# rug-marl-group2/scopa

Measured on AMD Instinct MI355X. Metric: MiniScopa infoset-traversals/sec, higher is better.
Workload: dtype f64

## Files before the change

include/scopa.h:

```cpp
#ifndef SCOPA_H
#define SCOPA_H
#include <stddef.h>
#include <stdint.h>

#ifdef __cplusplus
extern "C" {
#endif

#define SCOPA_ABI_VERSION 1

enum {
    SCOPA_OK = 0,
    SCOPA_EINVAL = -1,
    SCOPA_ENODEV = -2,
    SCOPA_EHIP = -3,
    SCOPA_ESTATE = -4,
    SCOPA_ENOMEM = -5,
    SCOPA_ELIMIT = -6,
    SCOPA_ETIMEOUT = -7
};

#define SCOPA_N_CARDS 16
#define SCOPA_N_PLIES 8
#define SCOPA_N_DECISION 1653
#define SCOPA_N_TERMINAL 576
#define SCOPA_N_NODES 2229
#define SCOPA_MAX_ACTIONS 4

#define SCOPA_STEP_CLONED 0x80u
#define SCOPA_STEP_COUNT_MASK 0x7Fu
typedef struct scopa_state {
    uint16_t hand[2];
    uint32_t table;
    uint8_t  nh[2];
    uint8_t  nt;
    uint8_t  step;
    uint8_t  ncap[2];
    uint8_t  scopas[2];
} scopa_state;

typedef struct scopa_ctx scopa_ctx;

int32_t     scopa_abi_version(void);
const char *scopa_strerror(int32_t status);
const char *scopa_last_error(const scopa_ctx *ctx);

int32_t scopa_ctx_create(int32_t device_id, void *hip_stream, scopa_ctx **out);
int32_t scopa_ctx_destroy(scopa_ctx *ctx);
int32_t scopa_ctx_synchronize(scopa_ctx *ctx);

int32_t scopa_deal_py_seed(int64_t seed, uint8_t perm16[16]);
int32_t scopa_state_init(const uint8_t perm16[16], scopa_state *out);
int32_t scopa_state_step(scopa_state *s, int32_t action);
int32_t scopa_state_clone(const scopa_state *s, scopa_state *out);
int32_t scopa_state_is_terminal(const scopa_state *s);
int32_t scopa_state_current_player(const scopa_state *s);
int32_t scopa_state_legal(const scopa_state *s, int32_t player , int32_t out[4], int32_t *n);
int32_t scopa_state_rewards_x2(const scopa_state *s, int32_t r2[2]);
int32_t scopa_state_infoset_key(const scopa_state *s, int32_t player, uint64_t *key);
int32_t scopa_key_to_string(uint64_t key, char *buf, int32_t cap);
int32_t scopa_state_infoset_string(const scopa_state *s, int32_t player, char *buf, int32_t cap);

int32_t scopa_step_batch(scopa_ctx *ctx, scopa_state *d_states, const uint8_t *d_actions, int64_t n);
int32_t scopa_step_batch_host(scopa_ctx *ctx, scopa_state *h_states, const uint8_t *h_actions, int64_t n);

int32_t scopa_set_deal(scopa_ctx *ctx, const uint8_t perm16[16]);
int32_t scopa_tree_counts(scopa_ctx *ctx, int32_t *n_nodes, int32_t *n_decision, int32_t *n_infosets);
int32_t scopa_tree_export(scopa_ctx *ctx, scopa_state *h_states, int32_t *h_infoset, int8_t *h_r2,
                          uint64_t *h_infoset_key, int8_t *h_infoset_nlegal, int8_t *h_infoset_legal);

int32_t scopa_tables_reset(scopa_ctx *ctx);
int32_t scopa_tables_get(scopa_ctx *ctx, double *h_regret, double *h_strategy, double *h_local);
int32_t scopa_tables_set(scopa_ctx *ctx, const double *h_regret, const double *h_strategy, const double *h_local);

int32_t scopa_visited_get(scopa_ctx *ctx, uint32_t *h_seq);

int32_t scopa_cfr_exact_iterate(scopa_ctx *ctx, int32_t n_iters, double *h_root_values);
int32_t scopa_cfr_exact_traverse(scopa_ctx *ctx, int32_t traverser, double *h_value);
int32_t scopa_cfr_exact_mode(scopa_ctx *ctx, int32_t sequential);
int32_t scopa_cfr_exact_last_route(scopa_ctx *ctx, int32_t *route);
int32_t scopa_cfr_exact_traverse_from(scopa_ctx *ctx, int32_t traverser, int32_t depth, const int32_t *path,
                                      double reach_p0, double reach_p1, double *h_value);

int32_t scopa_cfr_sync_iterate(scopa_ctx *ctx, int32_t n_iters);

int32_t scopa_mccfr_replay(scopa_ctx *ctx, int32_t n_iters, const double *h_uniforms, int64_t n_uniforms,
                           int64_t *consumed);

int32_t scopa_mccfr_seed(scopa_ctx *ctx, uint64_t seed);
int32_t scopa_mccfr_iterate(scopa_ctx *ctx, uint32_t batch, uint32_t n_iters);
int32_t scopa_mccfr_traverse(scopa_ctx *ctx, uint32_t iteration, uint32_t b0, uint32_t nb);
int32_t scopa_mccfr_delta_buffer(scopa_ctx *ctx, void **d_delta, size_t *bytes);
int32_t scopa_mccfr_bind_delta(scopa_ctx *ctx, void *d_buf, size_t bytes);
int32_t scopa_mccfr_delta_get(scopa_ctx *ctx, double *h_delta);
int32_t scopa_mccfr_delta_set(scopa_ctx *ctx, const double *h_delta);
int32_t scopa_mccfr_apply(scopa_ctx *ctx);
int32_t scopa_mccfr_iteration_counter(scopa_ctx *ctx, uint32_t *iteration);
int32_t scopa_mccfr_graph_mode(scopa_ctx *ctx, int32_t on);
int32_t scopa_debug_lds_limit(scopa_ctx *ctx, int32_t bytes);

int32_t scopa_sdcfr_frontier_width(int32_t traverser, int32_t ply);
int32_t scopa_sdcfr_features(scopa_ctx *ctx, int32_t ply, int64_t n, const int32_t *d_idx, float *d_feats, float *d_mask);
int32_t scopa_sdcfr_expand(scopa_ctx *ctx, int32_t ply, int32_t traverser, int64_t n, const int32_t *d_idx, const float *d_adv,
                           int32_t *d_child_idx, float *d_pol, const double *d_uniforms, uint32_t iteration, uint32_t b0);
int32_t scopa_sdcfr_terminal_values(scopa_ctx *ctx, int32_t traverser, int64_t n, const int32_t *d_idx, float *d_val);
int32_t scopa_sdcfr_backward(scopa_ctx *ctx, int32_t ply, int32_t traverser, int64_t n, const int32_t *d_idx, const float *d_pol,
                             const float *d_child_val, float *d_val, const float *d_feats, const float *d_mask, float *d_mem_feat,
                             float *d_mem_regret, float *d_mem_mask, int64_t capacity, int64_t write_base);
int32_t scopa_sdcfr_visits(scopa_ctx *ctx, uint64_t *decision_visits);
int32_t scopa_sdcfr_policy_get(scopa_ctx *ctx, float *h_policy, uint64_t *h_thr);
#define SCOPA_SDCFR_IMAGE_FLOATS 13520
int32_t scopa_sdcfr_image_floats(void);
int32_t scopa_sdcfr_pack_weights(scopa_ctx *ctx, int32_t player, const float *d_w1, const float *d_b1, const float *d_w2,
                                 const float *d_b2, const float *d_w3, const float *d_b3, float *d_image);
int32_t scopa_sdcfr_traverse_fused(scopa_ctx *ctx, int32_t traverser, int32_t batch, const float *d_image, float *d_mem_feat,
                                   float *d_mem_regret, float *d_mem_mask, int64_t capacity, int64_t write_base,
                                   float *d_root_values, const double *d_uniforms, uint32_t iteration, uint32_t b0);
int32_t scopa_sdcfr_mode(scopa_ctx *ctx, int32_t forward_per_visit);
int32_t scopa_sdcfr_tuning(scopa_ctx *ctx, int32_t traversals_per_task, int32_t wavefronts_per_task);
int32_t scopa_sdcfr_train_params(void);
int32_t scopa_sdcfr_train_steps(scopa_ctx *ctx, const int64_t *d_rows, int32_t n_rows, int32_t n_steps, const float *d_feat, const float *d_regret, const float *d_mask,
                                int64_t capacity, float *d_w1, float *d_b1, float *d_w2, float *d_b2, float *d_w3, float *d_b3, float *d_state,
                                int32_t first_step, float lr, float *d_loss);
int32_t scopa_sdcfr_train_step(scopa_ctx *ctx, const int64_t *d_rows, int32_t n_rows, const float *d_feat, const float *d_regret, const float *d_mask,
                               int64_t capacity, float *d_w1, float *d_b1, float *d_w2, float *d_b2, float *d_w3, float *d_b3, float *d_state,
                               int32_t step, float lr, float *d_loss);
int32_t scopa_sdcfr_average_policy(scopa_ctx *ctx, int32_t player, int32_t n_snap, const float *d_w1, const float *d_b1, const float *d_w2,
                                   const float *d_b2, const float *d_w3, const float *d_b3, int32_t max_size, const int32_t *d_slots,
                                   const float *d_coef, double *d_policy);
int32_t scopa_features_from_states(scopa_ctx *ctx, const scopa_state *d_states, int64_t n, float *d_feats, float *d_mask);
int32_t scopa_eval_init_states(scopa_ctx *ctx, scopa_state *d_states, int64_t n);
int32_t scopa_eval_step(scopa_ctx *ctx, scopa_state *d_states, int64_t n, const float *d_probs, const int32_t *d_trained_seat,
                        uint32_t stream_id, uint32_t ply_tag);

int32_t scopa_eval_tabular_prepare(scopa_ctx *ctx, const double *d_policy);
int32_t scopa_eval_tabular_step(scopa_ctx *ctx, scopa_state *d_states, int32_t *d_node_idx, int64_t n, int32_t ply,
                                const double *d_policy, const int32_t *d_trained_seat, uint32_t stream_id);
int32_t scopa_eval_tabular_match(scopa_ctx *ctx, int64_t n, int64_t n_seat0, uint32_t stream_id, scopa_state *d_states_out, int32_t *d_node_idx_out,
                                 int64_t h_stats[10]);

int32_t scopa_exploitability(scopa_ctx *ctx, const double *h_policy, double *h_out4, double *h_policy_out);

typedef struct scopa_multi scopa_multi;
int32_t scopa_multi_create(scopa_ctx *ctx, int32_t n_deals, scopa_multi **out);
int32_t scopa_multi_destroy(scopa_multi *m);
int32_t scopa_multi_deal_py_seeds(scopa_multi *m, const int64_t *h_seeds);
int32_t scopa_multi_set_perms(scopa_multi *m, const uint8_t *h_perms );
int32_t scopa_multi_perms_get(scopa_multi *m, uint8_t *h_perms);
int32_t scopa_multi_build(scopa_multi *m, int32_t *h_n_infosets);
int32_t scopa_multi_cfr_exact_iterate(scopa_multi *m, int32_t n_iters);
int32_t scopa_multi_cfr_exact_iterate_lanes(scopa_multi *m, int32_t n_iters);
int32_t scopa_multi_cfr_sync_iterate(scopa_multi *m, int32_t n_iters);
int32_t scopa_multi_mccfr_iterate(scopa_multi *m, uint32_t batch, uint32_t n_iters, uint64_t seed);
int32_t scopa_multi_exploitability(scopa_multi *m, double *h_out4);
int32_t scopa_multi_tables_get(scopa_multi *m, int32_t deal, double *h_regret, double *h_strategy, double *h_local, uint64_t *h_keys);
int32_t scopa_multi_tables_set(scopa_multi *m, int32_t deal, const double *h_regret, const double *h_strategy, const double *h_local);
int32_t scopa_multi_counters(scopa_multi *m, uint64_t *decision_visits, uint64_t *terminal_visits);

typedef struct scopa_full_state {
    uint64_t table[2];
    uint64_t cap[2];
    uint32_t hand[2];
    uint32_t game;
    uint8_t  nh[2], nt, deck_pos, round, last_capture , scopas[2];
    uint16_t step;
    uint8_t  terminal;
    int8_t   r2_p0;
    uint8_t  flags;
    uint8_t  pad[7];
} scopa_full_state;
int32_t scopa_full_deal_py_seed(int64_t seed, uint8_t perm40[40]);
int32_t scopa_full_state_init(const uint8_t deck40[40], uint32_t game, scopa_full_state *out);
int32_t scopa_full_state_step(scopa_full_state *s, const uint8_t deck40[40], int32_t action);
int32_t scopa_full_state_legal(const scopa_full_state *s, int32_t player, int32_t out[3], int32_t *n);
int32_t scopa_full_state_infoset_string(const scopa_full_state *s, int32_t player, char *buf, int32_t cap);
int32_t scopa_full_step_batch(scopa_ctx *ctx, scopa_full_state *d_states, const uint8_t *d_actions, const uint8_t *d_decks, int64_t n);
int32_t scopa_full_step_batch_host(scopa_ctx *ctx, scopa_full_state *h_states, const uint8_t *h_actions, const uint8_t *h_decks,
                                   int64_t n_decks, int64_t n);
int32_t scopa_full_random_playouts(scopa_ctx *ctx, const int64_t *h_seeds, int64_t n_games, int8_t *h_r2_p0, int16_t *h_plies);

typedef struct scopa_team_state {
    uint64_t history;
    uint32_t table;
    uint16_t hand[4];
    uint16_t cap[4];
    uint8_t  nh[4];
    uint8_t  scopas[4];
    uint8_t  nt, step, last_capture_team , flags ;
} scopa_team_state;
int32_t scopa_team_state_init(const uint8_t perm16[16], scopa_team_state *out);
int32_t scopa_team_state_step(scopa_team_state *s, int32_t action);
int32_t scopa_team_state_legal(const scopa_team_state *s, int32_t out[4], int32_t *n);
int32_t scopa_team_state_rewards_x2(const scopa_team_state *s, int32_t r2_seat[4]);
int32_t scopa_team_state_infoset_string(const scopa_team_state *s, int32_t team, char *buf, int32_t cap);
int32_t scopa_team_step_batch(scopa_ctx *ctx, scopa_team_state *d_states, const uint8_t *d_actions, int64_t n);
int32_t scopa_team_step_batch_host(scopa_ctx *ctx, scopa_team_state *h_states, const uint8_t *h_actions, int64_t n);
int32_t scopa_team_random_playouts(scopa_ctx *ctx, const int64_t *h_seeds, int64_t n_games, int8_t *h_r2_team0, uint8_t *h_scopas);

int32_t scopa_p2p_create(scopa_ctx *ctx, int32_t rank, int32_t world, uint8_t handle_out[64]);
int32_t scopa_p2p_connect(scopa_ctx *ctx, const uint8_t *handles );
int32_t scopa_p2p_allreduce_delta(scopa_ctx *ctx);
int32_t scopa_p2p_set_form(scopa_ctx *ctx, int32_t light);
int32_t scopa_p2p_set_budget(scopa_ctx *ctx, double seconds);
int32_t scopa_mccfr_iterate_sharded(scopa_ctx *ctx, uint32_t b0, uint32_t nb, uint32_t n_iters);
int32_t scopa_p2p_status(scopa_ctx *ctx, int32_t *timeouts, uint64_t *exchanges);
int32_t scopa_p2p_destroy(scopa_ctx *ctx);

int32_t scopa_counters(scopa_ctx *ctx, uint64_t *decision_visits, uint64_t *terminal_visits);
int32_t scopa_prof_enable(scopa_ctx *ctx, int32_t stride);
int32_t scopa_prof_read(scopa_ctx *ctx, int64_t *launches, double *kernel_ms);
int32_t scopa_prof_device(scopa_ctx *ctx, int64_t *launches, double *kernel_ms);
int32_t scopa_prof_phases(scopa_ctx *ctx, double out_us[3]);
int32_t scopa_prof_spread(scopa_ctx *ctx, double out_us[3]);

#ifdef __cplusplus
}
#endif
#endif
```

scopa_amd/_lib.py:

```python
import ctypes as C
import os

import numpy as np

_HERE = os.path.dirname(os.path.abspath(__file__))
LIB_PATH = os.environ.get("SCOPA_HIP_LIBRARY") or os.path.join(_HERE, "libscopa_hip.so")

SCOPA_OK, SCOPA_EINVAL, SCOPA_ENODEV, SCOPA_EHIP, SCOPA_ESTATE, SCOPA_ENOMEM, SCOPA_ELIMIT, SCOPA_ETIMEOUT = 0, -1, -2, -3, -4, -5, -6, -7
N_NODES, N_DECISION, N_TERMINAL = 2229, 1653, 576

SYMBOLS = [
    "scopa_abi_version", "scopa_strerror", "scopa_last_error", "scopa_ctx_create", "scopa_ctx_destroy",
    "scopa_ctx_synchronize", "scopa_deal_py_seed", "scopa_state_init", "scopa_state_step", "scopa_state_clone", "scopa_state_is_terminal",
    "scopa_state_current_player", "scopa_state_legal", "scopa_state_rewards_x2", "scopa_state_infoset_key",
    "scopa_key_to_string", "scopa_state_infoset_string", "scopa_step_batch", "scopa_step_batch_host", "scopa_set_deal",
    "scopa_tree_counts", "scopa_tree_export", "scopa_tables_reset", "scopa_tables_get", "scopa_tables_set",
    "scopa_visited_get", "scopa_cfr_exact_iterate", "scopa_cfr_exact_traverse", "scopa_cfr_exact_mode", "scopa_cfr_exact_last_route", "scopa_cfr_exact_traverse_from", "scopa_mccfr_replay", "scopa_mccfr_seed",
    "scopa_mccfr_iterate", "scopa_mccfr_traverse", "scopa_mccfr_delta_buffer", "scopa_mccfr_bind_delta", "scopa_mccfr_delta_get", "scopa_mccfr_delta_set", "scopa_mccfr_apply",
    "scopa_mccfr_iteration_counter", "scopa_mccfr_graph_mode", "scopa_debug_lds_limit", "scopa_sdcfr_frontier_width", "scopa_sdcfr_features", "scopa_sdcfr_expand",
    "scopa_sdcfr_terminal_values", "scopa_sdcfr_backward", "scopa_sdcfr_visits", "scopa_sdcfr_policy_get", "scopa_sdcfr_traverse_fused", "scopa_sdcfr_image_floats", "scopa_sdcfr_pack_weights", "scopa_sdcfr_tuning", "scopa_sdcfr_mode", "scopa_sdcfr_train_params", "scopa_sdcfr_train_step", "scopa_sdcfr_train_steps", "scopa_sdcfr_average_policy", "scopa_features_from_states",
    "scopa_eval_init_states", "scopa_eval_step", "scopa_eval_tabular_step", "scopa_eval_tabular_prepare", "scopa_eval_tabular_match", "scopa_cfr_sync_iterate", "scopa_multi_create", "scopa_multi_destroy",
    "scopa_multi_deal_py_seeds", "scopa_multi_set_perms", "scopa_multi_perms_get", "scopa_multi_build", "scopa_multi_cfr_exact_iterate",
    "scopa_multi_cfr_exact_iterate_lanes", "scopa_multi_cfr_sync_iterate", "scopa_multi_mccfr_iterate", "scopa_multi_exploitability", "scopa_multi_tables_get", "scopa_multi_tables_set", "scopa_multi_counters", "scopa_full_deal_py_seed",
    "scopa_full_state_init", "scopa_full_state_step", "scopa_full_state_legal", "scopa_full_state_infoset_string",
    "scopa_full_step_batch", "scopa_full_step_batch_host", "scopa_full_random_playouts",
    "scopa_team_state_init", "scopa_team_state_step", "scopa_team_state_legal", "scopa_team_state_rewards_x2", "scopa_team_state_infoset_string",
    "scopa_team_step_batch", "scopa_team_step_batch_host", "scopa_team_random_playouts",
    "scopa_mccfr_iterate_sharded", "scopa_p2p_create", "scopa_p2p_connect", "scopa_p2p_allreduce_delta", "scopa_p2p_set_form", "scopa_p2p_set_budget", "scopa_p2p_status", "scopa_p2p_destroy", "scopa_exploitability", "scopa_counters", "scopa_prof_enable", "scopa_prof_read", "scopa_prof_device", "scopa_prof_phases", "scopa_prof_spread",
]


class ScopaError(RuntimeError):
    def __init__(self, status, where, detail=""):
        self.status = status
        msg = f"{where}: status {status}"
        try:
            msg += f" ({lib().scopa_strerror(status).decode()})"
        except Exception:
            pass
        if detail:
            msg += f": {detail}"
        super().__init__(msg)


class State16(C.Structure):
    _fields_ = [("hand", C.c_uint16 * 2), ("table", C.c_uint32), ("nh", C.c_uint8 * 2), ("nt", C.c_uint8),
                ("step", C.c_uint8), ("ncap", C.c_uint8 * 2), ("scopas", C.c_uint8 * 2)]


STEP_CLONED, STEP_COUNT_MASK = 0x80, 0x7F
STATE_DTYPE = np.dtype([("hand", "<u2", (2,)), ("table", "<u4"), ("nh", "u1", (2,)), ("nt", "u1"), ("step", "u1"),
                        ("ncap", "u1", (2,)), ("scopas", "u1", (2,))])
assert STATE_DTYPE.itemsize == 16 and C.sizeof(State16) == 16

_lib = None


def lib():
    global _lib
    if _lib is not None:
        return _lib
    try:
        import torch
    except ImportError:
        pass
    if not os.path.exists(LIB_PATH):
        raise OSError(f"{LIB_PATH} is missing: build it with `python __graft_entry__.py` or `python scopa_amd/build.py` "
                      "(the MiniScopa solver path has no fallback)")
    L = C.CDLL(LIB_PATH)
    vp, i32, i64, u32, u64 = C.c_void_p, C.c_int32, C.c_int64, C.c_uint32, C.c_uint64
    sig = {
        "scopa_abi_version": (i32, []),
        "scopa_strerror": (C.c_char_p, [i32]),
        "scopa_last_error": (C.c_char_p, [vp]),
        "scopa_ctx_create": (i32, [i32, vp, C.POINTER(vp)]),
        "scopa_ctx_destroy": (i32, [vp]),
        "scopa_ctx_synchronize": (i32, [vp]),
        "scopa_deal_py_seed": (i32, [i64, vp]),
        "scopa_state_init": (i32, [vp, C.POINTER(State16)]),
        "scopa_state_step": (i32, [C.POINTER(State16), i32]),
        "scopa_state_clone": (i32, [C.POINTER(State16), C.POINTER(State16)]),
        "scopa_state_is_terminal": (i32, [C.POINTER(State16)]),
        "scopa_state_current_player": (i32, [C.POINTER(State16)]),
        "scopa_state_legal": (i32, [C.POINTER(State16), i32, C.POINTER(i32 * 4), C.POINTER(i32)]),
        "scopa_state_rewards_x2": (i32, [C.POINTER(State16), C.POINTER(i32 * 2)]),
        "scopa_state_infoset_key": (i32, [C.POINTER(State16), i32, C.POINTER(u64)]),
        "scopa_key_to_string": (i32, [u64, C.c_char_p, i32]),
        "scopa_state_infoset_string": (i32, [C.POINTER(State16), i32, C.c_char_p, i32]),
        "scopa_step_batch": (i32, [vp, vp, vp, i64]),
        "scopa_step_batch_host": (i32, [vp, vp, vp, i64]),
        "scopa_set_deal": (i32, [vp, vp]),
        "scopa_tree_counts": (i32, [vp, C.POINTER(i32), C.POINTER(i32), C.POINTER(i32)]),
        "scopa_tree_export": (i32, [vp, vp, vp, vp, vp, vp, vp]),
        "scopa_tables_reset": (i32, [vp]),
        "scopa_tables_get": (i32, [vp, vp, vp, vp]),
        "scopa_tables_set": (i32, [vp, vp, vp, vp]),
        "scopa_cfr_exact_iterate": (i32, [vp, i32, vp]),
        "scopa_cfr_exact_traverse": (i32, [vp, i32, C.POINTER(C.c_double)]),
        "scopa_cfr_exact_mode": (i32, [vp, i32]),
        "scopa_cfr_exact_last_route": (i32, [vp, C.POINTER(i32)]),
        "scopa_cfr_exact_traverse_from": (i32, [vp, i32, i32, vp, C.c_double, C.c_double, C.POINTER(C.c_double)]),
        "scopa_visited_get": (i32, [vp, vp]),
        "scopa_mccfr_replay": (i32, [vp, i32, vp, i64, C.POINTER(i64)]),
        "scopa_mccfr_seed": (i32, [vp, u64]),
        "scopa_mccfr_iterate": (i32, [vp, u32, u32]),
        "scopa_mccfr_traverse": (i32, [vp, u32, u32, u32]),
        "scopa_mccfr_delta_buffer": (i32, [vp, C.POINTER(vp), C.POINTER(C.c_size_t)]),
        "scopa_mccfr_bind_delta": (i32, [vp, vp, C.c_size_t]),
        "scopa_mccfr_delta_get": (i32, [vp, vp]),
        "scopa_mccfr_delta_set": (i32, [vp, vp]),
        "scopa_mccfr_apply": (i32, [vp]),
        "scopa_mccfr_iteration_counter": (i32, [vp, C.POINTER(u32)]),
        "scopa_mccfr_graph_mode": (i32, [vp, i32]),
        "scopa_debug_lds_limit": (i32, [vp, i32]),
        "scopa_exploitability": (i32, [vp, vp, vp, vp]),
        "scopa_sdcfr_frontier_width": (i32, [i32, i32]),
        "scopa_sdcfr_features": (i32, [vp, i32, i64, vp, vp, vp]),
        "scopa_sdcfr_expand": (i32, [vp, i32, i32, i64, vp, vp, vp, vp, vp, u32, u32]),
        "scopa_sdcfr_terminal_values": (i32, [vp, i32, i64, vp, vp]),
        "scopa_sdcfr_backward": (i32, [vp, i32, i32, i64, vp, vp, vp, vp, vp, vp, vp, vp, vp, i64, i64]),
        "scopa_sdcfr_visits": (i32, [vp, C.POINTER(u64)]),
        "scopa_sdcfr_policy_get": (i32, [vp, vp, vp]),
        "scopa_sdcfr_traverse_fused": (i32, [vp, i32, i32, vp, vp, vp, vp, i64, i64, vp, vp, u32, u32]),
        "scopa_sdcfr_image_floats": (i32, []),
        "scopa_sdcfr_pack_weights": (i32, [vp, i32, vp, vp, vp, vp, vp, vp, vp]),
        "scopa_sdcfr_tuning": (i32, [vp, i32, i32]),
        "scopa_sdcfr_train_params": (i32, []),
        "scopa_sdcfr_train_step": (i32, [vp, vp, i32, vp, vp, vp, i64, vp, vp, vp, vp, vp, vp, vp, i32, C.c_float, vp]),
        "scopa_sdcfr_train_steps": (i32, [vp, vp, i32, i32, vp, vp, vp, i64, vp, vp, vp, vp, vp, vp, vp, i32, C.c_float, vp]),
        "scopa_sdcfr_mode": (i32, [vp, i32]),
        "scopa_sdcfr_average_policy": (i32, [vp, i32, i32, vp, vp, vp, vp, vp, vp, i32, vp, vp, vp]),
        "scopa_features_from_states": (i32, [vp, vp, i64, vp, vp]),
        "scopa_eval_init_states": (i32, [vp, vp, i64]),
        "scopa_eval_step": (i32, [vp, vp, i64, vp, vp, u32, u32]),
        "scopa_eval_tabular_step": (i32, [vp, vp, vp, i64, i32, vp, vp, u32]),
        "scopa_eval_tabular_prepare": (i32, [vp, vp]),
        "scopa_eval_tabular_match": (i32, [vp, i64, i64, u32, vp, vp, vp]),
        "scopa_cfr_sync_iterate": (i32, [vp, i32]),
        "scopa_multi_create": (i32, [vp, i32, C.POINTER(vp)]),
        "scopa_multi_destroy": (i32, [vp]),
        "scopa_multi_deal_py_seeds": (i32, [vp, vp]),
        "scopa_multi_set_perms": (i32, [vp, vp]),
        "scopa_multi_perms_get": (i32, [vp, vp]),
        "scopa_multi_build": (i32, [vp, vp]),
        "scopa_multi_cfr_exact_iterate": (i32, [vp, i32]),
        "scopa_multi_cfr_sync_iterate": (i32, [vp, i32]),
        "scopa_multi_cfr_exact_iterate_lanes": (i32, [vp, i32]),
        "scopa_multi_exploitability": (i32, [vp, vp]),
        "scopa_multi_mccfr_iterate": (i32, [vp, u32, u32, u64]),
        "scopa_multi_tables_get": (i32, [vp, i32, vp, vp, vp, vp]),
        "scopa_multi_tables_set": (i32, [vp, i32, vp, vp, vp]),
        "scopa_multi_counters": (i32, [vp, C.POINTER(u64), C.POINTER(u64)]),
        "scopa_full_deal_py_seed": (i32, [i64, vp]),
        "scopa_full_state_init": (i32, [vp, u32, vp]),
        "scopa_full_state_step": (i32, [vp, vp, i32]),
        "scopa_full_state_legal": (i32, [vp, i32, C.POINTER(i32 * 3), C.POINTER(i32)]),
        "scopa_full_state_infoset_string": (i32, [vp, i32, C.c_char_p, i32]),
        "scopa_full_step_batch": (i32, [vp, vp, vp, vp, i64]),
        "scopa_full_step_batch_host": (i32, [vp, vp, vp, vp, i64, i64]),
        "scopa_full_random_playouts": (i32, [vp, vp, i64, vp, vp]),
        "scopa_mccfr_iterate_sharded": (i32, [vp, u32, u32, u32]),
        "scopa_p2p_create": (i32, [vp, i32, i32, vp]),
        "scopa_p2p_connect": (i32, [vp, vp]),
        "scopa_p2p_allreduce_delta": (i32, [vp]),
        "scopa_p2p_set_form": (i32, [vp, i32]),
        "scopa_p2p_set_budget": (i32, [vp, C.c_double]),
        "scopa_p2p_status": (i32, [vp, C.POINTER(i32), C.POINTER(u64)]),
        "scopa_p2p_destroy": (i32, [vp]),
        "scopa_team_state_init": (i32, [vp, vp]),
        "scopa_team_state_step": (i32, [vp, i32]),
        "scopa_team_state_legal": (i32, [vp, C.POINTER(i32 * 4), C.POINTER(i32)]),
        "scopa_team_state_rewards_x2": (i32, [vp, C.POINTER(i32 * 4)]),
        "scopa_team_state_infoset_string": (i32, [vp, i32, C.c_char_p, i32]),
        "scopa_team_step_batch": (i32, [vp, vp, vp, i64]),
        "scopa_team_step_batch_host": (i32, [vp, vp, vp, i64]),
        "scopa_team_random_playouts": (i32, [vp, vp, i64, vp, vp]),
        "scopa_counters": (i32, [vp, C.POINTER(u64), C.POINTER(u64)]),
        "scopa_prof_enable": (i32, [vp, i32]),
        "scopa_prof_read": (i32, [vp, C.POINTER(i64), C.POINTER(C.c_double)]),
        "scopa_prof_device": (i32, [vp, C.POINTER(i64), C.POINTER(C.c_double)]),
        "scopa_prof_phases": (i32, [vp, C.POINTER(C.c_double * 3)]),
        "scopa_prof_spread": (i32, [vp, C.POINTER(C.c_double * 3)]),
    }
    lenient = bool(os.environ.get("SCOPA_HIP_LIBRARY")) and os.environ.get("SCOPA_AB_OLD_LIBRARY") == "1"
    for name, (res, args) in sig.items():
        if lenient and not hasattr(L, name):
            continue
        fn = getattr(L, name)
        fn.restype, fn.argtypes = res, args
    if L.scopa_abi_version() != 1:
        raise OSError("libscopa_hip.so ABI version mismatch")
    _lib = L
    return L


def _ptr(a):
    return a.ctypes.data_as(C.c_void_p) if a is not None else None


def deal_py_seed(seed):
    perm = np.zeros(16, np.uint8)
    rc = lib().scopa_deal_py_seed(int(seed), _ptr(perm))
    if rc:
        raise ScopaError(rc, "scopa_deal_py_seed")
    return perm


def key_to_string(key):
    buf = C.create_string_buffer(96)
    rc = lib().scopa_key_to_string(int(key), buf, 96)
    if rc < 0:
        raise ScopaError(rc, "scopa_key_to_string")
    return buf.value.decode()


class Context:

    def __init__(self, device=0, stream=None):
        self._h = C.c_void_p()
        self._L = lib()
        rc = self._L.scopa_ctx_create(int(device), C.c_void_p(stream) if stream else None, C.byref(self._h))
        if rc:
            self._h = None
            raise ScopaError(rc, "scopa_ctx_create", "a GPU is required: the solver path has no CPU fallback")
        self.device = device
        self.n_infosets = 0
        self._children = []

    def close(self):
        if getattr(self, "_h", None):
            for ref in getattr(self, "_children", []):
                child = ref()
                if child is not None:
                    child.close()
            self._L.scopa_ctx_destroy(self._h)
            self._h = None

    def __del__(self):
        try:
            self.close()
        except Exception:
            pass

    def _ck(self, rc, where):
        if rc:
            raise ScopaError(rc, where, self._L.scopa_last_error(self._h).decode())

    def synchronize(self):
        self._ck(self._L.scopa_ctx_synchronize(self._h), "scopa_ctx_synchronize")

    def step_batch_host(self, states, actions):
        assert states.dtype == STATE_DTYPE and states.flags.c_contiguous
        actions = np.ascontiguousarray(actions, np.uint8)
        assert actions.size == states.size
        self._ck(self._L.scopa_step_batch_host(self._h, _ptr(states), _ptr(actions), states.size), "scopa_step_batch_host")
        return states

    def step_batch(self, d_states_ptr, d_actions_ptr, n):
        self._ck(self._L.scopa_step_batch(self._h, C.c_void_p(d_states_ptr), C.c_void_p(d_actions_ptr), int(n)), "scopa_step_batch")

    def set_deal(self, perm16):
        perm = np.ascontiguousarray(perm16, np.uint8)
        assert perm.size == 16
        self._ck(self._L.scopa_set_deal(self._h, _ptr(perm)), "scopa_set_deal")
        a, b, c = C.c_int32(), C.c_int32(), C.c_int32()
        self._ck(self._L.scopa_tree_counts(self._h, C.byref(a), C.byref(b), C.byref(c)), "scopa_tree_counts")
        self.n_infosets = c.value
        self.perm = perm
        return self.n_infosets

    def tree_export(self):
        I = self.n_infosets
        out = dict(states=np.zeros(N_NODES, STATE_DTYPE), infoset=np.zeros(N_NODES, np.int32), r2=np.zeros((N_NODES, 2), np.int8),
                   infoset_key=np.zeros(I, np.uint64), infoset_nlegal=np.zeros(I, np.int8), infoset_legal=np.zeros((I, 4), np.int8))
        self._ck(self._L.scopa_tree_export(self._h, _ptr(out["states"]), _ptr(out["infoset"]), _ptr(out["r2"]),
                                           _ptr(out["infoset_key"]), _ptr(out["infoset_nlegal"]), _ptr(out["infoset_legal"])),
                 "scopa_tree_export")
        return out

    def tables_reset(self):
        self._ck(self._L.scopa_tables_reset(self._h), "scopa_tables_reset")

    def tables_get(self, regret=True, strategy=True, local=True):
        I = self.n_infosets
        R = np.zeros((I, 4)) if regret else None
        S = np.zeros((I, 4)) if strategy else None
        Lc = np.zeros((I, 4)) if local else None
        self._ck(self._L.scopa_tables_get(self._h, _ptr(R), _ptr(S), _ptr(Lc)), "scopa_tables_get")
        return R, S, Lc

    def tables_set(self, regret=None, strategy=None, local=None):
        arrs = []
        for a in (regret, strategy, local):
            if a is not None:
                a = np.ascontiguousarray(a, np.float64)
                assert a.shape == (self.n_infosets, 4)
            arrs.append(a)
        self._ck(self._L.scopa_tables_set(self._h, _ptr(arrs[0]), _ptr(arrs[1]), _ptr(arrs[2])), "scopa_tables_set")

    def cfr_exact_iterate(self, n_iters):
        rv = np.zeros((max(int(n_iters), 0), 2))
        self._ck(self._L.scopa_cfr_exact_iterate(self._h, int(n_iters), _ptr(rv)), "scopa_cfr_exact_iterate")
        return rv

    def cfr_exact_mode(self, sequential):
        self._ck(self._L.scopa_cfr_exact_mode(self._h, 1 if sequential else 0), "scopa_cfr_exact_mode")

    def cfr_exact_last_route(self):
        r = C.c_int32()
        self._ck(self._L.scopa_cfr_exact_last_route(self._h, C.byref(r)), "scopa_cfr_exact_last_route")
        return r.value

    def cfr_exact_traverse(self, traverser):
        v = C.c_double()
        self._ck(self._L.scopa_cfr_exact_traverse(self._h, int(traverser), C.byref(v)), "scopa_cfr_exact_traverse")
        return v.value

    def cfr_exact_traverse_from(self, traverser, path, reach_p0=1.0, reach_p1=1.0):
        pa = np.ascontiguousarray(path, np.int32)
        v = C.c_double()
        self._ck(self._L.scopa_cfr_exact_traverse_from(self._h, int(traverser), pa.size, _ptr(pa), float(reach_p0), float(reach_p1),
                                                       C.byref(v)), "scopa_cfr_exact_traverse_from")
        return v.value

    def visited_get(self):
        seq = np.zeros(self.n_infosets, np.uint32)
        self._ck(self._L.scopa_visited_get(self._h, _ptr(seq)), "scopa_visited_get")
        return seq

    def mccfr_replay(self, n_iters, uniforms):
        u = np.ascontiguousarray(uniforms, np.float64)
        used = C.c_int64()
        self._ck(self._L.scopa_mccfr_replay(self._h, int(n_iters), _ptr(u), u.size, C.byref(used)), "scopa_mccfr_replay")
        return used.value

    def mccfr_seed(self, seed):
        self._ck(self._L.scopa_mccfr_seed(self._h, int(seed)), "scopa_mccfr_seed")

    def mccfr_iterate(self, batch, n_iters):
        self._ck(self._L.scopa_mccfr_iterate(self._h, int(batch), int(n_iters)), "scopa_mccfr_iterate")

    def mccfr_traverse(self, iteration, b0, nb):
        self._ck(self._L.scopa_mccfr_traverse(self._h, int(iteration), int(b0), int(nb)), "scopa_mccfr_traverse")

    def mccfr_delta_buffer(self):
        p, n = C.c_void_p(), C.c_size_t()
        self._ck(self._L.scopa_mccfr_delta_buffer(self._h, C.byref(p), C.byref(n)), "scopa_mccfr_delta_buffer")
        return p.value, n.value

    def mccfr_bind_delta(self, d_ptr, nbytes):
        self._ck(self._L.scopa_mccfr_bind_delta(self._h, C.c_void_p(d_ptr) if d_ptr else None, int(nbytes)), "scopa_mccfr_bind_delta")

    def mccfr_delta_get(self):
        d = np.zeros((self.n_infosets, 5))
        self._ck(self._L.scopa_mccfr_delta_get(self._h, _ptr(d)), "scopa_mccfr_delta_get")
        return d

    def mccfr_delta_set(self, d):
        d = np.ascontiguousarray(d, np.float64)
        assert d.shape == (self.n_infosets, 5)
        self._ck(self._L.scopa_mccfr_delta_set(self._h, _ptr(d)), "scopa_mccfr_delta_set")

    def mccfr_apply(self):
        self._ck(self._L.scopa_mccfr_apply(self._h), "scopa_mccfr_apply")

    def mccfr_graph_mode(self, on):
        self._ck(self._L.scopa_mccfr_graph_mode(self._h, 1 if on else 0), "scopa_mccfr_graph_mode")

    def debug_lds_limit(self, nbytes):
        self._ck(self._L.scopa_debug_lds_limit(self._h, int(nbytes)), "scopa_debug_lds_limit")

    def mccfr_iteration(self):
        v = C.c_uint32()
        self._ck(self._L.scopa_mccfr_iteration_counter(self._h, C.byref(v)), "scopa_mccfr_iteration_counter")
        return v.value

    def exploitability(self, policy=None, return_policy=False):
        pin = None if policy is None else np.ascontiguousarray(policy, np.float64)
        out = np.zeros(4)
        pout = np.zeros((self.n_infosets, 4)) if return_policy else None
        self._ck(self._L.scopa_exploitability(self._h, _ptr(pin), _ptr(out), _ptr(pout)), "scopa_exploitability")
        res = dict(exploitability=out[0], br0=out[1], br1=out[2], value_p0=out[3])
        if return_policy:
            res["policy"] = pout
        return res

    def sdcfr_features(self, ply, n, idx_ptr, feats_ptr, mask_ptr):
        self._ck(self._L.scopa_sdcfr_features(self._h, ply, n, C.c_void_p(idx_ptr), C.c_void_p(feats_ptr), C.c_void_p(mask_ptr)), "scopa_sdcfr_features")

    def sdcfr_expand(self, ply, traverser, n, idx_ptr, adv_ptr, child_ptr, pol_ptr, uniforms_ptr, iteration, b0):
        self._ck(self._L.scopa_sdcfr_expand(self._h, ply, traverser, n, C.c_void_p(idx_ptr), C.c_void_p(adv_ptr), C.c_void_p(child_ptr),
                                            C.c_void_p(pol_ptr), C.c_void_p(uniforms_ptr) if uniforms_ptr else None, iteration, b0), "scopa_sdcfr_expand")

    def sdcfr_terminal_values(self, traverser, n, idx_ptr, val_ptr):
        self._ck(self._L.scopa_sdcfr_terminal_values(self._h, traverser, n, C.c_void_p(idx_ptr), C.c_void_p(val_ptr)), "scopa_sdcfr_terminal_values")

    def sdcfr_backward(self, ply, traverser, n, idx_ptr, pol_ptr, child_val_ptr, val_ptr, feats_ptr, mask_ptr, mem_feat_ptr, mem_regret_ptr,
                       mem_mask_ptr, capacity, write_base):
        vp = lambda x: C.c_void_p(x) if x else None
        self._ck(self._L.scopa_sdcfr_backward(self._h, ply, traverser, n, vp(idx_ptr), vp(pol_ptr), vp(child_val_ptr), vp(val_ptr), vp(feats_ptr),
                                              vp(mask_ptr), vp(mem_feat_ptr), vp(mem_regret_ptr), vp(mem_mask_ptr), capacity, write_base),
                 "scopa_sdcfr_backward")

    def sdcfr_pack_weights(self, player, w1_ptr, b1_ptr, w2_ptr, b2_ptr, w3_ptr, b3_ptr, image_ptr):
        self._ck(self._L.scopa_sdcfr_pack_weights(self._h, player, *(C.c_void_p(x) for x in (w1_ptr, b1_ptr, w2_ptr, b2_ptr, w3_ptr, b3_ptr, image_ptr))),
                 "scopa_sdcfr_pack_weights")

    def sdcfr_mode(self, forward_per_visit):
        self._ck(self._L.scopa_sdcfr_mode(self._h, 1 if forward_per_visit else 0), "scopa_sdcfr_mode")

    def sdcfr_tuning(self, traversals_per_task=0, wavefronts_per_task=0):
        self._ck(self._L.scopa_sdcfr_tuning(self._h, traversals_per_task, wavefronts_per_task), "scopa_sdcfr_tuning")

    def sdcfr_train_steps(self, rows_ptr, n_rows, n_steps, feat_ptr, regret_ptr, mask_ptr, capacity, param_ptrs, state_ptr, first_step, lr, loss_ptr):
        self._ck(self._L.scopa_sdcfr_train_steps(self._h, C.c_void_p(rows_ptr), int(n_rows), int(n_steps), C.c_void_p(feat_ptr), C.c_void_p(regret_ptr), C.c_void_p(mask_ptr),
                                                 int(capacity), *(C.c_void_p(p) for p in param_ptrs), C.c_void_p(state_ptr), int(first_step), float(lr),
                                                 C.c_void_p(loss_ptr)), "scopa_sdcfr_train_steps")

    def sdcfr_train_step(self, rows_ptr, n_rows, feat_ptr, regret_ptr, mask_ptr, capacity, param_ptrs, state_ptr, step, lr, loss_ptr):
        self._ck(self._L.scopa_sdcfr_train_step(self._h, C.c_void_p(rows_ptr), int(n_rows), C.c_void_p(feat_ptr), C.c_void_p(regret_ptr), C.c_void_p(mask_ptr),
                                                int(capacity), *(C.c_void_p(p) for p in param_ptrs), C.c_void_p(state_ptr), int(step), float(lr),
                                                C.c_void_p(loss_ptr)), "scopa_sdcfr_train_step")

    def sdcfr_traverse_fused(self, traverser, batch, weights_ptr, mem_feat_ptr, mem_regret_ptr, mem_mask_ptr, capacity, write_base,
                             root_values_ptr, uniforms_ptr, iteration, b0):
        self._ck(self._L.scopa_sdcfr_traverse_fused(self._h, traverser, batch, C.c_void_p(weights_ptr), C.c_void_p(mem_feat_ptr),
                                                    C.c_void_p(mem_regret_ptr), C.c_void_p(mem_mask_ptr), capacity, write_base,
                                                    C.c_void_p(root_values_ptr), C.c_void_p(uniforms_ptr) if uniforms_ptr else None,
                                                    iteration, b0), "scopa_sdcfr_traverse_fused")

    def sdcfr_average_policy(self, player, n_snap, param_ptrs, max_size, slots_ptr, coef_ptr, policy_ptr):
        vp = lambda x: C.c_void_p(x) if x else None
        self._ck(self._L.scopa_sdcfr_average_policy(self._h, int(player), int(n_snap), *(vp(p) for p in param_ptrs), int(max_size), vp(slots_ptr),
                                                    vp(coef_ptr), vp(policy_ptr)), "scopa_sdcfr_average_policy")

    def sdcfr_visits(self):
        v = C.c_uint64()
        self._ck(self._L.scopa_sdcfr_visits(self._h, C.byref(v)), "scopa_sdcfr_visits")
        return v.value

    def sdcfr_policy_get(self):
        pol, thr = np.zeros((N_DECISION, 4), np.float32), np.zeros((N_DECISION, 3), np.uint64)
        self._ck(self._L.scopa_sdcfr_policy_get(self._h, _ptr(pol), _ptr(thr)), "scopa_sdcfr_policy_get")
        return pol, thr

    def features_from_states(self, states_ptr, n, feats_ptr, mask_ptr):
        self._ck(self._L.scopa_features_from_states(self._h, C.c_void_p(states_ptr), n, C.c_void_p(feats_ptr), C.c_void_p(mask_ptr)), "scopa_features_from_states")

    def eval_init_states(self, states_ptr, n):
        self._ck(self._L.scopa_eval_init_states(self._h, C.c_void_p(states_ptr), n), "scopa_eval_init_states")

    def eval_step(self, states_ptr, n, probs_ptr, seat_ptr, stream_id, ply_tag):
        self._ck(self._L.scopa_eval_step(self._h, C.c_void_p(states_ptr), n, C.c_void_p(probs_ptr) if probs_ptr else None, C.c_void_p(seat_ptr),
                                         stream_id, ply_tag), "scopa_eval_step")

    def eval_tabular_prepare(self, policy_ptr):
        self._ck(self._L.scopa_eval_tabular_prepare(self._h, C.c_void_p(policy_ptr)), "scopa_eval_tabular_prepare")

    def eval_tabular_step(self, states_ptr, idx_ptr, n, ply, policy_ptr, seat_ptr, stream_id):
        self._ck(self._L.scopa_eval_tabular_step(self._h, C.c_void_p(states_ptr), C.c_void_p(idx_ptr), n, ply, C.c_void_p(policy_ptr) if policy_ptr else None,
                                                 C.c_void_p(seat_ptr), stream_id), "scopa_eval_tabular_step")

    def eval_tabular_match(self, n, n_seat0, stream_id, states_ptr=0, idx_ptr=0):
        st = np.zeros((2, 5), np.int64)
        self._ck(self._L.scopa_eval_tabular_match(self._h, int(n), int(n_seat0), stream_id, C.c_void_p(states_ptr) if states_ptr else None,
                                                  C.c_void_p(idx_ptr) if idx_ptr else None, _ptr(st)), "scopa_eval_tabular_match")
        return st

    def cfr_sync_iterate(self, n_iters):
        self._ck(self._L.scopa_cfr_sync_iterate(self._h, int(n_iters)), "scopa_cfr_sync_iterate")

    def full_step_batch_host(self, states, actions, decks):
        assert states.dtype == FULL_STATE_DTYPE
        actions = np.ascontiguousarray(actions, np.uint8)
        decks = np.ascontiguousarray(decks, np.uint8).reshape(-1, 40)
        self._ck(self._L.scopa_full_step_batch_host(self._h, _ptr(states), _ptr(actions), _ptr(decks), decks.shape[0], states.size),
                 "scopa_full_step_batch_host")
        return states

    def full_step_batch(self, states_ptr, actions_ptr, decks_ptr, n):
        self._ck(self._L.scopa_full_step_batch(self._h, C.c_void_p(states_ptr), C.c_void_p(actions_ptr), C.c_void_p(decks_ptr), int(n)), "scopa_full_step_batch")

    def full_random_playouts(self, seeds):
        seeds = np.ascontiguousarray(seeds, np.int64)
        r2, plies = np.zeros(seeds.size, np.int8), np.zeros(seeds.size, np.int16)
        self._ck(self._L.scopa_full_random_playouts(self._h, _ptr(seeds), seeds.size, _ptr(r2), _ptr(plies)), "scopa_full_random_playouts")
        return r2, plies

    def p2p_create(self, rank, world):
        h = np.zeros(64, np.uint8)
        self._ck(self._L.scopa_p2p_create(self._h, int(rank), int(world), _ptr(h)), "scopa_p2p_create")
        return h

    def p2p_connect(self, handles):
        handles = np.ascontiguousarray(handles, np.uint8).reshape(-1, 64)
        self._ck(self._L.scopa_p2p_connect(self._h, _ptr(handles)), "scopa_p2p_connect")

    def p2p_allreduce_delta(self):
        self._ck(self._L.scopa_p2p_allreduce_delta(self._h), "scopa_p2p_allreduce_delta")

    def mccfr_iterate_sharded(self, b0, nb, n_iters=1):
        self._ck(self._L.scopa_mccfr_iterate_sharded(self._h, int(b0), int(nb), int(n_iters)), "scopa_mccfr_iterate_sharded")

    def p2p_status(self):
        t, n = C.c_int32(), C.c_uint64()
        self._ck(self._L.scopa_p2p_status(self._h, C.byref(t), C.byref(n)), "scopa_p2p_status")
        return t.value, n.value

    def p2p_set_form(self, light):
        self._ck(self._L.scopa_p2p_set_form(self._h, 1 if light else 0), "scopa_p2p_set_form")

    def p2p_set_budget(self, seconds):
        self._ck(self._L.scopa_p2p_set_budget(self._h, float(seconds)), "scopa_p2p_set_budget")

    def p2p_destroy(self):
        self._ck(self._L.scopa_p2p_destroy(self._h), "scopa_p2p_destroy")

    def team_step_batch_host(self, states, actions):
        assert states.dtype == TEAM_STATE_DTYPE
        actions = np.ascontiguousarray(actions, np.uint8)
        self._ck(self._L.scopa_team_step_batch_host(self._h, _ptr(states), _ptr(actions), states.size), "scopa_team_step_batch_host")
        return states

    def team_step_batch(self, states_ptr, actions_ptr, n):
        self._ck(self._L.scopa_team_step_batch(self._h, C.c_void_p(states_ptr), C.c_void_p(actions_ptr), int(n)), "scopa_team_step_batch")

    def team_random_playouts(self, seeds):
        seeds = np.ascontiguousarray(seeds, np.int64)
        r2, sc = np.zeros(seeds.size, np.int8), np.zeros((seeds.size, 4), np.uint8)
        self._ck(self._L.scopa_team_random_playouts(self._h, _ptr(seeds), seeds.size, _ptr(r2), _ptr(sc)), "scopa_team_random_playouts")
        return r2, sc

    def counters(self):
        a, b = C.c_uint64(), C.c_uint64()
        self._ck(self._L.scopa_counters(self._h, C.byref(a), C.byref(b)), "scopa_counters")
        return a.value, b.value

    def prof_enable(self, stride=1):
        self._ck(self._L.scopa_prof_enable(self._h, int(stride)), "scopa_prof_enable")

    def prof_read(self):
        n, ms = C.c_int64(), C.c_double()
        self._ck(self._L.scopa_prof_read(self._h, C.byref(n), C.byref(ms)), "scopa_prof_read")
        return n.value, ms.value

    def prof_phases(self):
        out = (C.c_double * 3)()
        self._ck(self._L.scopa_prof_phases(self._h, C.byref(out)), "scopa_prof_phases")
        return tuple(out)

    def prof_spread(self):
        out = (C.c_double * 3)()
        self._ck(self._L.scopa_prof_spread(self._h, C.byref(out)), "scopa_prof_spread")
        return [out[0], out[1], out[2]]

    def prof_device(self):
        n, ms = C.c_int64(), C.c_double()
        self._ck(self._L.scopa_prof_device(self._h, C.byref(n), C.byref(ms)), "scopa_prof_device")
        return n.value, ms.value


FULL_STATE_DTYPE = np.dtype([("table", "<u8", (2,)), ("cap", "<u8", (2,)), ("hand", "<u4", (2,)), ("game", "<u4"), ("nh", "u1", (2,)),
                             ("nt", "u1"), ("deck_pos", "u1"), ("round", "u1"), ("last_capture", "u1"), ("scopas", "u1", (2,)),
                             ("step", "<u2"), ("terminal", "u1"), ("r2_p0", "i1"), ("flags", "u1"), ("pad", "u1", (7,))])
assert FULL_STATE_DTYPE.itemsize == 64


def full_deal_py_seed(seed):
    perm = np.zeros(40, np.uint8)
    rc = lib().scopa_full_deal_py_seed(int(seed), _ptr(perm))
    if rc:
        raise ScopaError(rc, "scopa_full_deal_py_seed")
    return perm


class FullState:

    def __init__(self, seed=42, deck=None, game=0):
        self.deck = np.ascontiguousarray(full_deal_py_seed(seed) if deck is None else deck, np.uint8)
        self.s = np.zeros(1, FULL_STATE_DTYPE)
        rc = lib().scopa_full_state_init(_ptr(self.deck), int(game), _ptr(self.s))
        if rc:
            raise ScopaError(rc, "scopa_full_state_init")

    def step(self, action):
        rc = lib().scopa_full_state_step(_ptr(self.s), _ptr(self.deck), int(action))
        if rc:
            raise ScopaError(rc, "scopa_full_state_step")

    def legal(self, player=-1):
        out, n = (C.c_int32 * 3)(), C.c_int32()
        lib().scopa_full_state_legal(_ptr(self.s), int(player), C.byref(out), C.byref(n))
        return [out[i] for i in range(n.value)]

    def is_terminal(self):
        return bool(self.s[0]["terminal"])

    def current_player(self):
        return -4 if self.is_terminal() else int(self.s[0]["step"]) & 1

    def rewards(self):
        r = int(self.s[0]["r2_p0"])
        return [r / 2.0, -r / 2.0] if self.is_terminal() else [0, 0]

    def infoset_string(self, player):
        buf = C.create_string_buffer(256)
        lib().scopa_full_state_infoset_string(_ptr(self.s), int(player), buf, 256)
        return buf.value.decode()

    def snapshot(self):
        return unpack_full_state(self.s[0])


def unpack_full_state(s):
    tab = [int((int(s["table"][i // 10]) >> (6 * (i % 10))) & 63) for i in range(int(s["nt"]))]
    hands = [[int((int(s["hand"][p]) >> (6 * i)) & 63) for i in range(int(s["nh"][p]))] for p in range(2)]
    caps = [[c for c in range(40) if (int(s["cap"][p]) >> c) & 1] for p in range(2)]
    last = int(s["last_capture"])
    return dict(hands=hands, table=tab, caps=caps, scopas=[int(s["scopas"][0]), int(s["scopas"][1])], round=int(s["round"]),
                step=int(s["step"]), deck_remaining=40 - int(s["deck_pos"]), last=-1 if last == 255 else last)


TEAM_STATE_DTYPE = np.dtype([("history", "<u8"), ("table", "<u4"), ("hand", "<u2", (4,)), ("cap", "<u2", (4,)), ("nh", "u1", (4,)),
                             ("scopas", "u1", (4,)), ("nt", "u1"), ("step", "u1"), ("last_capture_team", "u1"), ("flags", "u1")])
assert TEAM_STATE_DTYPE.itemsize == 40


class TeamState:

    def __init__(self, seed=42, perm=None):
        self.perm = np.ascontiguousarray(deal_py_seed(seed) if perm is None else perm, np.uint8)
        self.s = np.zeros(1, TEAM_STATE_DTYPE)
        rc = lib().scopa_team_state_init(_ptr(self.perm), _ptr(self.s))
        if rc:
            raise ScopaError(rc, "scopa_team_state_init")

    def copy(self):
        c = TeamState.__new__(TeamState)
        c.perm, c.s = self.perm, self.s.copy()
        return c

    def step(self, action):
        rc = lib().scopa_team_state_step(_ptr(self.s), int(action))
        if rc:
            raise ScopaError(rc, "scopa_team_state_step")

    def legal(self):
        out, n = (C.c_int32 * 4)(), C.c_int32()
        lib().scopa_team_state_legal(_ptr(self.s), C.byref(out), C.byref(n))
        return [out[i] for i in range(n.value)]

    def is_terminal(self):
        return bool(int(self.s[0]["flags"]) & 1)

    def seat(self):
        return int(self.s[0]["step"]) & 3

    def current_player(self):
        return -4 if self.is_terminal() else self.seat() >> 1

    def player_rewards(self):
        r = (C.c_int32 * 4)()
        lib().scopa_team_state_rewards_x2(_ptr(self.s), C.byref(r))
        return [r[i] / 2.0 for i in range(4)]

    def rewards(self):
        if not self.is_terminal():
            return [0, 0]
        r = self.player_rewards()
        return [(r[0] + r[1]) / 2, (r[2] + r[3]) / 2]

    def infoset_string(self, team):
        buf = C.create_string_buffer(256)
        lib().scopa_team_state_infoset_string(_ptr(self.s), int(team), buf, 256)
        return buf.value.decode()

    def history(self):
        h = int(self.s[0]["history"])
        return [(h >> (4 * i)) & 15 for i in range(int(self.s[0]["step"]))]

    def history_str(self):
        h = "-".join(map(str, self.history()))
        if self.is_terminal():
            return f"TERMINAL:{h}:" + ",".join(f"{r:.2f}" for r in self.rewards())
        return f"H:{h}:T{self.current_player()}"

    def snapshot(self):
        d = unpack_team_state(self.s[0])
        d.update(cur=self.current_player(), legal=self.legal(), info0=self.infoset_string(0), info1=self.infoset_string(1),
                 hist=self.history_str(), rewards=[float(r) for r in self.rewards()])
        return d


def unpack_team_state(s):
    hands = [[(int(s["hand"][p]) >> (4 * i)) & 15 for i in range(int(s["nh"][p]))] for p in range(4)]
    last = int(s["last_capture_team"])
    return dict(hands=hands, table=[(int(s["table"]) >> (4 * i)) & 15 for i in range(int(s["nt"]))],
                caps=[[c for c in range(16) if (int(s["cap"][p]) >> c) & 1] for p in range(4)], scopas=[int(x) for x in s["scopas"]],
                last=-1 if last == 255 else last, step=int(s["step"]), seat=int(s["step"]) & 3, term=bool(int(s["flags"]) & 1))


class MultiDeal:

    def __init__(self, ctx, n_deals):
        self.ctx, self.n = ctx, int(n_deals)
        self._L = lib()
        self._h = C.c_void_p()
        ctx._ck(self._L.scopa_multi_create(ctx._h, self.n, C.byref(self._h)), "scopa_multi_create")
        self.n_infosets = None
        import weakref
        ctx._children.append(weakref.ref(self))

    def close(self):
        if getattr(self, "_h", None):
            self._L.scopa_multi_destroy(self._h)
            self._h = None

    def __del__(self):
        try:
            self.close()
        except Exception:
            pass

    def deal_py_seeds(self, seeds):
        s = np.ascontiguousarray(seeds, np.int64)
        assert s.size == self.n
        self.ctx._ck(self._L.scopa_multi_deal_py_seeds(self._h, _ptr(s)), "scopa_multi_deal_py_seeds")

    def set_perms(self, perms):
        p = np.ascontiguousarray(perms, np.uint8)
        assert p.shape == (self.n, 16)
        self.ctx._ck(self._L.scopa_multi_set_perms(self._h, _ptr(p)), "scopa_multi_set_perms")

    def perms(self):
        p = np.zeros((self.n, 16), np.uint8)
        self.ctx._ck(self._L.scopa_multi_perms_get(self._h, _ptr(p)), "scopa_multi_perms_get")
        return p

    def build(self):
        ninf = np.zeros(self.n, np.int32)
        self.ctx._ck(self._L.scopa_multi_build(self._h, _ptr(ninf)), "scopa_multi_build")
        self.n_infosets = ninf
        return ninf

    def cfr_exact_iterate(self, n_iters):
        self.ctx._ck(self._L.scopa_multi_cfr_exact_iterate(self._h, int(n_iters)), "scopa_multi_cfr_exact_iterate")

    def cfr_exact_iterate_lanes(self, n_iters):
        self.ctx._ck(self._L.scopa_multi_cfr_exact_iterate_lanes(self._h, int(n_iters)), "scopa_multi_cfr_exact_iterate_lanes")

    def cfr_sync_iterate(self, n_iters):
        self.ctx._ck(self._L.scopa_multi_cfr_sync_iterate(self._h, int(n_iters)), "scopa_multi_cfr_sync_iterate")

    def mccfr_iterate(self, batch, n_iters, seed=0x5C09A):
        self.ctx._ck(self._L.scopa_multi_mccfr_iterate(self._h, int(batch), int(n_iters), int(seed)), "scopa_multi_mccfr_iterate")

    def exploitability(self):
        out = np.zeros((self.n, 4))
        self.ctx._ck(self._L.scopa_multi_exploitability(self._h, _ptr(out)), "scopa_multi_exploitability")
        return out

    def tables_get(self, deal):
        I = int(self.n_infosets[deal])
        R, S, Lc, K = np.zeros((I, 4)), np.zeros((I, 4)), np.zeros((I, 4)), np.zeros(I, np.uint64)
        self.ctx._ck(self._L.scopa_multi_tables_get(self._h, int(deal), _ptr(R), _ptr(S), _ptr(Lc), _ptr(K)), "scopa_multi_tables_get")
        return R, S, Lc, K

    def tables_set(self, deal, regret=None, strategy=None, local=None):
        arrs = []
        for a in (regret, strategy, local):
            if a is not None:
                a = np.ascontiguousarray(a, np.float64)
                assert a.shape == (int(self.n_infosets[deal]), 4)
            arrs.append(a)
        self.ctx._ck(self._L.scopa_multi_tables_set(self._h, int(deal), _ptr(arrs[0]), _ptr(arrs[1]), _ptr(arrs[2])), "scopa_multi_tables_set")

    def counters(self):
        a, b = C.c_uint64(), C.c_uint64()
        self.ctx._ck(self._L.scopa_multi_counters(self._h, C.byref(a), C.byref(b)), "scopa_multi_counters")
        return a.value, b.value
```

scopa_amd/csrc/scopa_ctx.h:

```cpp
#pragma once
#include <hip/hip_runtime.h>
#include <stdint.h>
#include <stdio.h>

#include <vector>

#include "../../include/scopa.h"
#include "scopa_rules.h"

struct scopa_p2p;

struct scopa_ctx {
    int device = -1;
    hipStream_t stream = nullptr;
    bool own_stream = false;
    char err[512] = {0};

    bool has_deal = false;
    uint8_t perm[16] = {0};
    int n_infosets = 0;

    scopa_state *d_states = nullptr;
    uint16_t *d_infoset = nullptr;
    int8_t *d_payoff = nullptr;
    uint64_t *d_key = nullptr;
    int32_t *d_meta = nullptr;
    uint32_t *d_visit = nullptr;

    double *d_regret = nullptr, *d_strat = nullptr, *d_local = nullptr;
    double *d_delta = nullptr;
    double *d_delta_own = nullptr;
    double *d_scratch = nullptr;
    double *d_sigcdf = nullptr;
    bool sigcdf_valid = false;
    bool mccfr_all_seen = false;
    uint32_t mccfr_seen_wait = 0;
    double *d_groups = nullptr;
    unsigned long long *d_clock = nullptr;
    uint16_t clock_grid[2048] = {0};
    double prof_phase_us[3] = {0.0, 0.0, 0.0};
    double prof_spread_us[3] = {0.0, 0.0, 0.0};
    size_t scratch_bytes = 0;

    unsigned long long *d_counters = nullptr;

    uint64_t seed = 0x5C09A;
    uint64_t sdcfr_visits = 0;
    void *d_sdnode = nullptr;
    bool sdnode_valid = false;
    void *d_eval_thr = nullptr;
    bool eval_thr_valid = false;
    void *d_train_partial = nullptr;
    void *d_sdpol = nullptr;
    void *d_sdavg = nullptr;
    size_t sdavg_bytes = 0;
    int sdcfr_mode = 0;
    uint32_t iteration = 0;

    bool prof_on = false;
    int prof_stride = 1;
    long long prof_tick = 0;
    std::vector<hipEvent_t> ev_pool;
    size_t ev_used = 0;
    int64_t prof_launches = 0;
    double prof_ms = 0.0;

    uint32_t *d_lane_tab = nullptr;
    uint16_t *d_sched = nullptr;
    int sched_steps = 0;
    bool sched_valid = false;
    int exact_last_route = -1;
    bool exact_sequential = false;

    scopa_p2p *p2p = nullptr;

    struct GraphEntry { uint32_t batch, k, track; void *exec; };
    std::vector<GraphEntry> mccfr_graphs;
    bool mccfr_graph_mode = false;

    int lds_limit = 160 * 1024;
    int n_cus = 256;
    uint32_t lds_attr_done = 0;
};

namespace scopa {

#ifndef SCOPA_GROUPS
#define SCOPA_GROUPS 16
#endif
#ifndef SCOPA_GROUP_PERM
#define SCOPA_GROUP_PERM 0
#endif
constexpr int kDeltaGroups = SCOPA_GROUPS;
constexpr int kGroupRows = 1664;
constexpr size_t kDeltaTable = (size_t)kGroupRows * 5;
__host__ __device__ inline size_t group_cell(int k, int r) {
#if SCOPA_GROUP_PERM == 1
    return (size_t)k * kGroupRows + (size_t)((r & 63) * 26 + (r >> 6));
#elif SCOPA_GROUP_PERM == 2
    return (size_t)k * kGroupRows + (size_t)((r & 7) * 208 + (r >> 3));
#else
    return (size_t)k * kGroupRows + (size_t)r;
#endif
}
constexpr int kClockSamples = 2048, kClockStride = 2048;

inline int32_t fail(scopa_ctx *ctx, int32_t code, const char *what, hipError_t e = hipSuccess) {
    if (ctx) {
        if (e != hipSuccess) snprintf(ctx->err, sizeof ctx->err, "%s: %s", what, hipGetErrorString(e));
        else snprintf(ctx->err, sizeof ctx->err, "%s", what);
    }
    return code;
}

#define SC_HIP(ctx, call)                                                         \
    do {                                                                          \
        hipError_t e__ = (call);                                                  \
        if (e__ != hipSuccess) return scopa::fail((ctx), SCOPA_EHIP, #call, e__); \
    } while (0)

#define SC_REQUIRE(ctx, cond, code, msg)                        \
    do {                                                        \
        if (!(cond)) return scopa::fail((ctx), (code), (msg)); \
    } while (0)

int32_t ensure_scratch(scopa_ctx *ctx, size_t bytes);

void range_push(const char *name);
void range_pop();
struct Range { explicit Range(const char *n) { range_push(n); } ~Range() { range_pop(); } };

enum LdsAttrKernel : uint32_t { kLdsTraverse = 1u, kLdsReplay = 8u, kLdsCfrExact = 16u, kLdsCfrSched = 512u, kLdsExploit = 32u, kLdsCfrSync = 64u, kLdsSdcfr = 128u, kLdsMulti = 256u, kLdsSdcfrReplay = 1024u, kLdsSdPolicy = 2048u, kLdsSdWalk0 = 4096u, kLdsSdWalk1 = 8192u };
inline int32_t ensure_lds_attr(scopa_ctx *ctx, uint32_t kernel_bit, const void *fn, int bytes) {
    if (ctx->lds_attr_done & kernel_bit) return SCOPA_OK;
    SC_HIP(ctx, hipFuncSetAttribute(fn, hipFuncAttributeMaxDynamicSharedMemorySize, bytes));
    ctx->lds_attr_done |= kernel_bit;
    return SCOPA_OK;
}
#define SC_LDS_ATTR(ctx, bit, kernel, bytes)                                                                     \
    do {                                                                                                         \
        const int32_t rc__ = scopa::ensure_lds_attr((ctx), (bit), reinterpret_cast<const void *>(kernel), (bytes)); \
        if (rc__ != SCOPA_OK) return rc__;                                                                       \
    } while (0)
bool prof_events(scopa_ctx *ctx, hipEvent_t *start, hipEvent_t *stop);
void p2p_release(scopa_ctx *ctx);
void mccfr_graphs_clear(scopa_ctx *ctx);

}
```

scopa_amd/csrc/scopa_host.hip:

```cpp
#include <string.h>

#include <new>

#include "scopa_ctx.h"

using namespace scopa;

namespace scopa {

int32_t ensure_scratch(scopa_ctx *ctx, size_t bytes) {
    if (bytes <= ctx->scratch_bytes) return SCOPA_OK;
    if (ctx->d_scratch) SC_HIP(ctx, hipFree(ctx->d_scratch));
    ctx->d_scratch = nullptr;
    ctx->scratch_bytes = 0;
    SC_HIP(ctx, hipMalloc(&ctx->d_scratch, bytes));
    ctx->scratch_bytes = bytes;
    return SCOPA_OK;
}

static void prof_pool_fill(scopa_ctx *ctx) {
    while (ctx->ev_pool.size() < 4096) {
        hipEvent_t e;
        if (hipEventCreate(&e) != hipSuccess) break;
        ctx->ev_pool.push_back(e);
    }
}

bool prof_events(scopa_ctx *ctx, hipEvent_t *start, hipEvent_t *stop) {
    if (!ctx->prof_on) return false;
    if ((ctx->prof_tick++ % ctx->prof_stride) != 0) return false;
    if (ctx->ev_used + 2 > ctx->ev_pool.size()) {
        if (ctx->ev_used) {
            (void)hipEventSynchronize(ctx->ev_pool[ctx->ev_used - 1]);
            for (size_t i = 0; i + 1 < ctx->ev_used; i += 2) {
                float ms = 0.f;
                if (hipEventElapsedTime(&ms, ctx->ev_pool[i], ctx->ev_pool[i + 1]) == hipSuccess) ctx->prof_ms += ms;
            }
            ctx->ev_used = 0;
        }
        if (ctx->ev_pool.empty()) prof_pool_fill(ctx);
    }
    if (ctx->ev_used + 2 > ctx->ev_pool.size()) return false;
    *start = ctx->ev_pool[ctx->ev_used];
    *stop = ctx->ev_pool[ctx->ev_used + 1];
    ctx->ev_used += 2;
    ctx->prof_launches++;
    return true;
}

}

#include <dlfcn.h>
namespace scopa {
namespace {
int (*g_roctx_push)(const char *) = nullptr;
int (*g_roctx_pop)() = nullptr;
int g_roctx_state = 0;
void roctx_resolve() {
    g_roctx_state = -1;
    const char *on = getenv("SCOPA_ROCTX");
    if (!on || on[0] != '1') return;
    for (const char *lib : {"librocprofiler-sdk-roctx.so", "libroctx64.so"}) {
        void *h = dlopen(lib, RTLD_NOW | RTLD_GLOBAL);
        if (!h) continue;
        g_roctx_push = reinterpret_cast<int (*)(const char *)>(dlsym(h, "roctxRangePushA"));
        g_roctx_pop = reinterpret_cast<int (*)()>(dlsym(h, "roctxRangePop"));
        if (g_roctx_push && g_roctx_pop) { g_roctx_state = 1; return; }
    }
}
}
void range_push(const char *name) {
    if (g_roctx_state == 0) roctx_resolve();
    if (g_roctx_state == 1) (void)g_roctx_push(name);
}
void range_pop() {
    if (g_roctx_state == 1) (void)g_roctx_pop();
}
}

extern "C" {

int32_t scopa_abi_version(void) { return SCOPA_ABI_VERSION; }

const char *scopa_strerror(int32_t status) {
    switch (status) {
        case SCOPA_OK: return "ok";
        case SCOPA_EINVAL: return "invalid argument";
        case SCOPA_ENODEV: return "no usable HIP device (the solver path has no CPU fallback)";
        case SCOPA_EHIP: return "HIP runtime error";
        case SCOPA_ESTATE: return "call order violated";
        case SCOPA_ENOMEM: return "out of memory";
        case SCOPA_ELIMIT: return "problem exceeds a compiled-in capacity";
        case SCOPA_ETIMEOUT: return "a peer did not answer within the wait budget";
        default: return "unknown status";
    }
}

const char *scopa_last_error(const scopa_ctx *ctx) { return ctx ? ctx->err : "null context"; }

int32_t scopa_ctx_create(int32_t device_id, void *hip_stream, scopa_ctx **out) {
    if (!out || device_id < 0) return SCOPA_EINVAL;
    *out = nullptr;
    int count = 0;
    if (hipGetDeviceCount(&count) != hipSuccess || count <= 0) return SCOPA_ENODEV;
    if (device_id >= count) return SCOPA_ENODEV;
    scopa_ctx *ctx = new (std::nothrow) scopa_ctx();
    if (!ctx) return SCOPA_ENOMEM;
    ctx->device = device_id;
    hipError_t e = hipSetDevice(device_id);
    if (e != hipSuccess) { delete ctx; return SCOPA_ENODEV; }
    hipDeviceProp_t prop;
    if (hipGetDeviceProperties(&prop, device_id) == hipSuccess) {
        ctx->n_cus = prop.multiProcessorCount;
        ctx->lds_limit = (int)prop.sharedMemPerBlock;
    }
    if (hip_stream) ctx->stream = (hipStream_t)hip_stream;
    else {
        e = hipStreamCreateWithFlags(&ctx->stream, hipStreamNonBlocking);
        if (e != hipSuccess) { delete ctx; return SCOPA_EHIP; }
        ctx->own_stream = true;
    }
    const size_t rows = (size_t)kDecision;
    bool ok = hipMalloc(&ctx->d_states, sizeof(scopa_state) * kNodes) == hipSuccess &&
              hipMalloc(&ctx->d_infoset, sizeof(uint16_t) * kDecision) == hipSuccess &&
              hipMalloc(&ctx->d_payoff, kTerminal) == hipSuccess &&
              hipMalloc(&ctx->d_key, sizeof(uint64_t) * kDecision) == hipSuccess &&
              hipMalloc(&ctx->d_meta, sizeof(int32_t) * 8) == hipSuccess &&
              hipMalloc(&ctx->d_visit, sizeof(uint32_t) * kDecision) == hipSuccess &&
              hipMalloc(&ctx->d_sigcdf, (size_t)kDecision * 6 * sizeof(double)) == hipSuccess &&
              hipMalloc(&ctx->d_groups, scopa::kDeltaGroups * scopa::kDeltaTable * sizeof(double)) == hipSuccess &&
              hipMalloc(&ctx->d_regret, rows * 4 * sizeof(double)) == hipSuccess &&
              hipMalloc(&ctx->d_strat, rows * 4 * sizeof(double)) == hipSuccess &&
              hipMalloc(&ctx->d_local, rows * 4 * sizeof(double)) == hipSuccess &&
              hipMalloc(&ctx->d_delta_own, rows * 5 * sizeof(double)) == hipSuccess &&
              hipMalloc(&ctx->d_counters, (8 + 2 * 1024) * sizeof(unsigned long long)) == hipSuccess;
    ctx->d_delta = ctx->d_delta_own;
    if (ok) ok = hipMemsetAsync(ctx->d_counters, 0, (8 + 2 * 1024) * sizeof(unsigned long long), ctx->stream) == hipSuccess &&
                 hipMemsetAsync(ctx->d_delta, 0, rows * 5 * sizeof(double), ctx->stream) == hipSuccess &&
                 hipMemsetAsync(ctx->d_groups, 0, scopa::kDeltaGroups * scopa::kDeltaTable * sizeof(double), ctx->stream) == hipSuccess;
    if (!ok) { scopa_ctx_destroy(ctx); return SCOPA_ENOMEM; }
    *out = ctx;
    return SCOPA_OK;
}

int32_t scopa_ctx_destroy(scopa_ctx *ctx) {
    if (!ctx) return SCOPA_EINVAL;
    (void)hipSetDevice(ctx->device);
    (void)hipStreamSynchronize(ctx->stream);
    scopa::p2p_release(ctx);
    scopa::mccfr_graphs_clear(ctx);
    for (hipEvent_t e : ctx->ev_pool) (void)hipEventDestroy(e);
    void *bufs[] = {ctx->d_states, ctx->d_infoset, ctx->d_payoff, ctx->d_key, ctx->d_meta, ctx->d_regret, ctx->d_strat,
                    ctx->d_local, ctx->d_delta_own, ctx->d_scratch, ctx->d_counters, ctx->d_visit, ctx->d_sigcdf, ctx->d_groups, ctx->d_clock, ctx->d_sched, ctx->d_lane_tab, ctx->d_sdnode, ctx->d_sdpol, ctx->d_train_partial, ctx->d_eval_thr, ctx->d_sdavg};
    for (void *b : bufs) if (b) (void)hipFree(b);
    if (ctx->own_stream) (void)hipStreamDestroy(ctx->stream);
    delete ctx;
    return SCOPA_OK;
}

int32_t scopa_debug_lds_limit(scopa_ctx *ctx, int32_t bytes) {
    if (!ctx || bytes < 0) return SCOPA_EINVAL;
    hipDeviceProp_t prop;
    SC_HIP(ctx, hipGetDeviceProperties(&prop, ctx->device));
    SC_REQUIRE(ctx, bytes == 0 || (bytes >= 64 * 1024 && (size_t)bytes <= prop.sharedMemPerBlock), SCOPA_EINVAL, "scopa_debug_lds_limit: 0 or 64 KB .. the device's limit");
    ctx->lds_limit = bytes ? bytes : (int)prop.sharedMemPerBlock;
    ctx->lds_attr_done = 0;
    scopa::mccfr_graphs_clear(ctx);
    return SCOPA_OK;
}

int32_t scopa_ctx_synchronize(scopa_ctx *ctx) {
    if (!ctx) return SCOPA_EINVAL;
    SC_HIP(ctx, hipStreamSynchronize(ctx->stream));
    return SCOPA_OK;
}

namespace {
struct Mt19937 {
    uint32_t mt[624];
    int at = 624;
    void seed_u32(uint32_t s) {
        mt[0] = s;
        for (int i = 1; i < 624; i++) mt[i] = 1812433253u * (mt[i - 1] ^ (mt[i - 1] >> 30)) + (uint32_t)i;
        at = 624;
    }
    void seed_array(const uint32_t *key, int n) {
        seed_u32(19650218u);
        int i = 1, j = 0;
        for (int k = n > 624 ? n : 624; k > 0; k--) {
            mt[i] = (mt[i] ^ ((mt[i - 1] ^ (mt[i - 1] >> 30)) * 1664525u)) + key[j] + (uint32_t)j;
            if (++i >= 624) { mt[0] = mt[623]; i = 1; }
            if (++j >= n) j = 0;
        }
        for (int k = 623; k > 0; k--) {
            mt[i] = (mt[i] ^ ((mt[i - 1] ^ (mt[i - 1] >> 30)) * 1566083941u)) - (uint32_t)i;
            if (++i >= 624) { mt[0] = mt[623]; i = 1; }
        }
        mt[0] = 0x80000000u;
    }
    void refill() {
        for (int k = 0; k < 624; k++) {
            const uint32_t y = (mt[k] & 0x80000000u) | (mt[(k + 1) % 624] & 0x7fffffffu);
            mt[k] = mt[(k + 397) % 624] ^ (y >> 1) ^ ((y & 1u) ? 0x9908b0dfu : 0u);
        }
        at = 0;
    }
    uint32_t next() {
        if (at >= 624) refill();
        uint32_t y = mt[at++];
        y ^= y >> 11;
        y ^= (y << 7) & 0x9d2c5680u;
        y ^= (y << 15) & 0xefc60000u;
        y ^= y >> 18;
        return y;
    }
    uint32_t below(uint32_t n) {
        int bits = 32 - __builtin_clz(n);
        uint32_t r;
        do r = next() >> (32 - bits); while (r >= n);
        return r;
    }
};
}

int32_t scopa_deal_py_seed(int64_t seed, uint8_t perm16[16]) {
    if (!perm16) return SCOPA_EINVAL;
    const uint64_t a = seed < 0 ? (uint64_t)0 - (uint64_t)seed : (uint64_t)seed;
    const uint32_t key[2] = {(uint32_t)a, (uint32_t)(a >> 32)};
    Mt19937 g;
    g.seed_array(key, key[1] ? 2 : 1);
    for (int i = 0; i < 16; i++) perm16[i] = (uint8_t)i;
    for (uint32_t i = 15; i >= 1; i--) {
        const uint32_t j = g.below(i + 1);
        const uint8_t t = perm16[i]; perm16[i] = perm16[j]; perm16[j] = t;
    }
    return SCOPA_OK;
}

static bool perm_ok(const uint8_t *p) {
    uint32_t seen = 0;
    for (int i = 0; i < 16; i++) { if (p[i] > 15) return false; seen |= 1u << p[i]; }
    return seen == 0xFFFFu;
}

int32_t scopa_state_init(const uint8_t perm16[16], scopa_state *out) {
    if (!perm16 || !out || !perm_ok(perm16)) return SCOPA_EINVAL;
    state_init(*out, perm16);
    return SCOPA_OK;
}

int32_t scopa_state_step(scopa_state *s, int32_t action) {
    if (!s || action < 0 || action > 15) return SCOPA_EINVAL;
    step(*s, action);
    return SCOPA_OK;
}

int32_t scopa_state_clone(const scopa_state *s, scopa_state *out) {
    if (!s || !out) return SCOPA_EINVAL;
    scopa_state c = *s;
    if (!is_terminal(c)) c.step = (uint8_t)(c.step | SCOPA_STEP_CLONED);
    *out = c;
    return SCOPA_OK;
}

int32_t scopa_state_is_terminal(const scopa_state *s) { return s ? (is_terminal(*s) ? 1 : 0) : SCOPA_EINVAL; }

int32_t scopa_state_current_player(const scopa_state *s) { return s ? current_player(*s) : SCOPA_EINVAL; }

int32_t scopa_state_legal(const scopa_state *s, int32_t player, int32_t out[4], int32_t *n) {
    if (!s || !out || !n || player > 1) return SCOPA_EINVAL;
    int tmp[4];
    *n = legal(*s, player, tmp);
    for (int i = 0; i < *n; i++) out[i] = tmp[i];
    return SCOPA_OK;
}

int32_t scopa_state_rewards_x2(const scopa_state *s, int32_t r2[2]) {
    if (!s || !r2) return SCOPA_EINVAL;
    int a, b;
    rewards_x2(*s, a, b);
    r2[0] = a; r2[1] = b;
    return SCOPA_OK;
}

int32_t scopa_state_infoset_key(const scopa_state *s, int32_t player, uint64_t *key) {
    if (!s || !key || player > 1) return SCOPA_EINVAL;
    if (player < 0) player = s->step & 1;
    *key = infoset_key(*s, player);
    return SCOPA_OK;
}

int32_t scopa_key_to_string(uint64_t key, char *buf, int32_t cap) {
    if (!buf || cap < 64) return SCOPA_EINVAL;
    static const char suit[4] = {'c', 'f', 'p', 'b'};
    const int player = (int)(key & 1), nh = (int)((key >> 1) & 7), nt = (int)((key >> 20) & 15);
    const uint32_t hand = (uint32_t)((key >> 4) & 0xFFFF), table = (uint32_t)(key >> 24);
    char *w = buf;
    w += sprintf(w, "P%d:H[", player);
    for (int i = 0; i < nh; i++) w += sprintf(w, "%s%d%c", i ? "-" : "", card_rank(nib(hand, i)), suit[nib(hand, i) >> 2]);
    w += sprintf(w, "]_T[");
    for (int i = 0; i < nt; i++) w += sprintf(w, "%s%d%c", i ? "-" : "", card_rank(nib(table, i)), suit[nib(table, i) >> 2]);
    w += sprintf(w, "]");
    return (int32_t)(w - buf);
}

int32_t scopa_state_infoset_string(const scopa_state *s, int32_t player, char *buf, int32_t cap) {
    if (!s || !buf || cap < 64 || player > 1) return SCOPA_EINVAL;
    if (player < 0) player = current_player(*s);
    if (is_terminal(*s) || player < 0) return (int32_t)sprintf(buf, "TERMINAL");
    return scopa_key_to_string(infoset_key(*s, player), buf, cap);
}

int32_t scopa_tables_get(scopa_ctx *ctx, double *h_regret, double *h_strategy, double *h_local) {
    if (!ctx) return SCOPA_EINVAL;
    SC_REQUIRE(ctx, ctx->has_deal, SCOPA_ESTATE, "scopa_tables_get: no deal set");
    const size_t bytes = (size_t)ctx->n_infosets * 4 * sizeof(double);
    if (h_regret) SC_HIP(ctx, hipMemcpyAsync(h_regret, ctx->d_regret, bytes, hipMemcpyDeviceToHost, ctx->stream));
    if (h_strategy) SC_HIP(ctx, hipMemcpyAsync(h_strategy, ctx->d_strat, bytes, hipMemcpyDeviceToHost, ctx->stream));
    if (h_local) SC_HIP(ctx, hipMemcpyAsync(h_local, ctx->d_local, bytes, hipMemcpyDeviceToHost, ctx->stream));
    SC_HIP(ctx, hipStreamSynchronize(ctx->stream));
    return SCOPA_OK;
}

int32_t scopa_tables_set(scopa_ctx *ctx, const double *h_regret, const double *h_strategy, const double *h_local) {
    if (!ctx) return SCOPA_EINVAL;
    SC_REQUIRE(ctx, ctx->has_deal, SCOPA_ESTATE, "scopa_tables_set: no deal set");
    const size_t bytes = (size_t)ctx->n_infosets * 4 * sizeof(double);
    if (h_regret) SC_HIP(ctx, hipMemcpyAsync(ctx->d_regret, h_regret, bytes, hipMemcpyHostToDevice, ctx->stream));
    if (h_strategy) SC_HIP(ctx, hipMemcpyAsync(ctx->d_strat, h_strategy, bytes, hipMemcpyHostToDevice, ctx->stream));
    if (h_local) SC_HIP(ctx, hipMemcpyAsync(ctx->d_local, h_local, bytes, hipMemcpyHostToDevice, ctx->stream));
    SC_HIP(ctx, hipStreamSynchronize(ctx->stream));
    ctx->sigcdf_valid = false;
    return SCOPA_OK;
}

int32_t scopa_sdcfr_policy_get(scopa_ctx *ctx, float *h_policy, uint64_t *h_thr) {
    if (!ctx || (!h_policy && !h_thr)) return SCOPA_EINVAL;
    SC_REQUIRE(ctx, ctx->d_sdpol != nullptr, SCOPA_ESTATE, "scopa_sdcfr_policy_get: no policy-table launch yet");
    if (h_policy) SC_HIP(ctx, hipMemcpyAsync(h_policy, ctx->d_sdpol, (size_t)kDecision * 4 * sizeof(float), hipMemcpyDeviceToHost, ctx->stream));
    if (h_thr) SC_HIP(ctx, hipMemcpyAsync(h_thr, reinterpret_cast<const float4 *>(ctx->d_sdpol) + kDecision, (size_t)kDecision * 3 * sizeof(uint64_t),
                                          hipMemcpyDeviceToHost, ctx->stream));
    SC_HIP(ctx, hipStreamSynchronize(ctx->stream));
    return SCOPA_OK;
}

int32_t scopa_visited_get(scopa_ctx *ctx, uint32_t *h_seq) {
    if (!ctx || !h_seq) return SCOPA_EINVAL;
    SC_REQUIRE(ctx, ctx->has_deal, SCOPA_ESTATE, "scopa_visited_get: no deal set");
    SC_HIP(ctx, hipMemcpyAsync(h_seq, ctx->d_visit, (size_t)ctx->n_infosets * sizeof(uint32_t), hipMemcpyDeviceToHost, ctx->stream));
    SC_HIP(ctx, hipStreamSynchronize(ctx->stream));
    return SCOPA_OK;
}

int32_t scopa_counters(scopa_ctx *ctx, uint64_t *decision_visits, uint64_t *terminal_visits) {
    if (!ctx) return SCOPA_EINVAL;
    static_assert(sizeof(unsigned long long) == 8, "counter layout");
    std::vector<unsigned long long> h(8 + 2 * 1024);
    SC_HIP(ctx, hipMemcpyAsync(h.data(), ctx->d_counters, h.size() * sizeof(unsigned long long), hipMemcpyDeviceToHost, ctx->stream));
    SC_HIP(ctx, hipStreamSynchronize(ctx->stream));
    unsigned long long d = h[0], t = h[1];
    for (int w = 0; w < 1024; w++) { d += h[8 + 2 * w]; t += h[9 + 2 * w]; }
    if (decision_visits) *decision_visits = d;
    if (terminal_visits) *terminal_visits = t;
    return SCOPA_OK;
}

int32_t scopa_prof_device(scopa_ctx *ctx, int64_t *launches, double *kernel_ms) {
    if (!ctx) return SCOPA_EINVAL;
    SC_HIP(ctx, hipStreamSynchronize(ctx->stream));
    const int64_t n = ctx->d_clock ? (ctx->prof_launches < scopa::kClockSamples ? ctx->prof_launches : scopa::kClockSamples) : 0;
    unsigned long long ticks = 0;
    if (n > 0) {
        std::vector<unsigned long long> h((size_t)n * scopa::kClockStride);
        SC_HIP(ctx, hipMemcpy(h.data(), ctx->d_clock, h.size() * sizeof(unsigned long long), hipMemcpyDeviceToHost));
        double ph[3] = {0.0, 0.0, 0.0}, sp[4] = {0.0, 0.0, 0.0, 0.0};
        long long wgs = 0, launches_seen = 0;
        for (int64_t s = 0; s < n; s++) {
            unsigned long long t0 = ~0ull, t1 = 0ull, late = 0ull, longest = 0ull;
            for (int w = 0; w < ctx->clock_grid[s]; w++) {
                const unsigned long long *q = &h[(size_t)s * scopa::kClockStride + 4 * w];
                t0 = q[0] < t0 ? q[0] : t0; t1 = q[3] > t1 ? q[3] : t1;
                for (int k = 0; k < 3; k++) ph[k] += (double)(q[k + 1] - q[k]);
                wgs++;
            }
            for (int w = 0; w < ctx->clock_grid[s]; w++) {
                const unsigned long long *q = &h[(size_t)s * scopa::kClockStride + 4 * w];
                sp[0] += (double)(q[0] - t0);
                late = q[0] - t0 > late ? q[0] - t0 : late;
                longest = q[3] - q[0] > longest ? q[3] - q[0] : longest;
            }
            if (ctx->clock_grid[s]) { sp[1] += (double)late; sp[2] += (double)longest; launches_seen++; }
            if (t1 > t0) ticks += t1 - t0;
        }
        for (int k = 0; k < 3; k++) ctx->prof_phase_us[k] = wgs ? ph[k] * 1e-2 / (double)wgs : 0.0;
        ctx->prof_spread_us[0] = wgs ? sp[0] * 1e-2 / (double)wgs : 0.0;
        ctx->prof_spread_us[1] = launches_seen ? sp[1] * 1e-2 / (double)launches_seen : 0.0;
        ctx->prof_spread_us[2] = launches_seen ? sp[2] * 1e-2 / (double)launches_seen : 0.0;
    }
    if (launches) *launches = n;
    if (kernel_ms) *kernel_ms = (double)ticks * 1e-5;
    return SCOPA_OK;
}

int32_t scopa_prof_phases(scopa_ctx *ctx, double out_us[3]) {
    if (!ctx || !out_us) return SCOPA_EINVAL;
    for (int k = 0; k < 3; k++) out_us[k] = ctx->prof_phase_us[k];
    return SCOPA_OK;
}

int32_t scopa_debug_clock_dump(scopa_ctx *ctx, unsigned long long *out, int32_t n, int32_t max_grid) {
    if (!ctx || !out || n <= 0 || !ctx->d_clock) return SCOPA_EINVAL;
    SC_HIP(ctx, hipStreamSynchronize(ctx->stream));
    const int64_t have = ctx->prof_launches < scopa::kClockSamples ? ctx->prof_launches : scopa::kClockSamples;
    if (have < n) return SCOPA_ESTATE;
    int grid = 0;
    for (int32_t s = 0; s < n; s++) {
        const int64_t slot = (ctx->prof_launches - 1 - s) % scopa::kClockSamples;
        grid = ctx->clock_grid[slot];
        if (grid <= 0 || grid > max_grid) return SCOPA_ELIMIT;
        SC_HIP(ctx, hipMemcpy(out + (size_t)s * max_grid * 4, ctx->d_clock + (size_t)slot * scopa::kClockStride, (size_t)grid * 4 * sizeof(unsigned long long), hipMemcpyDeviceToHost));
    }
    return grid;
}

int32_t scopa_prof_spread(scopa_ctx *ctx, double out_us[3]) {
    if (!ctx || !out_us) return SCOPA_EINVAL;
    for (int k = 0; k < 3; k++) out_us[k] = ctx->prof_spread_us[k];
    return SCOPA_OK;
}

int32_t scopa_prof_enable(scopa_ctx *ctx, int32_t stride) {
    if (!ctx || stride < 0) return SCOPA_EINVAL;
    SC_HIP(ctx, hipStreamSynchronize(ctx->stream));
    ctx->prof_on = stride != 0;
    ctx->prof_stride = stride > 0 ? stride : 1;
    ctx->prof_tick = 0;
    ctx->ev_used = 0;
    ctx->prof_launches = 0;
    ctx->prof_ms = 0.0;
    if (ctx->prof_on) scopa::prof_pool_fill(ctx);
    if (ctx->prof_on && !ctx->d_clock)
        SC_HIP(ctx, hipMalloc(&ctx->d_clock, (size_t)scopa::kClockSamples * scopa::kClockStride * sizeof(unsigned long long)));
    return SCOPA_OK;
}

int32_t scopa_prof_read(scopa_ctx *ctx, int64_t *launches, double *kernel_ms) {
    if (!ctx) return SCOPA_EINVAL;
    SC_HIP(ctx, hipStreamSynchronize(ctx->stream));
    for (size_t i = 0; i + 1 < ctx->ev_used; i += 2) {
        float ms = 0.f;
        if (hipEventElapsedTime(&ms, ctx->ev_pool[i], ctx->ev_pool[i + 1]) == hipSuccess) ctx->prof_ms += ms;
    }
    ctx->ev_used = 0;
    if (launches) *launches = ctx->prof_launches;
    if (kernel_ms) *kernel_ms = ctx->prof_ms;
    return SCOPA_OK;
}

}
```

scopa_amd/csrc/scopa_mccfr.hip:

```cpp
#include <hip/hip_ext.h>

#include "scopa_ctx.h"
#include "scopa_p2p.h"
#include "scopa_philox.h"

using namespace scopa;

namespace {

__device__ __forceinline__ void mc_sigma(const double *R, int n, double *sigma) {
    double pos[4];
#pragma unroll
    for (int i = 0; i < 4; i++) pos[i] = (i < n && R[i] > 0.0) ? R[i] : 0.0;
    double s = pos[0];
#pragma unroll
    for (int i = 1; i < 4; i++) if (i < n) s += pos[i];
#pragma unroll
    for (int i = 0; i < 4; i++) sigma[i] = i < n ? (s == 0.0 ? 1.0 / (double)n : pos[i] / s) : 0.0;
}

__device__ __forceinline__ void choice_cdf(const double *sigma, int n, uint32_t *thr) {
    double cdf[4];
    double c = sigma[0];
    cdf[0] = c;
#pragma unroll
    for (int i = 1; i < 4; i++) { if (i < n) c += sigma[i]; cdf[i] = c; }
    const double last = c;
#pragma unroll
    for (int i = 0; i < 4; i++) thr[i] = i < n ? (uint32_t)ceil((cdf[i] / last) * 2147483648.0) : 0xFFFFFFFFu;
}
__device__ __forceinline__ void row_store(double *__restrict__ row, const double *sg, const uint32_t *thr) {
    double2 *out = reinterpret_cast<double2 *>(row);
    out[0] = make_double2(sg[0], sg[1]);
    out[1] = make_double2(sg[2], sg[3]);
    out[2] = make_double2(__longlong_as_double((long long)(((unsigned long long)thr[1] << 32) | thr[0])),
                          __longlong_as_double((long long)(((unsigned long long)thr[3] << 32) | thr[2])));
}
__device__ __forceinline__ void choice_cdf_f64(const double *sigma, int n, double *cdf) {
    double c = sigma[0];
    cdf[0] = c;
    for (int i = 1; i < n; i++) { c += sigma[i]; cdf[i] = c; }
    const double last = cdf[n - 1];
    for (int i = 0; i < 4; i++) cdf[i] = i < n ? cdf[i] / last : 2.0;
}

__host__ __device__ constexpr int ntl_at(int trav, int d) { return trav == 0 ? (d + 1) >> 1 : d >> 1; }
__host__ __device__ constexpr int task_nodes(int trav, int d) {
    return ntl_at(trav, d) == 0 ? 1 : ntl_at(trav, d) == 1 ? 5 : ntl_at(trav, d) == 2 ? 20 : 60;
}

constexpr int kRow = 6;
constexpr int kUpd = 26;
constexpr unsigned int kPairDecisionVisits = (1 + 5 + 5 + 20 + 20 + 60 + 60 + 120) + (1 + 1 + 5 + 5 + 20 + 20 + 60 + 60), kPairTerminalVisits = 120 + 120;
static_assert(kPairDecisionVisits == 463, "291 + 172");

}

__global__ void __launch_bounds__(256)
k_mccfr_prepare(const uint64_t *__restrict__ g_key, const double *__restrict__ g_regret, double *__restrict__ g_sigcdf, int n_infosets) {
    const int r = blockIdx.x * blockDim.x + threadIdx.x;
    if (r >= n_infosets) return;
    const int n = (int)((g_key[r] >> 1) & 7);
    double R[4], sg[4];
    uint32_t thr[4];
    for (int c = 0; c < 4; c++) R[c] = g_regret[r * 4 + c];
    mc_sigma(R, n, sg);
    choice_cdf(sg, n, thr);
    row_store(g_sigcdf + r * kRow, sg, thr);
}

constexpr int kIdentSlot = 166;
struct WaveScratch {
    uint32_t npk[168];
    int8_t p6[128];
    uint32_t kdraw[64][4];
};
static_assert(sizeof(WaveScratch) % 16 == 0, "WaveScratch must keep 16-byte alignment");

__device__ __forceinline__ void wave_lds_sync() {
    __builtin_amdgcn_fence(__ATOMIC_RELEASE, "wavefront");
    __builtin_amdgcn_s_waitcnt(0xc07f);
    __builtin_amdgcn_wave_barrier();
    __builtin_amdgcn_fence(__ATOMIC_ACQUIRE, "wavefront");
}

__device__ __forceinline__ uint32_t lds_addr(const void *p) { return (uint32_t)(uintptr_t)(__attribute__((address_space(3))) const void *)p; }
__device__ __forceinline__ uint32_t lds_read_u32(uint32_t a) { return *(__attribute__((address_space(3))) const uint32_t *)(uintptr_t)a; }
__device__ __forceinline__ int lds_read_i8(uint32_t a) { return *(__attribute__((address_space(3))) const int8_t *)(uintptr_t)a; }
__device__ __forceinline__ double lds_read_f64(uint32_t a) { return *(__attribute__((address_space(3))) const double *)(uintptr_t)a; }
typedef uint32_t u32x4 __attribute__((ext_vector_type(4)));
__device__ __forceinline__ uint4 lds_read_u4(uint32_t a) {
    const u32x4 v = *(__attribute__((address_space(3))) const u32x4 *)(uintptr_t)a;
    return make_uint4(v.x, v.y, v.z, v.w);
}
__device__ __forceinline__ void lds_write_u4(uint32_t a, uint32_t x, uint32_t y, uint32_t z, uint32_t w) {
    *(__attribute__((address_space(3))) u32x4 *)(uintptr_t)a = u32x4{x, y, z, w};
}

constexpr int kLaneSlotVecs = 15;
constexpr int kStaticLds = 64 + kLaneSlotVecs * 1024;
constexpr int kStaticLdsMulti = kStaticLds;

template <int NP>
__device__ __forceinline__ void draw_pairs(uint32_t wsb, int lane, const uint32_t (&b)[NP], uint32_t iteration, uint32_t seed_lo, uint32_t seed_hi) {
    const int trav = lane < 44 ? 0 : 1, p = trav ? lane - 44 : lane;
    philox_out x[NP];
#pragma unroll
    for (int i = 0; i < NP; i++) x[i] = philox4x32_10((uint32_t)p, b[i], iteration, (uint32_t)trav, seed_lo, seed_hi);
#pragma unroll
    for (int i = 0; i < NP; i++)
        lds_write_u4(wsb + (uint32_t)(i * sizeof(WaveScratch) + offsetof(WaveScratch, kdraw)) + 16u * (uint32_t)lane, x[i].x0 >> 1, x[i].x1 >> 1, x[i].x2 >> 1, x[i].x3 >> 1);
    wave_lds_sync();
}

struct NodeRegs {
    uint32_t pk;
};

__host__ __device__ constexpr int npk_offset(int d) { return d == 0 ? 0 : d == 1 ? 2 : d == 2 ? 8 : d == 3 ? 18 : d == 4 ? 43 : 86; }
__host__ __device__ constexpr int npk_slot(int trav, int d, int j) { return npk_offset(d) + (trav ? task_nodes(0, d) : 0) + j; }
static_assert(npk_offset(1) == task_nodes(0, 0) + task_nodes(1, 0) && npk_offset(2) == npk_offset(1) + task_nodes(0, 1) + task_nodes(1, 1) &&
              npk_offset(3) == npk_offset(2) + task_nodes(0, 2) + task_nodes(1, 2) && npk_offset(4) == npk_offset(3) + task_nodes(0, 3) + task_nodes(1, 3) &&
              npk_offset(4) + task_nodes(0, 4) + task_nodes(1, 4) <= npk_offset(5) && npk_offset(5) + task_nodes(0, 5) + task_nodes(1, 5) == kIdentSlot,
              "record slots of plies 0..5 tile WaveScratch::npk");

constexpr int kLvLeaf = 7, kLvUpd = 9;
struct LaneTabRow { uint4 v[kLaneSlotVecs]; };

template <int D, int ROUND>
__device__ __forceinline__ void lane_slot_build(LaneTabRow &row, int lane) {
    constexpr int S = D + ROUND;
    constexpr int c0 = task_nodes(0, D), c1 = task_nodes(1, D);
    const int t = lane + 64 * ROUND;
    const bool valid = t < c0 + c1;
    const int trav = t < c0 ? 0 : 1;
    const int j = valid ? (trav ? t - c0 : t) : 0;
    const bool is_trav = (D & 1) == trav;
    const int ntl = trav == 0 ? (D + 1) >> 1 : D >> 1;
    uint32_t plane4 = 0u, amask = valid ? ~0u : 0u, aforce = 0u;
    if constexpr (D > 0) {
        constexpr int pd = D > 0 ? D - 1 : 0, pn = 4 - (pd >> 1);
        const bool p_trav = (pd & 1) == trav;
        int pj = j, br = 0;
        if (p_trav) { pj = j / (pn + 1); br = j - pj * (pn + 1); }
        if (valid) plane4 = 4u * (uint32_t)((trav ? task_nodes(0, pd) : 0) + pj);
        if (valid && p_trav && br > 0) { amask = 0u; aforce = (uint32_t)(br - 1); }
    }
    const int blk = (ntl == 0 ? 0 : ntl == 1 ? 1 : ntl == 2 ? 4 : 14) + (j >> 1);
    const uint32_t kword = valid ? (uint32_t)(offsetof(WaveScratch, kdraw) + 16 * ((trav ? 44 : 0) + blk) + 4 * ((j & 1) * 2 + (is_trav ? 1 : 0)))
                                 : (uint32_t)offsetof(WaveScratch, kdraw);
    row.v[S] = make_uint4(plane4, amask, aforce, kword);
}

__device__ __forceinline__ void upd_build(LaneTabRow &row, int x) {
    const uint32_t ident = (uint32_t)(offsetof(WaveScratch, npk) + 4 * kIdentSlot);
    uint32_t rec[5] = {ident, ident, ident, ident, ident}, am[5] = {24u, 24u, 24u, 24u, 24u}, af[5] = {0u, 0u, 0u, 0u, 0u};
    uint32_t own = ident, nX = 1u, p6o[4] = {(uint32_t)offsetof(WaveScratch, p6), (uint32_t)offsetof(WaveScratch, p6), (uint32_t)offsetof(WaveScratch, p6), (uint32_t)offsetof(WaveScratch, p6)};
    if (x < 2 * kUpd) {
        const int trav = x < kUpd ? 0 : 1, xx = trav ? x - kUpd : x;
        const int m = xx == 0 ? 0 : xx < 6 ? 1 : 2;
        int j = xx - (m == 0 ? 0 : m == 1 ? 1 : 6);
        const int d = 2 * m + trav;
        nX = (uint32_t)(4 - m);
        const int stride = m == 0 ? 12 : m == 1 ? 3 : 1;
        const int base = m == 0 ? 0 : m == 1 ? j * 12 : j * 3;
        for (int c = 0; c < 4; c++) p6o[c] = (uint32_t)(offsetof(WaveScratch, p6) + trav * 60 + base + ((c < (int)nX ? c : (int)nX - 1) + 1) * stride);
        own = (uint32_t)(offsetof(WaveScratch, npk) + 4 * npk_slot(trav, d, j));
        for (int c = d; c > 0; c--) {
            const int pd = c - 1, pn = 4 - (pd >> 1);
            int forced = 0;
            if ((pd & 1) == trav) { const int pj = j / (pn + 1), br = j - pj * (pn + 1); forced = br; j = pj; }
            rec[pd] = (uint32_t)(offsetof(WaveScratch, npk) + 4 * npk_slot(trav, pd, j));
            if (forced) { am[pd] = 0u; af[pd] = 8u * (uint32_t)(forced - 1); }
        }
    }
    row.v[kLvUpd + 0] = make_uint4(rec[0], rec[1], rec[2], rec[3]);
    row.v[kLvUpd + 1] = make_uint4(rec[4], own, nX, 0u);
    row.v[kLvUpd + 2] = make_uint4(p6o[0], p6o[1], p6o[2], p6o[3]);
    row.v[kLvUpd + 3] = make_uint4(am[0], am[1], am[2], am[3]);
    row.v[kLvUpd + 4] = make_uint4(am[4], af[0], af[1], af[2]);
    row.v[kLvUpd + 5] = make_uint4(af[3], af[4], 0u, 0u);
}

struct WalkEnv {
    uint32_t wsb;
    uint32_t tab;
    const uint16_t *s_inf;
    const int8_t *s_pay;
    const double *s_sigcdf;
    double *s_dR;
    uint8_t *s_seen;
    unsigned int *s_cnt;
};

template <int D, int NP>
__device__ __forceinline__ void ply_step(const WalkEnv &e, int lane, NodeRegs (&st)[NP]) {
    constexpr int n = 4 - (D >> 1);
    constexpr int c0 = task_nodes(0, D), c1 = task_nodes(1, D);
    constexpr int NR = c0 + c1 > 64 ? 2 : 1;
    struct Pre {
        int idx, In;
        uint32_t k, thr0, thr1, thr2;
    };
    Pre g[NP][NR];
    uint4 sl[NR];
#pragma unroll
    for (int r = 0; r < NR; r++) sl[r] = lds_read_u4(e.tab + 1024u * (uint32_t)(D + r));
#pragma unroll
    for (int i = 0; i < NP; i++)
#pragma unroll
        for (int r = 0; r < NR; r++) {
            Pre &q = g[i][r];
            q.idx = 0;
            if constexpr (D > 0) {
                constexpr int pn = 4 - ((D > 0 ? D - 1 : 0) >> 1);
                const uint32_t ppk = (uint32_t)__builtin_amdgcn_ds_bpermute((int)sl[r].x, (int)st[i].pk);
                const uint32_t act = ((ppk >> 21) & sl[r].y) | sl[r].z;
                q.idx = (int)((ppk & 1023u) * pn + act);
            }
            q.In = e.s_inf[level_offset(D) + q.idx];
            q.k = lds_read_u32(e.wsb + sl[r].w + (uint32_t)(i * sizeof(WaveScratch)));
            const uint32_t *thr = reinterpret_cast<const uint32_t *>(e.s_sigcdf + q.In * kRow + 4);
            q.thr0 = thr[0];
            q.thr1 = n > 2 ? thr[1] : 0xFFFFFFFFu;
            q.thr2 = n > 3 ? thr[2] : 0xFFFFFFFFu;
        }
#pragma unroll
    for (int i = 0; i < NP; i++)
#pragma unroll
        for (int r = 0; r < NR; r++) {
            const Pre &q = g[i][r];
            const int t = 64 * r + lane;
            if (t < c0 + c1) {
                const int a = (q.thr0 <= q.k) + (q.thr1 <= q.k) + (q.thr2 <= q.k);
                if ((D & 1) == (t < c0 ? 0 : 1)) atomicAdd(&e.s_cnt[q.In], 1u);
                else if (e.s_seen) e.s_seen[q.In] = 1;
                const uint32_t pk = (uint32_t)q.idx | ((uint32_t)q.In << 10) | ((uint32_t)a << 21);
                *(__attribute__((address_space(3))) uint32_t *)(uintptr_t)(e.wsb + (uint32_t)(i * sizeof(WaveScratch) + offsetof(WaveScratch, npk) + 4 * npk_offset(D)) + 4u * (uint32_t)t) = pk;
                if constexpr (D < 5) st[i].pk = pk;
            }
        }
    if constexpr (D == 5) wave_lds_sync();
}

#ifdef SCOPA_WALK_STAMPS
__device__ unsigned long long g_walk_stamps[16];
__device__ unsigned long long g_wave_clocks[3 * 16];
__device__ unsigned long long g_wave_phases[4 * 16];
#define WALK_STAMP(i) do { const unsigned long long now_ = clock64(); if (blockIdx.x == 0 && threadIdx.x == 0) { g_walk_stamps[i] += now_ - t_prev_; } t_prev_ = now_; } while (0)
#else
#define WALK_STAMP(i) do { } while (0)
#endif

template <int NP>
__device__ __forceinline__ void walk_pairs(const WalkEnv &e, int lane, const uint32_t (&b)[NP], uint32_t iteration, uint32_t seed_lo,
                                           uint32_t seed_hi, unsigned int &my_pairs) {
#ifdef SCOPA_WALK_STAMPS
    const unsigned long long w_start_ = wall_clock64();
    unsigned long long t_prev_ = clock64();
#endif
    draw_pairs<NP>(e.wsb, lane, b, iteration, seed_lo, seed_hi);
    WALK_STAMP(0);
    NodeRegs st[NP];
#pragma unroll
    for (int i = 0; i < NP; i++) st[i].pk = 0u;
    ply_step<0, NP>(e, lane, st); WALK_STAMP(1);
    ply_step<1, NP>(e, lane, st); WALK_STAMP(2);
    ply_step<2, NP>(e, lane, st); WALK_STAMP(3);
    ply_step<3, NP>(e, lane, st); WALK_STAMP(4);
    ply_step<4, NP>(e, lane, st); WALK_STAMP(5);
    ply_step<5, NP>(e, lane, st); WALK_STAMP(6);
    my_pairs += NP;
    {
        uint4 lf[2];
#pragma unroll
        for (int q = 0; q < 2; q++) lf[q] = lds_read_u4(e.tab + 1024u * (uint32_t)(kLvLeaf + q));
        uint32_t ppk[NP][2];
#pragma unroll
        for (int i = 0; i < NP; i++)
#pragma unroll
            for (int q = 0; q < 2; q++) ppk[i][q] = lds_read_u32(e.wsb + lf[q].x + (uint32_t)(i * sizeof(WaveScratch)));
        int I6[NP][2], I7[NP][2], pay[NP][2];
#pragma unroll
        for (int i = 0; i < NP; i++)
#pragma unroll
            for (int q = 0; q < 2; q++) {
                const uint32_t act = ((ppk[i][q] >> 21) & lf[q].y) | lf[q].z;
                const int idx6 = (int)((ppk[i][q] & 1023u) * 2 + act);
                I6[i][q] = e.s_inf[level_offset(6) + idx6];
                I7[i][q] = e.s_inf[level_offset(7) + idx6];
                pay[i][q] = e.s_pay[idx6];
            }
#pragma unroll
        for (int i = 0; i < NP; i++)
#pragma unroll
            for (int q = 0; q < 2; q++) {
                const int t = lane + 64 * q;
                if (t < 2 * 60) {
                    const int trv = t < 60 ? 0 : 1;
                    if (e.s_seen) e.s_seen[trv == 0 ? I7[i][q] : I6[i][q]] = 1;
                    atomicAdd(&e.s_cnt[trv == 0 ? I6[i][q] : I7[i][q]], 1u);
                    *(__attribute__((address_space(3))) int8_t *)(uintptr_t)(e.wsb + (uint32_t)(i * sizeof(WaveScratch) + offsetof(WaveScratch, p6)) + (uint32_t)t) =
                        (int8_t)(trv == 0 ? pay[i][q] : -pay[i][q]);
                }
            }
    }
    wave_lds_sync();
    WALK_STAMP(7);
    if (lane < 2 * kUpd) {
        const bool trav1 = lane >= kUpd;
        uint4 u[6];
#pragma unroll
        for (int q = 0; q < 6; q++) u[q] = lds_read_u4(e.tab + 1024u * (uint32_t)(kLvUpd + q));
        const uint32_t ro[5] = {u[0].x, u[0].y, u[0].z, u[0].w, u[1].x}, own = u[1].y;
        const int nX = (int)u[1].z;
        const uint32_t p6o[4] = {u[2].x, u[2].y, u[2].z, u[2].w};
        const uint32_t am[5] = {u[3].x, u[3].y, u[3].z, u[3].w, u[4].x}, af[5] = {u[4].y, u[4].z, u[4].w, u[5].x, u[5].y};
        uint32_t rec[NP][5];
        int IX[NP], pv[NP][4];
#pragma unroll
        for (int i = 0; i < NP; i++) {
            const uint32_t wi = e.wsb + (uint32_t)(i * sizeof(WaveScratch));
#pragma unroll
            for (int q = 0; q < 5; q++) rec[i][q] = lds_read_u32(wi + ro[q]);
            IX[i] = (int)((lds_read_u32(wi + own) >> 10) & 2047u);
#pragma unroll
            for (int c = 0; c < 4; c++) pv[i][c] = lds_read_i8(wi + p6o[c]);
        }
        double fq[NP][5], sg[NP][4];
        const uint32_t sig = lds_addr(e.s_sigcdf);
#pragma unroll
        for (int i = 0; i < NP; i++) {
#pragma unroll
            for (int q = 0; q < 5; q++)
                fq[i][q] = lds_read_f64(sig + ((rec[i][q] >> 10) & 2047u) * (uint32_t)(kRow * 8) + (((rec[i][q] >> 18) & am[q]) | af[q]));
            const double2 s01 = *reinterpret_cast<const double2 *>(e.s_sigcdf + IX[i] * kRow), s23 = *reinterpret_cast<const double2 *>(e.s_sigcdf + IX[i] * kRow + 2);
            sg[i][0] = s01.x; sg[i][1] = s01.y; sg[i][2] = s23.x; sg[i][3] = s23.y;
        }
#pragma unroll
        for (int i = 0; i < NP; i++) {
            const double even = (fq[i][0] * fq[i][2]) * fq[i][4], odd = fq[i][1] * fq[i][3];
            const double sX = trav1 ? odd : even, rX = trav1 ? even : odd;
            const double w = sX > 0.0 ? rX / sX : 0.0;
            double cfv[4], v = 0.0;
#pragma unroll
            for (int c = 0; c < 4; c++) {
                cfv[c] = 0.5 * (double)pv[i][c];
                const double t = fma(sg[i][c], cfv[c], v);
                v = c < nX ? t : v;
            }
#pragma unroll
            for (int c = 0; c < 4; c++) {
                const double delta = w * (cfv[c] - v);
                if (c < nX && delta != 0.0) atomicAdd(&e.s_dR[IX[i] * 4 + c], delta);
            }
        }
    }
    wave_lds_sync();
    WALK_STAMP(8);
#ifdef SCOPA_WALK_STAMPS
    if (blockIdx.x == 0 && threadIdx.x == 0) { g_walk_stamps[15] += NP; g_walk_stamps[14] += wall_clock64() - w_start_; }
#endif
}

__global__ void __launch_bounds__(64) k_lane_table(uint4 *__restrict__ g_tab) {
    const int lane = threadIdx.x;
    LaneTabRow row;
    for (int i = 0; i < kLaneSlotVecs; i++) row.v[i] = make_uint4(0u, 0u, 0u, 0u);
    lane_slot_build<0, 0>(row, lane);
    lane_slot_build<1, 0>(row, lane);
    lane_slot_build<2, 0>(row, lane);
    lane_slot_build<3, 0>(row, lane);
    lane_slot_build<4, 0>(row, lane);
    lane_slot_build<5, 0>(row, lane);
    lane_slot_build<5, 1>(row, lane);
    for (int q = 0; q < 2; q++) {
        const int t = lane + 64 * q;
        const bool on = t < 2 * 60;
        const int tt = on ? t : 0, trv = tt < 60 ? 0 : 1, j = trv ? tt - 60 : tt;
        int pj = j, kk = 0;
        if (trv == 1) { pj = j / 3; kk = j - pj * 3; }
        row.v[kLvLeaf + q] = make_uint4((uint32_t)(offsetof(WaveScratch, npk) + 4 * (npk_offset(5) + (trv ? 60 : 0) + pj)),
                                        (trv == 1 && kk > 0) ? 0u : ~0u, (trv == 1 && kk > 0) ? (uint32_t)(kk - 1) : 0u, 0u);
    }
    upd_build(row, lane);
    for (int i = 0; i < kLaneSlotVecs; i++) g_tab[i * 64 + lane] = row.v[i];
}

__device__ __forceinline__ void wave_scratch_init(WaveScratch *ws, int n_scratch, int lane, int n_infosets) {
    if (lane == 0)
        for (int i = 0; i < n_scratch; i++) ws[i].npk[kIdentSlot] = (uint32_t)n_infosets << 10;
}

__device__ __forceinline__ int group_of(unsigned int b) { return (int)((b >> 3) % kDeltaGroups); }

__global__ void __launch_bounds__(1024)
k_mccfr_traverse(const uint16_t *__restrict__ g_infoset, const int8_t *__restrict__ g_payoff,
                 const double *__restrict__ g_sigcdf, double *__restrict__ g_groups,
                 int n_infosets, uint32_t seed_lo, uint32_t seed_hi, uint32_t iteration, uint32_t b0, uint32_t nb,
                 unsigned long long *__restrict__ g_wg_counts, uint32_t *__restrict__ g_visit, unsigned long long *__restrict__ g_clock,
                 const uint4 *__restrict__ g_lane_tab, const uint32_t *__restrict__ g_iter, uint32_t track_seen) {
    extern __shared__ __align__(16) unsigned char smem[];
    __shared__ unsigned int s_vis[2];
    if (g_iter) iteration = *g_iter;
    __shared__ uint32_t s_next[1];
    __shared__ uint32_t s_slice[1];
    __shared__ uint4 s_lane_tab[kLaneSlotVecs * 64];
    const unsigned long long t_start = wall_clock64();
#ifdef SCOPA_WALK_STAMPS
    const unsigned long long c_entry_ = clock64();
#endif
    const int I = n_infosets;
    double *s_sigcdf = reinterpret_cast<double *>(smem);
    double *s_dR = s_sigcdf + (size_t)(I + 1) * kRow;
    WaveScratch *s_wave = reinterpret_cast<WaveScratch *>(s_dR + (size_t)I * 4);
    unsigned int *s_cnt = reinterpret_cast<unsigned int *>(s_wave + 2 * (blockDim.x >> 6));
    uint16_t *s_inf = reinterpret_cast<uint16_t *>(reinterpret_cast<unsigned char *>(s_cnt) + (((size_t)I * 4 + 15) & ~(size_t)15));
    int8_t *s_pay = reinterpret_cast<int8_t *>(s_inf + 1656);
    uint8_t *s_seen = reinterpret_cast<uint8_t *>(s_pay + kTerminal);

    const int tid = threadIdx.x, lane = tid & 63, wave = tid >> 6, n_waves = blockDim.x >> 6, nthr = blockDim.x;
    if (tid < 2) s_vis[tid] = 0u;
    const uint4 lane_piece = tid < kLaneSlotVecs * 64 ? g_lane_tab[tid] : make_uint4(0u, 0u, 0u, 0u);
    if (tid == 0) {
        s_slice[0] = 0u;
        const uint32_t per_wg = (nb + gridDim.x - 1) / gridDim.x, W = blockDim.x >> 6;
        const uint32_t first = blockIdx.x * per_wg, count = first < nb ? (nb - first < per_wg ? nb - first : per_wg) : 0u;
        s_next[0] = count >= 2 * W ? 2 * W : W;
    }
    const uint32_t *gi = reinterpret_cast<const uint32_t *>(g_infoset), *gp = reinterpret_cast<const uint32_t *>(g_payoff);
    {
        constexpr int kSig = 5;
        const double2 *g2 = reinterpret_cast<const double2 *>(g_sigcdf);
        double2 *s2 = reinterpret_cast<double2 *>(s_sigcdf);
        double2 v[kSig];
#pragma unroll
        for (int j = 0; j < kSig; j++) {
            const int idx = tid + j * nthr;
            v[j] = idx < I * 3 ? g2[idx] : make_double2(0.0, 0.0);
        }
        const uint32_t wi = tid < kDecision / 2 ? gi[tid] : 0u;
        const uint32_t wp = tid < kTerminal / 4 ? gp[tid] : 0u;
        const uint16_t last_inf = g_infoset[kDecision - 1];
        for (int i = tid; i < I * 2; i += nthr) reinterpret_cast<double2 *>(s_dR)[i] = make_double2(0.0, 0.0);
        for (int r = tid; r < I; r += nthr) s_cnt[r] = 0u;
        if (track_seen) for (int r = tid; r < I; r += nthr) s_seen[r] = 0;
        if (tid < 4) s_sigcdf[(size_t)I * kRow + tid] = 1.0;
#pragma unroll
        for (int j = 0; j < kSig; j++) {
            const int idx = tid + j * nthr;
            if (idx < I * 3) s2[idx] = v[j];
        }
        for (int idx = tid + kSig * nthr; idx < I * 3; idx += nthr) s2[idx] = g2[idx];
        if (tid < kLaneSlotVecs * 64) s_lane_tab[tid] = lane_piece;
        if (tid < kDecision / 2) reinterpret_cast<uint32_t *>(s_inf)[tid] = wi;
        if (tid == 0) s_inf[kDecision - 1] = last_inf;
        if (tid < kTerminal / 4) reinterpret_cast<uint32_t *>(s_pay)[tid] = wp;
    }
    for (int i = tid + nthr; i < kLaneSlotVecs * 64; i += nthr) s_lane_tab[i] = g_lane_tab[i];
    for (int i = tid + nthr; i < kDecision / 2; i += nthr) reinterpret_cast<uint32_t *>(s_inf)[i] = gi[i];
    for (int i = tid + nthr; i < kTerminal / 4; i += nthr) reinterpret_cast<uint32_t *>(s_pay)[i] = gp[i];
    __syncthreads();
    const unsigned long long t_pro = wall_clock64();
#ifdef SCOPA_WALK_STAMPS
    const unsigned long long c_barrier_ = clock64();
    unsigned long long c_loop0_ = 0, c_loop1_ = 0;
#endif

    WaveScratch *ws = s_wave + 2 * wave;
    wave_scratch_init(ws, 2, lane, I);
    WalkEnv env;
    env.wsb = lds_addr(ws); env.tab = lds_addr(s_lane_tab) + 16u * (uint32_t)lane;
    env.s_inf = s_inf; env.s_pay = s_pay; env.s_sigcdf = s_sigcdf; env.s_dR = s_dR; env.s_seen = track_seen ? s_seen : nullptr; env.s_cnt = s_cnt;
    unsigned int my_pairs = 0;
    {
#ifdef SCOPA_WALK_STAMPS
        const unsigned long long loop_start_ = clock64();
        c_loop0_ = loop_start_;
#endif
        const uint32_t per_wg = (nb + gridDim.x - 1) / gridDim.x;
        const uint32_t first = blockIdx.x * per_wg, count = first < nb ? (nb - first < per_wg ? nb - first : per_wg) : 0u;
        const uint32_t W = (uint32_t)n_waves;
        const bool start_two = count >= 2 * W;
        uint32_t c = start_two ? 2 * (uint32_t)wave : (uint32_t)wave, g = start_two ? 2u : 1u;
        for (;;) {
            if (g == 2 && c + 1 < count) {
                const uint32_t two[2] = {b0 + first + c, b0 + first + c + 1};
                walk_pairs<2>(env, lane, two, iteration, seed_lo, seed_hi, my_pairs);
            } else if (c < count) {
                const uint32_t one[1] = {b0 + first + c};
                walk_pairs<1>(env, lane, one, iteration, seed_lo, seed_hi, my_pairs);
            }
            if (count <= W || c + g >= count) break;
            g = count - c > 4 * W ? 2u : 1u;
            uint32_t got = 0;
            if (lane == 0) got = atomicAdd(s_next, g);
            c = (uint32_t)__builtin_amdgcn_readfirstlane((int)got);
            if (c >= count) break;
        }
#ifdef SCOPA_WALK_STAMPS
        c_loop1_ = clock64();
        if (lane == 0 && (blockIdx.x == 0 || blockIdx.x == 100)) g_wave_clocks[(blockIdx.x == 0 ? 0 : 16) + wave] += c_loop1_ - loop_start_;
        if (lane == 0 && blockIdx.x == 0) { unsigned int hw; asm volatile("s_getreg_b32 %0, hwreg(HW_REG_HW_ID)" : "=s"(hw)); g_wave_clocks[32 + wave] = hw; }
#endif
    }
    {
        uint32_t sl = 0;
        if (lane == 0) sl = atomicAdd(s_slice, 1u);
        sl = (uint32_t)__builtin_amdgcn_readfirstlane((int)sl);
        const int W = n_waves;
        if ((int)sl < W - W / 4) {
            const int per = (I + W - 1) / W, r0 = (W - 1 - (int)sl) * per, r1 = r0 + per < I ? r0 + per : I;
            double *tab = g_groups + (size_t)group_of(blockIdx.x) * kDeltaTable;
            for (int r = r0 + lane; r < r1; r += 64) {
#pragma unroll
                for (int k = 0; k < 4; k++) {
                    const double v = __longlong_as_double((long long)atomicExch(reinterpret_cast<unsigned long long *>(&s_dR[r * 4 + k]), 0ull));
                    if (v != 0.0) atomicAdd(&tab[group_cell(k, r)], v);
                }
                const unsigned int c = atomicExch(&s_cnt[r], 0u);
                if (c != 0u) { atomicAdd(&tab[group_cell(4, r)], (double)c); if (track_seen) s_seen[r] = 1; }
            }
        }
    }
    __syncthreads();

    const unsigned long long t_walk = wall_clock64();
    {
        const bool first0 = track_seen && tid < I && (s_seen[tid] || s_cnt[tid]) && g_visit[tid] == 0u;
        const bool first1 = track_seen && tid + nthr < I && (s_seen[tid + nthr] || s_cnt[tid + nthr]) && g_visit[tid + nthr] == 0u;
        double *tab = g_groups + (size_t)group_of(blockIdx.x) * kDeltaTable;
        for (int r = tid; r < I; r += nthr) {
            const double2 a = reinterpret_cast<const double2 *>(s_dR)[r * 2], b = reinterpret_cast<const double2 *>(s_dR)[r * 2 + 1];
            const unsigned int c = s_cnt[r];
            if (a.x != 0.0) atomicAdd(&tab[group_cell(0, r)], a.x);
            if (a.y != 0.0) atomicAdd(&tab[group_cell(1, r)], a.y);
            if (b.x != 0.0) atomicAdd(&tab[group_cell(2, r)], b.x);
            if (b.y != 0.0) atomicAdd(&tab[group_cell(3, r)], b.y);
            if (c != 0u) atomicAdd(&tab[group_cell(4, r)], (double)c);
        }
        if (first0) g_visit[tid] = 0x40000000u + (uint32_t)tid;
        if (first1) g_visit[tid + nthr] = 0x40000000u + (uint32_t)(tid + nthr);
        if (track_seen)
            for (int r = tid + 2 * nthr; r < I; r += nthr)
                if ((s_seen[r] || s_cnt[r]) && g_visit[r] == 0u) g_visit[r] = 0x40000000u + (uint32_t)r;
    }
    if (lane == 0) { atomicAdd(&s_vis[0], my_pairs * kPairDecisionVisits); atomicAdd(&s_vis[1], my_pairs * kPairTerminalVisits); }
    __syncthreads();
    if (tid < 2) atomicAdd(&g_wg_counts[blockIdx.x * 2 + tid], (unsigned long long)s_vis[tid]);
#ifdef SCOPA_WALK_STAMPS
    if (blockIdx.x == 0 && (tid & 63) == 0) {
        g_wave_phases[(tid >> 6)] += c_barrier_ - c_entry_; g_wave_phases[16 + (tid >> 6)] += c_loop0_ - c_barrier_;
        g_wave_phases[32 + (tid >> 6)] += c_loop1_ - c_loop0_; g_wave_phases[48 + (tid >> 6)] += clock64() - c_loop1_;
    }
#endif
    if (g_clock && tid == 0) {
        g_clock[blockIdx.x * 4] = t_start; g_clock[blockIdx.x * 4 + 1] = t_pro; g_clock[blockIdx.x * 4 + 2] = t_walk; g_clock[blockIdx.x * 4 + 3] = wall_clock64();
    }
}

__global__ void __launch_bounds__(1024)
k_mccfr_multi(const uint16_t *__restrict__ g_infoset, const int8_t *__restrict__ g_payoff, const uint64_t *__restrict__ g_key,
              double *__restrict__ g_regret, double *__restrict__ g_strat, const int32_t *__restrict__ g_meta, uint32_t *__restrict__ g_visit,
              unsigned long long *__restrict__ g_counters, uint32_t seed_lo, uint32_t seed_hi, uint32_t iter0, uint32_t n_iters,
              uint32_t batch, const uint4 *__restrict__ g_lane_tab) {
    extern __shared__ __align__(16) unsigned char smem[];
    __shared__ unsigned int s_vis[2];
    __shared__ uint4 s_lane_tab[kLaneSlotVecs * 64];
    for (int i = threadIdx.x; i < kLaneSlotVecs * 64; i += blockDim.x) s_lane_tab[i] = g_lane_tab[i];
    {
        const size_t deal = blockIdx.x;
        g_infoset += deal * kDecision; g_payoff += deal * kTerminal; g_key += deal * kDecision; g_regret += deal * kDecision * 4;
        g_strat += deal * kDecision * 4; g_meta += deal * 8; g_visit += deal * kDecision; g_counters += deal * 8;
    }
    const int I = g_meta[0];
    double *s_sigcdf = reinterpret_cast<double *>(smem);
    double *s_R = s_sigcdf + (size_t)(I + 1) * kRow;
    WaveScratch *s_wave = reinterpret_cast<WaveScratch *>(s_R + (size_t)I * 4);
    unsigned int *s_cnt = reinterpret_cast<unsigned int *>(s_wave + (blockDim.x >> 6));
    uint16_t *s_inf = reinterpret_cast<uint16_t *>(reinterpret_cast<unsigned char *>(s_cnt) + (((size_t)I * 4 + 15) & ~(size_t)15));
    int8_t *s_pay = reinterpret_cast<int8_t *>(s_inf + 1656);
    uint8_t *s_seen = reinterpret_cast<uint8_t *>(s_pay + kTerminal);
    const int tid = threadIdx.x, lane = tid & 63, wave = tid >> 6, n_waves = blockDim.x >> 6;
    if (tid < 2) s_vis[tid] = 0u;
    for (int i = tid; i < I * 4; i += blockDim.x) s_R[i] = g_regret[i];
    for (int r = tid; r < I; r += blockDim.x) { s_cnt[r] = 0u; s_seen[r] = 0; }
    for (int i = tid; i < kDecision; i += blockDim.x) s_inf[i] = g_infoset[i];
    for (int i = tid; i < kTerminal; i += blockDim.x) s_pay[i] = g_payoff[i];
    if (tid < 4) s_sigcdf[(size_t)I * kRow + tid] = 1.0;
    __syncthreads();
    WaveScratch *ws = s_wave + wave;
    wave_scratch_init(ws, 1, lane, I);
    WalkEnv env;
    env.wsb = lds_addr(ws); env.tab = lds_addr(s_lane_tab) + 16u * (uint32_t)lane;
    env.s_inf = s_inf; env.s_pay = s_pay; env.s_sigcdf = s_sigcdf; env.s_dR = s_R; env.s_seen = s_seen; env.s_cnt = s_cnt;
    unsigned int my_pairs = 0;
    for (uint32_t it = 0; it < n_iters; it++) {
        for (int r = tid; r < I; r += blockDim.x) {
            const int n = (int)((g_key[r] >> 1) & 7);
            double sg[4];
            uint32_t thr[4];
            mc_sigma(s_R + r * 4, n, sg);
            choice_cdf(sg, n, thr);
            for (int c = 0; c < 4; c++) { s_sigcdf[r * kRow + c] = sg[c]; reinterpret_cast<uint32_t *>(s_sigcdf + r * kRow + 4)[c] = thr[c]; }
        }
        __syncthreads();
        for (uint32_t pg = (uint32_t)wave; pg < batch; pg += (uint32_t)n_waves) {
            const uint32_t one[1] = {pg};
            walk_pairs<1>(env, lane, one, iter0 + it, seed_lo, seed_hi, my_pairs);
        }
        __syncthreads();
        for (int r = tid; r < I; r += blockDim.x) {
            const unsigned int c = s_cnt[r];
            if (c) {
                s_seen[r] = 1;
                const int n = (int)((g_key[r] >> 1) & 7);
                for (int k = 0; k < n; k++) g_strat[r * 4 + k] += (double)c * s_sigcdf[r * kRow + k];
                s_cnt[r] = 0u;
            }
        }
        __syncthreads();
    }
    for (int i = tid; i < I * 4; i += blockDim.x) g_regret[i] = s_R[i];
    for (int r = tid; r < I; r += blockDim.x) if (s_seen[r] && g_visit[r] == 0u) g_visit[r] = 0x40000000u + (uint32_t)r;
    if (lane == 0) { atomicAdd(&s_vis[0], my_pairs * kPairDecisionVisits); atomicAdd(&s_vis[1], my_pairs * kPairTerminalVisits); }
    __syncthreads();
    if (tid < 2) g_counters[tid] += s_vis[tid];
}

__global__ void __launch_bounds__(256)
k_mccfr_fold(double *__restrict__ g_groups, double *__restrict__ g_delta, int n_infosets) {
    const int r = blockIdx.x * blockDim.x + threadIdx.x;
    if (r >= n_infosets) return;
    double d[5] = {0.0, 0.0, 0.0, 0.0, 0.0};
    for (int g = 0; g < kDeltaGroups; g++)
        for (int k = 0; k < 5; k++) {
            double *q = g_groups + (size_t)g * kDeltaTable + group_cell(k, r);
            d[k] += *q;
            *q = 0.0;
        }
    for (int k = 0; k < 5; k++) g_delta[r * 5 + k] += d[k];
}

struct ApplyRow { double R[4], S[4], sg[4]; int n; };

__device__ __forceinline__ ApplyRow apply_row_load(int r, const uint64_t *__restrict__ g_key, const double *__restrict__ g_regret,
                                                   const double *__restrict__ g_strat, const double *__restrict__ g_sigcdf) {
    ApplyRow a;
    const double2 r0 = *reinterpret_cast<const double2 *>(g_regret + r * 4), r1 = *reinterpret_cast<const double2 *>(g_regret + r * 4 + 2);
    const double2 s0 = *reinterpret_cast<const double2 *>(g_strat + r * 4), s1 = *reinterpret_cast<const double2 *>(g_strat + r * 4 + 2);
    const double2 g0 = *reinterpret_cast<const double2 *>(g_sigcdf + r * kRow), g1 = *reinterpret_cast<const double2 *>(g_sigcdf + r * kRow + 2);
    a.n = (int)((g_key[r] >> 1) & 7);
    a.R[0] = r0.x; a.R[1] = r0.y; a.R[2] = r1.x; a.R[3] = r1.y;
    a.S[0] = s0.x; a.S[1] = s0.y; a.S[2] = s1.x; a.S[3] = s1.y;
    a.sg[0] = g0.x; a.sg[1] = g0.y; a.sg[2] = g1.x; a.sg[3] = g1.y;
    return a;
}

__device__ __forceinline__ void apply_row_store(int r, ApplyRow &a, const double (&d)[5], double *__restrict__ g_regret,
                                                double *__restrict__ g_strat, double *__restrict__ g_sigcdf) {
#pragma unroll
    for (int c = 0; c < 4; c++)
        if (c < a.n) { a.R[c] += d[c]; a.S[c] += d[4] * a.sg[c]; }
    *reinterpret_cast<double2 *>(g_regret + r * 4) = make_double2(a.R[0], a.R[1]);
    *reinterpret_cast<double2 *>(g_regret + r * 4 + 2) = make_double2(a.R[2], a.R[3]);
    *reinterpret_cast<double2 *>(g_strat + r * 4) = make_double2(a.S[0], a.S[1]);
    *reinterpret_cast<double2 *>(g_strat + r * 4 + 2) = make_double2(a.S[2], a.S[3]);
    double sg[4];
    uint32_t thr[4];
    mc_sigma(a.R, a.n, sg);
    choice_cdf(sg, a.n, thr);
    row_store(g_sigcdf + r * kRow, sg, thr);
}

__device__ __forceinline__ double groups_cell_take(double *__restrict__ g_groups, int r, int k) {
    double v[kDeltaGroups];
#pragma unroll
    for (int g = 0; g < kDeltaGroups; g++) v[g] = g_groups[(size_t)g * kDeltaTable + group_cell(k, r)];
    double d = 0.0;
#pragma unroll
    for (int g = 0; g < kDeltaGroups; g++) {
        d += v[g];
        if (v[g] != 0.0) g_groups[(size_t)g * kDeltaTable + group_cell(k, r)] = 0.0;
    }
    return d;
}

constexpr int kApplyLanes = 8, kApplyThreads = 64;

__global__ void __launch_bounds__(kApplyThreads)
k_mccfr_apply_groups(const uint64_t *__restrict__ g_key, double *__restrict__ g_regret, double *__restrict__ g_strat,
                     double *__restrict__ g_groups, int n_infosets, double *__restrict__ g_sigcdf, uint32_t *__restrict__ g_iter) {
    if (g_iter && blockIdx.x == 0 && threadIdx.x == 0) *g_iter += 1u;
    const int lane = threadIdx.x & 63, k = lane & (kApplyLanes - 1);
    const int r = (int)(blockIdx.x * blockDim.x + threadIdx.x) / kApplyLanes;
    const bool valid = r < n_infosets;
    ApplyRow a{};
    if (valid && k == 0) a = apply_row_load(r, g_key, g_regret, g_strat, g_sigcdf);
    const double mine = (valid && k < 5) ? groups_cell_take(g_groups, r, k) : 0.0;
    double d[5];
#pragma unroll
    for (int j = 0; j < 5; j++) d[j] = __shfl(mine, (lane & ~(kApplyLanes - 1)) + j);
    if (valid && k == 0) apply_row_store(r, a, d, g_regret, g_strat, g_sigcdf);
}

__global__ void __launch_bounds__(64)
k_mccfr_apply(const uint64_t *__restrict__ g_key, double *__restrict__ g_regret, double *__restrict__ g_strat,
              double *__restrict__ g_delta, int n_infosets, double *__restrict__ g_sigcdf) {
    const int r = blockIdx.x * blockDim.x + threadIdx.x;
    if (r >= n_infosets) return;
    double d[5];
    for (int k = 0; k < 5; k++) d[k] = g_delta[r * 5 + k];
    ApplyRow a = apply_row_load(r, g_key, g_regret, g_strat, g_sigcdf);
    for (int k = 0; k < 5; k++) g_delta[r * 5 + k] = 0.0;
    apply_row_store(r, a, d, g_regret, g_strat, g_sigcdf);
}

__global__ void __launch_bounds__(64)
k_mccfr_exchange_apply(scopa::P2PArgs xa, double *__restrict__ g_groups, const uint64_t *__restrict__ g_key, double *__restrict__ g_regret,
                       double *__restrict__ g_strat, double *__restrict__ g_sigcdf, int n_infosets) {
    __shared__ double xch[4][scopa::kP2PMaxWorld][5];
    const int rl = threadIdx.x >> 4, q = threadIdx.x & 15;
    const int r = blockIdx.x * 4 + rl;
    const bool valid = r < n_infosets;
    const double mine = (valid && q < 5) ? groups_cell_take(g_groups, r, q) : 0.0;
    double d[5];
#pragma unroll
    for (int j = 0; j < 5; j++) d[j] = __shfl(mine, (int)(threadIdx.x & ~15u) + j);
    ApplyRow a{};
    if (valid && q == 0) a = apply_row_load(r, g_key, g_regret, g_strat, g_sigcdf);
    scopa::p2p_exchange_wave4(xa, r, valid, q, d, xch[rl]);
    if (valid && q == 0) apply_row_store(r, a, d, g_regret, g_strat, g_sigcdf);
}

namespace {
struct ReplayWalk {
    double *R, *S;
    const uint16_t *inf;
    const int8_t *pay;
    uint32_t *visit;
    const double *uniforms;
    long long upos, n_uniforms;
    uint32_t seq;
    unsigned long long dvis, tvis;
};

template <int D, int TRAV>
__device__ __forceinline__ double replay_rec(ReplayWalk &w, int idx, double reach_opp, double samp_trav) {
    if constexpr (D == kPlies) {
        w.tvis++;
        const int p0 = w.pay[idx];
        return 0.5 * (double)(TRAV == 0 ? p0 : -p0);
    } else {
        constexpr int n = 4 - (D >> 1);
        constexpr bool is_trav = (D & 1) == TRAV;
        w.dvis++;
        const int I = w.inf[level_offset(D) + idx];
        if (w.visit[I] == 0u) w.visit[I] = ++w.seq;
        double R[4], sigma[4], cdf[4];
        for (int c = 0; c < 4; c++) R[c] = w.R[I * 4 + c];
        mc_sigma(R, n, sigma);
        choice_cdf_f64(sigma, n, cdf);
        const double u = w.upos < w.n_uniforms ? w.uniforms[w.upos] : 0.0;
        w.upos++;
        int a = (cdf[0] <= u) + (cdf[1] <= u) + (cdf[2] <= u) + (cdf[3] <= u);
        a = a < n - 1 ? a : n - 1;
        double sa = sigma[0];
        for (int i = 1; i < n; i++) sa = a == i ? sigma[i] : sa;
        if constexpr (!is_trav) {
            return replay_rec<D + 1, TRAV>(w, idx * n + a, reach_opp * sa, samp_trav);
        } else {
            const double util = replay_rec<D + 1, TRAV>(w, idx * n + a, reach_opp, samp_trav * sa);
            double cfv[4] = {0.0, 0.0, 0.0, 0.0};
#pragma unroll 1
            for (int i = 0; i < n; i++)
                cfv[i] = replay_rec<D + 1, TRAV>(w, idx * n + i, reach_opp, samp_trav * sigma[i]);
            double v = 0.0;
            for (int i = 0; i < n; i++) v = fma(sigma[i], cfv[i], v);
            const double wt = samp_trav > 0.0 ? reach_opp / samp_trav : 0.0;
            for (int i = 0; i < n; i++) {
                w.R[I * 4 + i] += wt * (cfv[i] - v);
                w.S[I * 4 + i] += 1.0 * sigma[i];
            }
            return util;
        }
    }
}
}

__global__ void __launch_bounds__(256)
k_mccfr_replay(const uint16_t *__restrict__ g_infoset, const int8_t *__restrict__ g_payoff, const uint64_t *__restrict__ g_key,
               double *__restrict__ g_regret, double *__restrict__ g_strat, const double *__restrict__ uniforms,
               long long n_uniforms, int n_iters, unsigned long long *__restrict__ g_counters, long long *__restrict__ consumed,
               uint32_t *__restrict__ g_visit, int32_t *__restrict__ g_meta) {
    extern __shared__ __align__(16) unsigned char smem[];
    __shared__ uint16_t s_inf[1656];
    __shared__ int8_t s_pay[kTerminal];
    __shared__ uint32_t s_visit[kDecision];
    const int tid = threadIdx.x, I = g_meta[0], cells = I * 4;
    double *R = reinterpret_cast<double *>(smem), *S = R + cells;
    for (int i = tid; i < cells; i += blockDim.x) { R[i] = g_regret[i]; S[i] = g_strat[i]; }
    for (int i = tid; i < kDecision; i += blockDim.x) s_inf[i] = g_infoset[i];
    for (int i = tid; i < kTerminal; i += blockDim.x) s_pay[i] = g_payoff[i];
    for (int i = tid; i < I; i += blockDim.x) s_visit[i] = g_visit[i];
    __syncthreads();
    if (tid == 0) {
        ReplayWalk w;
        w.R = R; w.S = S; w.inf = s_inf; w.pay = s_pay; w.visit = s_visit; w.uniforms = uniforms; w.upos = 0; w.n_uniforms = n_uniforms;
        w.seq = (uint32_t)g_meta[1]; w.dvis = 0; w.tvis = 0;
#pragma unroll 1
        for (int it = 0; it < n_iters; it++) {
            replay_rec<0, 0>(w, 0, 1.0, 1.0);
            replay_rec<0, 1>(w, 0, 1.0, 1.0);
        }
        g_counters[0] += w.dvis;
        g_counters[1] += w.tvis;
        g_meta[1] = (int32_t)w.seq;
        *consumed = w.upos;
    }
    __syncthreads();
    for (int i = tid; i < cells; i += blockDim.x) { g_regret[i] = R[i]; g_strat[i] = S[i]; }
    for (int i = tid; i < I; i += blockDim.x) g_visit[i] = s_visit[i];
}


static size_t traverse_lds_bytes(int n_infosets, int waves) {
    size_t b = ((size_t)(n_infosets + 1) * kRow + (size_t)n_infosets * 4) * sizeof(double);
    b += (size_t)waves * 2 * sizeof(WaveScratch);
    b += (((size_t)n_infosets * 4 + 15) & ~(size_t)15);
    b += 1656 * 2 + 576;
    b += (size_t)n_infosets;
    return (b + 15) & ~(size_t)15;
}

static int32_t ensure_lane_table(scopa_ctx *ctx) {
    if (ctx->d_lane_tab) return SCOPA_OK;
    SC_HIP(ctx, hipMalloc(&ctx->d_lane_tab, (size_t)kLaneSlotVecs * 64 * sizeof(uint4)));
    hipLaunchKernelGGL(k_lane_table, dim3(1), dim3(64), 0, ctx->stream, (uint4 *)ctx->d_lane_tab);
    SC_HIP(ctx, hipGetLastError());
    return SCOPA_OK;
}

struct TraverseGeom { int threads; size_t lds; uint32_t grid; };

static int32_t refresh_all_seen(scopa_ctx *ctx, bool now) {
    if (ctx->mccfr_all_seen) return SCOPA_OK;
    if (!now && ++ctx->mccfr_seen_wait < 16u) return SCOPA_OK;
    ctx->mccfr_seen_wait = 0;
    uint32_t h[kDecision];
    SC_HIP(ctx, hipMemcpyAsync(h, ctx->d_visit, (size_t)ctx->n_infosets * sizeof(uint32_t), hipMemcpyDeviceToHost, ctx->stream));
    SC_HIP(ctx, hipStreamSynchronize(ctx->stream));
    bool all = true;
    for (int r = 0; r < ctx->n_infosets; r++) all = all && h[r] != 0u;
    ctx->mccfr_all_seen = all;
    return SCOPA_OK;
}

static int32_t prepare_traverse(scopa_ctx *ctx, uint32_t nb, TraverseGeom *g) {
    int waves = 16;
    while (waves > 1 && traverse_lds_bytes(ctx->n_infosets, waves) + kStaticLds > (size_t)ctx->lds_limit) waves = waves > 2 ? waves - 2 : 1;
    g->threads = waves * 64;
    g->lds = traverse_lds_bytes(ctx->n_infosets, waves);
    SC_REQUIRE(ctx, g->lds + kStaticLds <= (size_t)ctx->lds_limit, SCOPA_ELIMIT, "mccfr traverse: infoset tables do not fit in LDS");
    SC_LDS_ATTR(ctx, scopa::kLdsTraverse, k_mccfr_traverse, ctx->lds_limit - kStaticLds);
    const uint32_t n_passes = (nb + waves - 1) / waves;
    g->grid = n_passes < (uint32_t)ctx->n_cus ? n_passes : (uint32_t)ctx->n_cus;
    SC_REQUIRE(ctx, g->grid <= 1024u, SCOPA_ELIMIT, "mccfr traverse: more than 1024 compute units");
    static_assert(kClockStride >= 4 * 512, "clock sample stride");
    if (int32_t rc = ensure_lane_table(ctx)) return rc;
    if (int32_t rc = refresh_all_seen(ctx, false)) return rc;
    if (!ctx->sigcdf_valid) {
        hipLaunchKernelGGL(k_mccfr_prepare, dim3((ctx->n_infosets + 255) / 256), dim3(256), 0, ctx->stream, ctx->d_key,
                           ctx->d_regret, ctx->d_sigcdf, ctx->n_infosets);
        SC_HIP(ctx, hipGetLastError());
        ctx->sigcdf_valid = true;
    }
    return SCOPA_OK;
}

static int32_t launch_traverse(scopa_ctx *ctx, uint32_t iteration, uint32_t b0, uint32_t nb) {
    TraverseGeom g;
    if (int32_t rc = prepare_traverse(ctx, nb, &g)) return rc;
    const int threads = g.threads;
    const size_t lds = g.lds;
    const uint32_t grid = g.grid;
    hipEvent_t ev0 = nullptr, ev1 = nullptr;
    const bool sampled = prof_events(ctx, &ev0, &ev1);
    unsigned long long *clock = sampled && ctx->d_clock && grid <= 512u ? ctx->d_clock + (size_t)((ctx->prof_launches - 1) % kClockSamples) * kClockStride : nullptr;
    if (sampled) ctx->clock_grid[(ctx->prof_launches - 1) % kClockSamples] = clock ? (uint16_t)grid : (uint16_t)0;
    if (sampled)
        hipExtLaunchKernelGGL(k_mccfr_traverse, dim3(grid), dim3(threads), lds, ctx->stream, ev0, ev1, 0, ctx->d_infoset, ctx->d_payoff,
                              ctx->d_sigcdf, ctx->d_groups, ctx->n_infosets, (uint32_t)ctx->seed, (uint32_t)(ctx->seed >> 32),
                              iteration, b0, nb, ctx->d_counters + 8, ctx->d_visit, clock, (const uint4 *)ctx->d_lane_tab, (const uint32_t *)nullptr,
                              ctx->mccfr_all_seen ? 0u : 1u);
    else
        hipLaunchKernelGGL(k_mccfr_traverse, dim3(grid), dim3(threads), lds, ctx->stream, ctx->d_infoset, ctx->d_payoff,
                           ctx->d_sigcdf, ctx->d_groups, ctx->n_infosets, (uint32_t)ctx->seed, (uint32_t)(ctx->seed >> 32),
                           iteration, b0, nb, ctx->d_counters + 8, ctx->d_visit, clock, (const uint4 *)ctx->d_lane_tab, (const uint32_t *)nullptr,
                           ctx->mccfr_all_seen ? 0u : 1u);
    SC_HIP(ctx, hipGetLastError());
    return SCOPA_OK;
}

void scopa::mccfr_graphs_clear(scopa_ctx *ctx) {
    for (auto &e : ctx->mccfr_graphs) (void)hipGraphExecDestroy((hipGraphExec_t)e.exec);
    ctx->mccfr_graphs.clear();
}

static int32_t graph_for(scopa_ctx *ctx, uint32_t batch, uint32_t k, hipGraphExec_t *out) {
    const uint32_t track = ctx->mccfr_all_seen ? 0u : 1u;
    for (auto &e : ctx->mccfr_graphs)
        if (e.batch == batch && e.k == k && e.track == track) { *out = (hipGraphExec_t)e.exec; return SCOPA_OK; }
    TraverseGeom g;
    if (int32_t rc = prepare_traverse(ctx, batch, &g)) return rc;
    uint32_t *d_iter = reinterpret_cast<uint32_t *>(ctx->d_meta + 2);
    hipGraph_t graph = nullptr;
    SC_HIP(ctx, hipStreamBeginCapture(ctx->stream, hipStreamCaptureModeThreadLocal));
    for (uint32_t i = 0; i < k; i++) {
        hipLaunchKernelGGL(k_mccfr_traverse, dim3(g.grid), dim3(g.threads), g.lds, ctx->stream, ctx->d_infoset, ctx->d_payoff,
                           ctx->d_sigcdf, ctx->d_groups, ctx->n_infosets, (uint32_t)ctx->seed, (uint32_t)(ctx->seed >> 32),
                           0u, 0u, batch, ctx->d_counters + 8, ctx->d_visit, (unsigned long long *)nullptr, (const uint4 *)ctx->d_lane_tab, (const uint32_t *)d_iter, track);
        hipLaunchKernelGGL(k_mccfr_apply_groups, dim3((ctx->n_infosets * kApplyLanes + kApplyThreads - 1) / kApplyThreads), dim3(kApplyThreads), 0, ctx->stream, ctx->d_key,
                           ctx->d_regret, ctx->d_strat, ctx->d_groups, ctx->n_infosets, ctx->d_sigcdf, d_iter);
    }
    const hipError_t e_end = hipStreamEndCapture(ctx->stream, &graph);
    if (e_end != hipSuccess || !graph) return scopa::fail(ctx, SCOPA_EHIP, "mccfr graph: stream capture", e_end);
    hipGraphExec_t exec = nullptr;
    const hipError_t e_inst = hipGraphInstantiate(&exec, graph, nullptr, nullptr, 0);
    (void)hipGraphDestroy(graph);
    if (e_inst != hipSuccess) return scopa::fail(ctx, SCOPA_EHIP, "mccfr graph: instantiate", e_inst);
    if (ctx->mccfr_graphs.size() >= 16) { (void)hipGraphExecDestroy((hipGraphExec_t)ctx->mccfr_graphs.front().exec); ctx->mccfr_graphs.erase(ctx->mccfr_graphs.begin()); }
    ctx->mccfr_graphs.push_back({batch, k, track, (void *)exec});
    *out = exec;
    return SCOPA_OK;
}

namespace scopa {
int32_t launch_mccfr_multi(scopa_ctx *ctx, int n_deals, int max_infosets, const uint16_t *d_infoset, const int8_t *d_payoff,
                           const uint64_t *d_key, double *d_regret, double *d_strat, const int32_t *d_meta, uint32_t *d_visit,
                           unsigned long long *d_counters, uint64_t seed, uint32_t iter0, uint32_t n_iters, uint32_t batch) {
    int waves = 16;
    auto need = [&](int w) {
        size_t b = ((size_t)(max_infosets + 1) * kRow + (size_t)max_infosets * 4) * sizeof(double) + (size_t)w * sizeof(WaveScratch);
        b += (((size_t)max_infosets * 4 + 15) & ~(size_t)15) + 1656 * 2 + 576 + (size_t)max_infosets;
        return (b + 15) & ~(size_t)15;
    };
    while (waves > 1 && need(waves) + kStaticLdsMulti > (size_t)ctx->lds_limit) waves -= 2;
    SC_REQUIRE(ctx, need(waves) + kStaticLdsMulti <= (size_t)ctx->lds_limit, SCOPA_ELIMIT, "mccfr multi: infoset tables do not fit in LDS");
    SC_LDS_ATTR(ctx, scopa::kLdsMulti, k_mccfr_multi, ctx->lds_limit - kStaticLdsMulti);
    if (int32_t rc = ensure_lane_table(ctx)) return rc;
    hipLaunchKernelGGL(k_mccfr_multi, dim3(n_deals), dim3(waves * 64), need(waves), ctx->stream, d_infoset, d_payoff, d_key, d_regret, d_strat,
                       d_meta, d_visit, d_counters, (uint32_t)seed, (uint32_t)(seed >> 32), iter0, n_iters, batch, (const uint4 *)ctx->d_lane_tab);
    SC_HIP(ctx, hipGetLastError());
    return SCOPA_OK;
}
}

extern "C" {

int32_t scopa_mccfr_seed(scopa_ctx *ctx, uint64_t seed) {
    if (!ctx) return SCOPA_EINVAL;
    if (seed != ctx->seed) scopa::mccfr_graphs_clear(ctx);
    ctx->seed = seed;
    return SCOPA_OK;
}

int32_t scopa_mccfr_traverse(scopa_ctx *ctx, uint32_t iteration, uint32_t b0, uint32_t nb) {
    if (!ctx) return SCOPA_EINVAL;
    SC_REQUIRE(ctx, ctx->has_deal, SCOPA_ESTATE, "scopa_mccfr_traverse: no deal set");
    SC_REQUIRE(ctx, nb <= (1u << 30), SCOPA_EINVAL, "scopa_mccfr_traverse: batch too large");
    if (nb == 0) return SCOPA_OK;
    SC_HIP(ctx, hipSetDevice(ctx->device));
    scopa::Range r("scopa mccfr traverse (split path)");
    const int32_t rc = launch_traverse(ctx, iteration, b0, nb);
    if (rc != SCOPA_OK) return rc;
    hipLaunchKernelGGL(k_mccfr_fold, dim3((ctx->n_infosets + 255) / 256), dim3(256), 0, ctx->stream, ctx->d_groups, ctx->d_delta, ctx->n_infosets);
    SC_HIP(ctx, hipGetLastError());
    return SCOPA_OK;
}

int32_t scopa_mccfr_delta_buffer(scopa_ctx *ctx, void **d_delta, size_t *bytes) {
    if (!ctx || !d_delta || !bytes) return SCOPA_EINVAL;
    SC_REQUIRE(ctx, ctx->has_deal, SCOPA_ESTATE, "scopa_mccfr_delta_buffer: no deal set");
    *d_delta = ctx->d_delta;
    *bytes = (size_t)ctx->n_infosets * 5 * sizeof(double);
    return SCOPA_OK;
}

int32_t scopa_mccfr_bind_delta(scopa_ctx *ctx, void *d_buf, size_t bytes) {
    if (!ctx) return SCOPA_EINVAL;
    SC_REQUIRE(ctx, ctx->has_deal, SCOPA_ESTATE, "scopa_mccfr_bind_delta: no deal set");
    const size_t need = (size_t)ctx->n_infosets * 5 * sizeof(double);
    if (d_buf) {
        SC_REQUIRE(ctx, bytes >= need, SCOPA_EINVAL, "scopa_mccfr_bind_delta: buffer smaller than n_infosets*5 float64");
        SC_REQUIRE(ctx, ((uintptr_t)d_buf & 15) == 0, SCOPA_EINVAL, "scopa_mccfr_bind_delta: buffer must be 16-byte aligned");
        ctx->d_delta = static_cast<double *>(d_buf);
    } else {
        ctx->d_delta = ctx->d_delta_own;
    }
    SC_HIP(ctx, hipSetDevice(ctx->device));
    SC_HIP(ctx, hipMemsetAsync(ctx->d_delta, 0, need, ctx->stream));
    return SCOPA_OK;
}

int32_t scopa_mccfr_delta_get(scopa_ctx *ctx, double *h_delta) {
    if (!ctx || !h_delta) return SCOPA_EINVAL;
    SC_REQUIRE(ctx, ctx->has_deal, SCOPA_ESTATE, "scopa_mccfr_delta_get: no deal set");
    SC_HIP(ctx, hipMemcpyAsync(h_delta, ctx->d_delta, (size_t)ctx->n_infosets * 5 * sizeof(double), hipMemcpyDeviceToHost, ctx->stream));
    SC_HIP(ctx, hipStreamSynchronize(ctx->stream));
    return SCOPA_OK;
}

int32_t scopa_mccfr_delta_set(scopa_ctx *ctx, const double *h_delta) {
    if (!ctx || !h_delta) return SCOPA_EINVAL;
    SC_REQUIRE(ctx, ctx->has_deal, SCOPA_ESTATE, "scopa_mccfr_delta_set: no deal set");
    SC_HIP(ctx, hipMemcpyAsync(ctx->d_delta, h_delta, (size_t)ctx->n_infosets * 5 * sizeof(double), hipMemcpyHostToDevice, ctx->stream));
    SC_HIP(ctx, hipStreamSynchronize(ctx->stream));
    return SCOPA_OK;
}

int32_t scopa_mccfr_apply(scopa_ctx *ctx) {
    if (!ctx) return SCOPA_EINVAL;
    SC_REQUIRE(ctx, ctx->has_deal, SCOPA_ESTATE, "scopa_mccfr_apply: no deal set");
    SC_HIP(ctx, hipSetDevice(ctx->device));
    scopa::Range r("scopa mccfr apply (split path)");
    if (!ctx->sigcdf_valid) {
        hipLaunchKernelGGL(k_mccfr_prepare, dim3((ctx->n_infosets + 255) / 256), dim3(256), 0, ctx->stream, ctx->d_key,
                           ctx->d_regret, ctx->d_sigcdf, ctx->n_infosets);
        SC_HIP(ctx, hipGetLastError());
    }
    hipLaunchKernelGGL(k_mccfr_apply, dim3((ctx->n_infosets + 63) / 64), dim3(64), 0, ctx->stream, ctx->d_key,
                       ctx->d_regret, ctx->d_strat, ctx->d_delta, ctx->n_infosets, ctx->d_sigcdf);
    SC_HIP(ctx, hipGetLastError());
    ctx->sigcdf_valid = true;
    ctx->iteration++;
    return SCOPA_OK;
}

int32_t scopa_mccfr_iteration_counter(scopa_ctx *ctx, uint32_t *iteration) {
    if (!ctx || !iteration) return SCOPA_EINVAL;
    *iteration = ctx->iteration;
    return SCOPA_OK;
}

int32_t scopa_mccfr_iterate(scopa_ctx *ctx, uint32_t batch, uint32_t n_iters) {
    if (!ctx) return SCOPA_EINVAL;
    SC_REQUIRE(ctx, ctx->has_deal, SCOPA_ESTATE, "scopa_mccfr_iterate: no deal set");
    SC_REQUIRE(ctx, batch > 0 && batch <= (1u << 30), SCOPA_EINVAL, "scopa_mccfr_iterate: bad batch");
    SC_HIP(ctx, hipSetDevice(ctx->device));
    if (ctx->mccfr_graph_mode && !ctx->prof_on && n_iters > 1) {
        TraverseGeom g;
        if (int32_t rc = prepare_traverse(ctx, batch, &g)) return rc;
        SC_HIP(ctx, hipMemsetD32Async(reinterpret_cast<hipDeviceptr_t>(ctx->d_meta + 2), (int)ctx->iteration, 1, ctx->stream));
        for (uint32_t left = n_iters; left > 0;) {
            const uint32_t k = left >= 64u ? 64u : left;
            if (int32_t rc = refresh_all_seen(ctx, true)) return rc;
            hipGraphExec_t exec = nullptr;
            if (int32_t rc = graph_for(ctx, batch, k, &exec)) return rc;
            SC_HIP(ctx, hipGraphLaunch(exec, ctx->stream));
            ctx->iteration += k;
            left -= k;
        }
        ctx->sigcdf_valid = true;
        return SCOPA_OK;
    }
    for (uint32_t it = 0; it < n_iters; it++) {
        int32_t rc;
        { scopa::Range r("scopa mccfr traverse"); rc = launch_traverse(ctx, ctx->iteration, 0, batch); }
        if (rc != SCOPA_OK) return rc;
        scopa::Range r("scopa mccfr apply");
        hipLaunchKernelGGL(k_mccfr_apply_groups, dim3((ctx->n_infosets * kApplyLanes + kApplyThreads - 1) / kApplyThreads), dim3(kApplyThreads), 0, ctx->stream, ctx->d_key,
                           ctx->d_regret, ctx->d_strat, ctx->d_groups, ctx->n_infosets, ctx->d_sigcdf, (uint32_t *)nullptr);
        SC_HIP(ctx, hipGetLastError());
        ctx->sigcdf_valid = true;
        ctx->iteration++;
    }
    return SCOPA_OK;
}

int32_t scopa_mccfr_graph_mode(scopa_ctx *ctx, int32_t on) {
    if (!ctx) return SCOPA_EINVAL;
    ctx->mccfr_graph_mode = on != 0;
    if (!on) scopa::mccfr_graphs_clear(ctx);
    return SCOPA_OK;
}

int32_t scopa_mccfr_iterate_sharded(scopa_ctx *ctx, uint32_t b0, uint32_t nb, uint32_t n_iters) {
    if (!ctx) return SCOPA_EINVAL;
    SC_REQUIRE(ctx, ctx->has_deal, SCOPA_ESTATE, "scopa_mccfr_iterate_sharded: no deal set");
    SC_REQUIRE(ctx, nb > 0 && nb <= (1u << 30), SCOPA_EINVAL, "scopa_mccfr_iterate_sharded: bad slice");
    SC_HIP(ctx, hipSetDevice(ctx->device));
    for (uint32_t it = 0; it < n_iters; it++) {
        scopa::P2PArgs xa{};
        SC_REQUIRE(ctx, scopa::p2p_next_args(ctx, &xa), SCOPA_ESTATE, "mccfr sharded iteration: peer exchange not connected");
        int32_t rc;
        { scopa::Range r("scopa mccfr traverse"); rc = launch_traverse(ctx, ctx->iteration, b0, nb); }
        if (rc != SCOPA_OK) return rc;
        scopa::Range r("scopa mccfr exchange + apply");
        hipLaunchKernelGGL(k_mccfr_exchange_apply, dim3((ctx->n_infosets + 3) / 4), dim3(64), 0, ctx->stream, xa, ctx->d_groups, ctx->d_key,
                           ctx->d_regret, ctx->d_strat, ctx->d_sigcdf, ctx->n_infosets);
        SC_HIP(ctx, hipGetLastError());
        ctx->sigcdf_valid = true;
        ctx->iteration++;
    }
    SC_HIP(ctx, hipStreamSynchronize(ctx->stream));
    return scopa::p2p_check(ctx, "scopa_mccfr_iterate_sharded");
}

int32_t scopa_mccfr_replay(scopa_ctx *ctx, int32_t n_iters, const double *h_uniforms, int64_t n_uniforms, int64_t *consumed) {
    if (!ctx || n_iters < 0 || n_uniforms < 0 || (n_uniforms > 0 && !h_uniforms)) return SCOPA_EINVAL;
    SC_REQUIRE(ctx, ctx->has_deal, SCOPA_ESTATE, "scopa_mccfr_replay: no deal set");
    SC_HIP(ctx, hipSetDevice(ctx->device));
    const size_t ubytes = (size_t)n_uniforms * sizeof(double);
    { const int32_t rc = ensure_scratch(ctx, ubytes + 64); if (rc != SCOPA_OK) return rc; }
    long long *d_consumed = reinterpret_cast<long long *>(ctx->d_scratch);
    double *d_u = ctx->d_scratch + 8;
    if (n_uniforms) SC_HIP(ctx, hipMemcpyAsync(d_u, h_uniforms, ubytes, hipMemcpyHostToDevice, ctx->stream));
    SC_LDS_ATTR(ctx, scopa::kLdsReplay, k_mccfr_replay, ctx->lds_limit - 12 * 1024);
    hipLaunchKernelGGL(k_mccfr_replay, dim3(1), dim3(256), (size_t)ctx->n_infosets * 64, ctx->stream, ctx->d_infoset, ctx->d_payoff, ctx->d_key,
                       ctx->d_regret, ctx->d_strat, d_u, (long long)n_uniforms, (int)n_iters, ctx->d_counters, d_consumed,
                       ctx->d_visit, ctx->d_meta);
    SC_HIP(ctx, hipGetLastError());
    long long used = 0;
    SC_HIP(ctx, hipMemcpyAsync(&used, d_consumed, sizeof used, hipMemcpyDeviceToHost, ctx->stream));
    SC_HIP(ctx, hipStreamSynchronize(ctx->stream));
    ctx->sigcdf_valid = false;
    if (consumed) *consumed = used;
    return SCOPA_OK;
}

}

#ifdef SCOPA_WALK_STAMPS
extern "C" int scopa_debug_wave_phases(unsigned long long *out64) {
    return hipMemcpyFromSymbol(out64, HIP_SYMBOL(g_wave_phases), sizeof(unsigned long long) * 64) == hipSuccess ? 0 : -1;
}
extern "C" int scopa_debug_wave_clocks(unsigned long long *out48) {
    return hipMemcpyFromSymbol(out48, HIP_SYMBOL(g_wave_clocks), sizeof(unsigned long long) * 48) == hipSuccess ? 0 : -1;
}
extern "C" int scopa_debug_walk_stamps(unsigned long long *out16, int reset) {
    if (hipMemcpyFromSymbol(out16, HIP_SYMBOL(g_walk_stamps), sizeof(unsigned long long) * 16) != hipSuccess) return -1;
    if (reset) { unsigned long long z[16] = {0}; if (hipMemcpyToSymbol(HIP_SYMBOL(g_walk_stamps), z, sizeof(z)) != hipSuccess) return -1; }
    return 0;
}
#endif
```

scopa_amd/csrc/scopa_tree.hip:

```cpp
#include <string.h>

#include <vector>

#include "scopa_ctx.h"

using namespace scopa;

#ifndef SCOPA_STEP_UNROLL
#define SCOPA_STEP_UNROLL 2
#endif
__global__ void __launch_bounds__(256) k_step_batch(scopa_state *__restrict__ states,
                                                     const uint8_t *__restrict__ actions, int64_t n) {
    constexpr int U = SCOPA_STEP_UNROLL;
    const int64_t stride = (int64_t)gridDim.x * blockDim.x;
    uint4 *st = reinterpret_cast<uint4 *>(states);
    for (int64_t i = (int64_t)blockIdx.x * blockDim.x + threadIdx.x; i < n; i += U * stride) {
        uint4 v[U];
        int act[U];
#pragma unroll
        for (int u = 0; u < U; u++) {
            const int64_t j = i + u * stride;
            v[u] = j < n ? st[j] : make_uint4(0u, 0u, 0u, 0u);
            act[u] = j < n ? actions[j] & 15 : 0;
        }
#pragma unroll
        for (int u = 0; u < U; u++) {
            const int64_t j = i + u * stride;
            if (j < n) {
                step_words(v[u].x, v[u].y, v[u].z, v[u].w, act[u]);
                st[j] = v[u];
            }
        }
    }
}

__device__ __forceinline__ int dfs_index(int d, int j) {
    int dfs = 0;
    for (int k = d - 1; k >= 0; k--) {
        const int n = nlegal_at(k);
        const int a = j % n;
        j /= n;
        dfs += 1 + a * subtree_size(k + 1);
    }
    return dfs;
}

__global__ void __launch_bounds__(1024) k_tree_build(const uint8_t *__restrict__ perm16, scopa_state *__restrict__ states,
                                                      uint16_t *__restrict__ infoset_of, int8_t *__restrict__ payoff,
                                                      uint64_t *__restrict__ key_of_infoset, int32_t *__restrict__ meta) {
    __shared__ uint64_t s_key[576];
    __shared__ int s_dfs[576];
    __shared__ int s_first[kDecision];
    __shared__ int s_scan[kNodes + 1];
    const int tid = threadIdx.x, nt = blockDim.x;
    {
        const size_t deal = blockIdx.x;
        perm16 += deal * 16; states += deal * kNodes; infoset_of += deal * kDecision; payoff += deal * kTerminal;
        key_of_infoset += deal * kDecision; meta += deal * 8;
    }

    for (int i = tid; i <= kNodes; i += nt) s_scan[i] = 0;
    if (tid == 0) {
        uint8_t p[16];
        for (int i = 0; i < 16; i++) p[i] = perm16[i];
        scopa_state root;
        state_init(root, p);
        states[0] = root;
    }
    __syncthreads();
    for (int d = 0; d < kPlies; d++) {
        const int n = nlegal_at(d), w1 = level_width(d + 1);
        for (int j = tid; j < w1; j += nt) {
            scopa_state s = states[level_offset(d) + j / n];
            const int action = nib(s.hand[s.step & 1], j % n);
            step(s, action);
            states[level_offset(d + 1) + j] = s;
        }
        __syncthreads();
    }
    for (int j = tid; j < kTerminal; j += nt) {
        int r0, r1;
        rewards_x2(states[level_offset(8) + j], r0, r1);
        payoff[j] = (int8_t)r0;
    }
    for (int d = 0; d < kPlies; d++) {
        const int w = level_width(d), off = level_offset(d);
        for (int j = tid; j < w; j += nt) { s_key[j] = infoset_key(states[off + j], d & 1); s_dfs[j] = dfs_index(d, j); }
        __syncthreads();
        for (int j = tid; j < w; j += nt) {
            const uint64_t k = s_key[j];
            int first = s_dfs[j];
            for (int m = 0; m < w; m++) {
                if (s_key[m] == k) { first = s_dfs[m]; break; }
            }
            s_first[off + j] = first;
            if (first == s_dfs[j]) s_scan[first + 1] = 1;
        }
        __syncthreads();
    }
    {
        __shared__ int s_wsum[16];
        const int lane = tid & 63, wave = tid >> 6, base = tid * 4;
        int v[4], sum = 0;
        for (int q = 0; q < 4; q++) { v[q] = base + q <= kNodes ? s_scan[base + q] : 0; sum += v[q]; }
        int x = sum;
        for (int o = 1; o < 64; o <<= 1) { const int y = __shfl_up(x, o); if (lane >= o) x += y; }
        if (lane == 63) s_wsum[wave] = x;
        __syncthreads();
        if (tid == 0) {
            int acc = 0;
            for (int w = 0; w < 16; w++) { const int t = s_wsum[w]; s_wsum[w] = acc; acc += t; }
            meta[0] = acc;
        }
        __syncthreads();
        int run = x - sum + s_wsum[wave];
        for (int q = 0; q < 4; q++) { run += v[q]; if (base + q <= kNodes) s_scan[base + q] = run; }
    }
    __syncthreads();
    for (int d = 0; d < kPlies; d++) {
        const int w = level_width(d), off = level_offset(d);
        for (int j = tid; j < w; j += nt) {
            const int first = s_first[off + j];
            const int id = s_scan[first];
            infoset_of[off + j] = (uint16_t)id;
            if (first == dfs_index(d, j)) key_of_infoset[id] = infoset_key(states[off + j], d & 1);
        }
    }
}

__global__ void k_tables_reset(double *regret, double *strat, double *local, const uint64_t *key_of_infoset,
                               const int32_t *meta) {
    {
        const size_t deal = blockIdx.y;
        regret += deal * kDecision * 4; strat += deal * kDecision * 4; local += deal * kDecision * 4;
        key_of_infoset += deal * kDecision; meta += deal * 8;
    }
    const int I = meta[0];
    for (int i = blockIdx.x * blockDim.x + threadIdx.x; i < kDecision * 4; i += gridDim.x * blockDim.x) {
        const int row = i >> 2, col = i & 3;
        regret[i] = 0.0;
        strat[i] = 0.0;
        double l = 0.0;
        if (row < I) {
            const int n = (int)((key_of_infoset[row] >> 1) & 7);
            if (col < n) l = 1.0 / (double)n;
        }
        local[i] = l;
    }
}

extern "C" {

int32_t scopa_step_batch(scopa_ctx *ctx, scopa_state *d_states, const uint8_t *d_actions, int64_t n) {
    if (!ctx || n < 0 || (n > 0 && (!d_states || !d_actions))) return SCOPA_EINVAL;
    if (n == 0) return SCOPA_OK;
    SC_REQUIRE(ctx, ((uintptr_t)d_states & 15) == 0, SCOPA_EINVAL, "scopa_step_batch: states must be 16-byte aligned");
    SC_HIP(ctx, hipSetDevice(ctx->device));
    int64_t blocks = (n + 255) / 256;
#ifndef SCOPA_STEP_BLOCKS_PER_CU
#define SCOPA_STEP_BLOCKS_PER_CU 128
#endif
    const int64_t cap = (int64_t)ctx->n_cus * SCOPA_STEP_BLOCKS_PER_CU;
    if (blocks > cap) blocks = cap;
    hipLaunchKernelGGL(k_step_batch, dim3((unsigned)blocks), dim3(256), 0, ctx->stream, d_states, d_actions, n);
    SC_HIP(ctx, hipGetLastError());
    return SCOPA_OK;
}

int32_t scopa_step_batch_host(scopa_ctx *ctx, scopa_state *h_states, const uint8_t *h_actions, int64_t n) {
    if (!ctx || n < 0 || (n > 0 && (!h_states || !h_actions))) return SCOPA_EINVAL;
    if (n == 0) return SCOPA_OK;
    SC_HIP(ctx, hipSetDevice(ctx->device));
    scopa_state *d_s = nullptr;
    uint8_t *d_a = nullptr;
    SC_HIP(ctx, hipMalloc(&d_s, (size_t)n * sizeof(scopa_state)));
    hipError_t e = hipMalloc(&d_a, (size_t)n);
    if (e != hipSuccess) { (void)hipFree(d_s); return fail(ctx, SCOPA_EHIP, "hipMalloc(actions)", e); }
    int32_t rc = SCOPA_OK;
    if ((e = hipMemcpyAsync(d_s, h_states, (size_t)n * sizeof(scopa_state), hipMemcpyHostToDevice, ctx->stream)) != hipSuccess ||
        (e = hipMemcpyAsync(d_a, h_actions, (size_t)n, hipMemcpyHostToDevice, ctx->stream)) != hipSuccess)
        rc = fail(ctx, SCOPA_EHIP, "hipMemcpyAsync(H2D)", e);
    if (rc == SCOPA_OK) rc = scopa_step_batch(ctx, d_s, d_a, n);
    if (rc == SCOPA_OK && (e = hipMemcpyAsync(h_states, d_s, (size_t)n * sizeof(scopa_state), hipMemcpyDeviceToHost, ctx->stream)) != hipSuccess)
        rc = fail(ctx, SCOPA_EHIP, "hipMemcpyAsync(D2H)", e);
    e = hipStreamSynchronize(ctx->stream);
    if (rc == SCOPA_OK && e != hipSuccess) rc = fail(ctx, SCOPA_EHIP, "hipStreamSynchronize", e);
    (void)hipFree(d_s);
    (void)hipFree(d_a);
    return rc;
}

int32_t scopa_tables_reset(scopa_ctx *ctx) {
    if (!ctx) return SCOPA_EINVAL;
    SC_REQUIRE(ctx, ctx->has_deal, SCOPA_ESTATE, "scopa_tables_reset: no deal set");
    SC_HIP(ctx, hipSetDevice(ctx->device));
    hipLaunchKernelGGL(k_tables_reset, dim3(8), dim3(1024), 0, ctx->stream, ctx->d_regret, ctx->d_strat, ctx->d_local,
                       ctx->d_key, ctx->d_meta);
    SC_HIP(ctx, hipGetLastError());
    SC_HIP(ctx, hipMemsetAsync(ctx->d_visit, 0, sizeof(uint32_t) * kDecision, ctx->stream));
    SC_HIP(ctx, hipMemsetAsync(ctx->d_meta + 1, 0, sizeof(int32_t), ctx->stream));
    SC_HIP(ctx, hipMemsetAsync(ctx->d_delta, 0, (size_t)(ctx->d_delta == ctx->d_delta_own ? kDecision : ctx->n_infosets) * 5 * sizeof(double), ctx->stream));
    ctx->iteration = 0;
    ctx->sigcdf_valid = false;
    ctx->mccfr_all_seen = false;
    ctx->mccfr_seen_wait = 0;
    return SCOPA_OK;
}

int32_t scopa_set_deal(scopa_ctx *ctx, const uint8_t perm16[16]) {
    if (!ctx || !perm16) return SCOPA_EINVAL;
    uint32_t seen = 0;
    for (int i = 0; i < 16; i++) { if (perm16[i] > 15) return fail(ctx, SCOPA_EINVAL, "scopa_set_deal: card id > 15"); seen |= 1u << perm16[i]; }
    SC_REQUIRE(ctx, seen == 0xFFFFu, SCOPA_EINVAL, "scopa_set_deal: not a permutation of the 16 cards");
    SC_HIP(ctx, hipSetDevice(ctx->device));
    { const int32_t rc = ensure_scratch(ctx, 4096); if (rc != SCOPA_OK) return rc; }
    memcpy(ctx->perm, perm16, 16);
    SC_HIP(ctx, hipMemcpyAsync(ctx->d_scratch, ctx->perm, 16, hipMemcpyHostToDevice, ctx->stream));
    hipLaunchKernelGGL(k_tree_build, dim3(1), dim3(1024), 0, ctx->stream, (const uint8_t *)ctx->d_scratch, ctx->d_states,
                       ctx->d_infoset, ctx->d_payoff, ctx->d_key, ctx->d_meta);
    SC_HIP(ctx, hipGetLastError());
    int32_t n_inf = 0;
    SC_HIP(ctx, hipMemcpyAsync(&n_inf, ctx->d_meta, sizeof n_inf, hipMemcpyDeviceToHost, ctx->stream));
    SC_HIP(ctx, hipStreamSynchronize(ctx->stream));
    SC_REQUIRE(ctx, n_inf > 0 && n_inf <= kDecision, SCOPA_EHIP, "scopa_set_deal: tree build produced a bad infoset count");
    ctx->n_infosets = n_inf;
    ctx->has_deal = true;
    ctx->d_delta = ctx->d_delta_own;
    ctx->sched_valid = false;
    ctx->sdnode_valid = false;
    ctx->eval_thr_valid = false;
    scopa::mccfr_graphs_clear(ctx);
    return scopa_tables_reset(ctx);
}

int32_t scopa_tree_counts(scopa_ctx *ctx, int32_t *n_nodes, int32_t *n_decision, int32_t *n_infosets) {
    if (!ctx) return SCOPA_EINVAL;
    SC_REQUIRE(ctx, ctx->has_deal, SCOPA_ESTATE, "scopa_tree_counts: no deal set");
    if (n_nodes) *n_nodes = kNodes;
    if (n_decision) *n_decision = kDecision;
    if (n_infosets) *n_infosets = ctx->n_infosets;
    return SCOPA_OK;
}

int32_t scopa_tree_export(scopa_ctx *ctx, scopa_state *h_states, int32_t *h_infoset, int8_t *h_r2, uint64_t *h_infoset_key,
                          int8_t *h_infoset_nlegal, int8_t *h_infoset_legal) {
    if (!ctx) return SCOPA_EINVAL;
    SC_REQUIRE(ctx, ctx->has_deal, SCOPA_ESTATE, "scopa_tree_export: no deal set");
    SC_HIP(ctx, hipSetDevice(ctx->device));
    std::vector<scopa_state> st(kNodes);
    std::vector<uint16_t> inf(kDecision);
    std::vector<int8_t> pay(kTerminal);
    std::vector<uint64_t> keys((size_t)ctx->n_infosets);
    SC_HIP(ctx, hipMemcpyAsync(st.data(), ctx->d_states, sizeof(scopa_state) * kNodes, hipMemcpyDeviceToHost, ctx->stream));
    SC_HIP(ctx, hipMemcpyAsync(inf.data(), ctx->d_infoset, sizeof(uint16_t) * kDecision, hipMemcpyDeviceToHost, ctx->stream));
    SC_HIP(ctx, hipMemcpyAsync(pay.data(), ctx->d_payoff, kTerminal, hipMemcpyDeviceToHost, ctx->stream));
    SC_HIP(ctx, hipMemcpyAsync(keys.data(), ctx->d_key, sizeof(uint64_t) * keys.size(), hipMemcpyDeviceToHost, ctx->stream));
    SC_HIP(ctx, hipStreamSynchronize(ctx->stream));
    for (int d = 0; d <= kPlies; d++) {
        for (int j = 0; j < level_width(d); j++) {
            int dfs = 0, jj = j;
            for (int k = d - 1; k >= 0; k--) { const int n = nlegal_at(k); dfs += 1 + (jj % n) * subtree_size(k + 1); jj /= n; }
            const int bfs = level_offset(d) + j;
            if (h_states) h_states[dfs] = st[(size_t)bfs];
            if (h_infoset) h_infoset[dfs] = d < kPlies ? (int32_t)inf[(size_t)bfs] : -1;
            if (h_r2) {
                const int r0 = d < kPlies ? 0 : pay[(size_t)j];
                h_r2[dfs * 2] = (int8_t)r0;
                h_r2[dfs * 2 + 1] = (int8_t)-r0;
            }
        }
    }
    for (int i = 0; i < ctx->n_infosets; i++) {
        const uint64_t k = keys[(size_t)i];
        if (h_infoset_key) h_infoset_key[i] = k;
        const int n = (int)((k >> 1) & 7);
        if (h_infoset_nlegal) h_infoset_nlegal[i] = (int8_t)n;
        if (h_infoset_legal)
            for (int c = 0; c < 4; c++) h_infoset_legal[i * 4 + c] = (int8_t)(c < n ? (int)((k >> (4 + 4 * c)) & 15) : -1);
    }
    return SCOPA_OK;
}

}
```

Before: 140.2 billion.

## Precompute per-node threshold table in LDS and software-pipeline ply lookups

Thresholds move out of the per-infoset sigcdf rows, which shrink from 6 to 4 doubles, into a per-walk-node table of uint4 holding three thresholds plus the infoset id. The prepare and apply kernels scatter into this table through a node-to-infoset map built on the host at deal time. The walk then does one LDS uint4 read per node instead of a chained infoset lookup followed by a threshold read. Lane-table slices and scratch keys for the next ply are prefetched one step ahead to hide LDS latency. The cost is extra LDS (8 KB), extra scatter writes in every apply, and more live registers.

```diff
diff --git a/include/scopa.h b/include/scopa.h
--- a/include/scopa.h
+++ b/include/scopa.h
@@ -98,6 +98,7 @@
 int32_t scopa_mccfr_iteration_counter(scopa_ctx *ctx, uint32_t *iteration);
 int32_t scopa_mccfr_graph_mode(scopa_ctx *ctx, int32_t on);
 int32_t scopa_debug_lds_limit(scopa_ctx *ctx, int32_t bytes);
+int32_t scopa_debug_mccfr_node_table(scopa_ctx *ctx, uint32_t *h_entries);
 
 int32_t scopa_sdcfr_frontier_width(int32_t traverser, int32_t ply);
 int32_t scopa_sdcfr_features(scopa_ctx *ctx, int32_t ply, int64_t n, const int32_t *d_idx, float *d_feats, float *d_mask);
diff --git a/scopa_amd/_lib.py b/scopa_amd/_lib.py
--- a/scopa_amd/_lib.py
+++ b/scopa_amd/_lib.py
@@ -17,7 +17,7 @@
     "scopa_tree_counts", "scopa_tree_export", "scopa_tables_reset", "scopa_tables_get", "scopa_tables_set",
     "scopa_visited_get", "scopa_cfr_exact_iterate", "scopa_cfr_exact_traverse", "scopa_cfr_exact_mode", "scopa_cfr_exact_last_route", "scopa_cfr_exact_traverse_from", "scopa_mccfr_replay", "scopa_mccfr_seed",
     "scopa_mccfr_iterate", "scopa_mccfr_traverse", "scopa_mccfr_delta_buffer", "scopa_mccfr_bind_delta", "scopa_mccfr_delta_get", "scopa_mccfr_delta_set", "scopa_mccfr_apply",
-    "scopa_mccfr_iteration_counter", "scopa_mccfr_graph_mode", "scopa_debug_lds_limit", "scopa_sdcfr_frontier_width", "scopa_sdcfr_features", "scopa_sdcfr_expand",
+    "scopa_mccfr_iteration_counter", "scopa_mccfr_graph_mode", "scopa_debug_lds_limit", "scopa_debug_mccfr_node_table", "scopa_sdcfr_frontier_width", "scopa_sdcfr_features", "scopa_sdcfr_expand",
     "scopa_sdcfr_terminal_values", "scopa_sdcfr_backward", "scopa_sdcfr_visits", "scopa_sdcfr_policy_get", "scopa_sdcfr_traverse_fused", "scopa_sdcfr_image_floats", "scopa_sdcfr_pack_weights", "scopa_sdcfr_tuning", "scopa_sdcfr_mode", "scopa_sdcfr_train_params", "scopa_sdcfr_train_step", "scopa_sdcfr_train_steps", "scopa_sdcfr_average_policy", "scopa_features_from_states",
     "scopa_eval_init_states", "scopa_eval_step", "scopa_eval_tabular_step", "scopa_eval_tabular_prepare", "scopa_eval_tabular_match", "scopa_cfr_sync_iterate", "scopa_multi_create", "scopa_multi_destroy",
     "scopa_multi_deal_py_seeds", "scopa_multi_set_perms", "scopa_multi_perms_get", "scopa_multi_build", "scopa_multi_cfr_exact_iterate",
@@ -113,6 +113,7 @@
         "scopa_mccfr_iteration_counter": (i32, [vp, C.POINTER(u32)]),
         "scopa_mccfr_graph_mode": (i32, [vp, i32]),
         "scopa_debug_lds_limit": (i32, [vp, i32]),
+        "scopa_debug_mccfr_node_table": (i32, [vp, vp]),
         "scopa_exploitability": (i32, [vp, vp, vp, vp]),
         "scopa_sdcfr_frontier_width": (i32, [i32, i32]),
         "scopa_sdcfr_features": (i32, [vp, i32, i64, vp, vp, vp]),
@@ -370,6 +371,11 @@
     def debug_lds_limit(self, nbytes):
         self._ck(self._L.scopa_debug_lds_limit(self._h, int(nbytes)), "scopa_debug_lds_limit")
 
+    def debug_mccfr_node_table(self):
+        e = np.zeros((501, 4), np.uint32)
+        self._ck(self._L.scopa_debug_mccfr_node_table(self._h, _ptr(e)), "scopa_debug_mccfr_node_table")
+        return e
+
     def mccfr_iteration(self):
         v = C.c_uint32()
         self._ck(self._L.scopa_mccfr_iteration_counter(self._h, C.byref(v)), "scopa_mccfr_iteration_counter")
diff --git a/scopa_amd/csrc/scopa_ctx.h b/scopa_amd/csrc/scopa_ctx.h
--- a/scopa_amd/csrc/scopa_ctx.h
+++ b/scopa_amd/csrc/scopa_ctx.h
@@ -32,6 +32,8 @@
     double *d_delta_own = nullptr;
     double *d_scratch = nullptr;
     double *d_sigcdf = nullptr;
+    uint32_t *d_nodethr = nullptr;
+    uint16_t *d_nodemap = nullptr;
     bool sigcdf_valid = false;
     bool mccfr_all_seen = false;
     uint32_t mccfr_seen_wait = 0;
@@ -145,5 +147,6 @@
 bool prof_events(scopa_ctx *ctx, hipEvent_t *start, hipEvent_t *stop);
 void p2p_release(scopa_ctx *ctx);
 void mccfr_graphs_clear(scopa_ctx *ctx);
+int32_t mccfr_node_map_build(scopa_ctx *ctx);
 
 }
diff --git a/scopa_amd/csrc/scopa_host.hip b/scopa_amd/csrc/scopa_host.hip
--- a/scopa_amd/csrc/scopa_host.hip
+++ b/scopa_amd/csrc/scopa_host.hip
@@ -127,7 +127,7 @@
               hipMalloc(&ctx->d_key, sizeof(uint64_t) * kDecision) == hipSuccess &&
               hipMalloc(&ctx->d_meta, sizeof(int32_t) * 8) == hipSuccess &&
               hipMalloc(&ctx->d_visit, sizeof(uint32_t) * kDecision) == hipSuccess &&
-              hipMalloc(&ctx->d_sigcdf, (size_t)kDecision * 6 * sizeof(double)) == hipSuccess &&
+              hipMalloc(&ctx->d_sigcdf, (size_t)kDecision * 4 * sizeof(double)) == hipSuccess &&
               hipMalloc(&ctx->d_groups, scopa::kDeltaGroups * scopa::kDeltaTable * sizeof(double)) == hipSuccess &&
               hipMalloc(&ctx->d_regret, rows * 4 * sizeof(double)) == hipSuccess &&
               hipMalloc(&ctx->d_strat, rows * 4 * sizeof(double)) == hipSuccess &&
@@ -151,7 +151,7 @@
     scopa::mccfr_graphs_clear(ctx);
     for (hipEvent_t e : ctx->ev_pool) (void)hipEventDestroy(e);
     void *bufs[] = {ctx->d_states, ctx->d_infoset, ctx->d_payoff, ctx->d_key, ctx->d_meta, ctx->d_regret, ctx->d_strat,
-                    ctx->d_local, ctx->d_delta_own, ctx->d_scratch, ctx->d_counters, ctx->d_visit, ctx->d_sigcdf, ctx->d_groups, ctx->d_clock, ctx->d_sched, ctx->d_lane_tab, ctx->d_sdnode, ctx->d_sdpol, ctx->d_train_partial, ctx->d_eval_thr, ctx->d_sdavg};
+                    ctx->d_local, ctx->d_delta_own, ctx->d_scratch, ctx->d_counters, ctx->d_visit, ctx->d_sigcdf, ctx->d_nodemap, ctx->d_groups, ctx->d_clock, ctx->d_sched, ctx->d_lane_tab, ctx->d_sdnode, ctx->d_sdpol, ctx->d_train_partial, ctx->d_eval_thr, ctx->d_sdavg};
     for (void *b : bufs) if (b) (void)hipFree(b);
     if (ctx->own_stream) (void)hipStreamDestroy(ctx->stream);
     delete ctx;
diff --git a/scopa_amd/csrc/scopa_mccfr.hip b/scopa_amd/csrc/scopa_mccfr.hip
--- a/scopa_amd/csrc/scopa_mccfr.hip
+++ b/scopa_amd/csrc/scopa_mccfr.hip
@@ -29,12 +29,10 @@
 #pragma unroll
     for (int i = 0; i < 4; i++) thr[i] = i < n ? (uint32_t)ceil((cdf[i] / last) * 2147483648.0) : 0xFFFFFFFFu;
 }
-__device__ __forceinline__ void row_store(double *__restrict__ row, const double *sg, const uint32_t *thr) {
+__device__ __forceinline__ void row_store(double *__restrict__ row, const double *sg) {
     double2 *out = reinterpret_cast<double2 *>(row);
     out[0] = make_double2(sg[0], sg[1]);
     out[1] = make_double2(sg[2], sg[3]);
-    out[2] = make_double2(__longlong_as_double((long long)(((unsigned long long)thr[1] << 32) | thr[0])),
-                          __longlong_as_double((long long)(((unsigned long long)thr[3] << 32) | thr[2])));
 }
 __device__ __forceinline__ void choice_cdf_f64(const double *sigma, int n, double *cdf) {
     double c = sigma[0];
@@ -49,15 +47,32 @@
     return ntl_at(trav, d) == 0 ? 1 : ntl_at(trav, d) == 1 ? 5 : ntl_at(trav, d) == 2 ? 20 : 60;
 }
 
-constexpr int kRow = 6;
+constexpr int kRow = 4;
+constexpr int kWalkNodes = 501, kNodeTabLds = 512;
+constexpr int kNodeMapInline = 7, kNodeMapOverflow = kDecision * 8, kNodeMapHalves = kDecision * 8 + 512;
 constexpr int kUpd = 26;
 constexpr unsigned int kPairDecisionVisits = (1 + 5 + 5 + 20 + 20 + 60 + 60 + 120) + (1 + 1 + 5 + 5 + 20 + 20 + 60 + 60), kPairTerminalVisits = 120 + 120;
 static_assert(kPairDecisionVisits == 463, "291 + 172");
 
+__device__ __forceinline__ void node_thr_scatter(int r, const uint32_t *thr, uint4 desc, const uint16_t *__restrict__ g_nodemap, uint4 *__restrict__ g_nodethr) {
+    const uint32_t w[4] = {desc.x, desc.y, desc.z, desc.w};
+    const int cnt = (int)(w[0] & 0xFFFFu);
+    const uint4 e = make_uint4(thr[0], thr[1], thr[2], (uint32_t)r);
+    if (cnt <= kNodeMapInline) {
+#pragma unroll
+        for (int i = 1; i <= kNodeMapInline; i++)
+            if (i <= cnt) g_nodethr[(w[i >> 1] >> (16 * (i & 1))) & 0xFFFFu] = e;
+    } else {
+        const uint16_t *list = g_nodemap + kNodeMapOverflow + (w[0] >> 16);
+        for (int i = 0; i < cnt; i++) g_nodethr[list[i]] = e;
+    }
+}
+
 }
 
 __global__ void __launch_bounds__(256)
-k_mccfr_prepare(const uint64_t *__restrict__ g_key, const double *__restrict__ g_regret, double *__restrict__ g_sigcdf, int n_infosets) {
+k_mccfr_prepare(const uint64_t *__restrict__ g_key, const double *__restrict__ g_regret, double *__restrict__ g_sigcdf, int n_infosets,
+                const uint16_t *__restrict__ g_nodemap, uint4 *__restrict__ g_nodethr) {
     const int r = blockIdx.x * blockDim.x + threadIdx.x;
     if (r >= n_infosets) return;
     const int n = (int)((g_key[r] >> 1) & 7);
@@ -66,7 +81,8 @@
     for (int c = 0; c < 4; c++) R[c] = g_regret[r * 4 + c];
     mc_sigma(R, n, sg);
     choice_cdf(sg, n, thr);
-    row_store(g_sigcdf + r * kRow, sg, thr);
+    row_store(g_sigcdf + r * kRow, sg);
+    node_thr_scatter(r, thr, *reinterpret_cast<const uint4 *>(g_nodemap + r * 8), g_nodemap, g_nodethr);
 }
 
 constexpr int kIdentSlot = 166;
@@ -98,7 +114,7 @@
 }
 
 constexpr int kLaneSlotVecs = 15;
-constexpr int kStaticLds = 64 + kLaneSlotVecs * 1024;
+constexpr int kStaticLds = 64 + kLaneSlotVecs * 1024 + kNodeTabLds * 16;
 constexpr int kStaticLdsMulti = kStaticLds;
 
 template <int NP>
@@ -185,6 +201,7 @@
 struct WalkEnv {
     uint32_t wsb;
     uint32_t tab;
+    uint32_t nthr;
     const uint16_t *s_inf;
     const int8_t *s_pay;
     const double *s_sigcdf;
@@ -193,19 +210,32 @@
     unsigned int *s_cnt;
 };
 
-template <int D, int NP>
-__device__ __forceinline__ void ply_step(const WalkEnv &e, int lane, NodeRegs (&st)[NP]) {
+constexpr int ply_rounds(int d) { return task_nodes(0, d) + task_nodes(1, d) > 64 ? 2 : 1; }
+template <int NP, int NR>
+struct PlyAhead {
+    uint4 sl[NR];
+    uint32_t k[NP][NR];
+};
+struct LeafAhead { uint4 lf[2]; };
+
+template <int D, int NP, class Next>
+__device__ __forceinline__ void ply_step(const WalkEnv &e, int lane, NodeRegs (&st)[NP], const PlyAhead<NP, ply_rounds(D)> &cur, Next &nx) {
     constexpr int n = 4 - (D >> 1);
     constexpr int c0 = task_nodes(0, D), c1 = task_nodes(1, D);
-    constexpr int NR = c0 + c1 > 64 ? 2 : 1;
+    constexpr int NR = ply_rounds(D);
     struct Pre {
         int idx, In;
         uint32_t k, thr0, thr1, thr2;
     };
     Pre g[NP][NR];
-    uint4 sl[NR];
-#pragma unroll
-    for (int r = 0; r < NR; r++) sl[r] = lds_read_u4(e.tab + 1024u * (uint32_t)(D + r));
+    const uint4 (&sl)[NR] = cur.sl;
+    if constexpr (D < 5) {
+#pragma unroll
+        for (int r = 0; r < ply_rounds(D < 5 ? D + 1 : D); r++) nx.sl[r] = lds_read_u4(e.tab + 1024u * (uint32_t)(D + 1 + r));
+    } else {
+#pragma unroll
+        for (int q = 0; q < 2; q++) nx.lf[q] = lds_read_u4(e.tab + 1024u * (uint32_t)(kLvLeaf + q));
+    }
 #pragma unroll
     for (int i = 0; i < NP; i++)
 #pragma unroll
@@ -218,13 +248,19 @@
                 const uint32_t act = ((ppk >> 21) & sl[r].y) | sl[r].z;
                 q.idx = (int)((ppk & 1023u) * pn + act);
             }
-            q.In = e.s_inf[level_offset(D) + q.idx];
-            q.k = lds_read_u32(e.wsb + sl[r].w + (uint32_t)(i * sizeof(WaveScratch)));
-            const uint32_t *thr = reinterpret_cast<const uint32_t *>(e.s_sigcdf + q.In * kRow + 4);
-            q.thr0 = thr[0];
-            q.thr1 = n > 2 ? thr[1] : 0xFFFFFFFFu;
-            q.thr2 = n > 3 ? thr[2] : 0xFFFFFFFFu;
-        }
+            const uint4 nt = lds_read_u4(e.nthr + 16u * (uint32_t)(level_offset(D) + q.idx));
+            q.k = cur.k[i][r];
+            q.In = (int)nt.w;
+            q.thr0 = nt.x;
+            q.thr1 = n > 2 ? nt.y : 0xFFFFFFFFu;
+            q.thr2 = n > 3 ? nt.z : 0xFFFFFFFFu;
+        }
+    if constexpr (D < 5) {
+#pragma unroll
+        for (int i = 0; i < NP; i++)
+#pragma unroll
+            for (int r = 0; r < ply_rounds(D < 5 ? D + 1 : D); r++) nx.k[i][r] = lds_read_u32(e.wsb + nx.sl[r].w + (uint32_t)(i * sizeof(WaveScratch)));
+    }
 #pragma unroll
     for (int i = 0; i < NP; i++)
 #pragma unroll
@@ -259,27 +295,34 @@
     const unsigned long long w_start_ = wall_clock64();
     unsigned long long t_prev_ = clock64();
 #endif
+    PlyAhead<NP, 1> a0, a1, a2, a3, a4;
+    PlyAhead<NP, 2> a5;
+    LeafAhead al;
+    a0.sl[0] = lds_read_u4(e.tab);
     draw_pairs<NP>(e.wsb, lane, b, iteration, seed_lo, seed_hi);
+#pragma unroll
+    for (int i = 0; i < NP; i++) a0.k[i][0] = lds_read_u32(e.wsb + a0.sl[0].w + (uint32_t)(i * sizeof(WaveScratch)));
     WALK_STAMP(0);
     NodeRegs st[NP];
 #pragma unroll
     for (int i = 0; i < NP; i++) st[i].pk = 0u;
-    ply_step<0, NP>(e, lane, st); WALK_STAMP(1);
-    ply_step<1, NP>(e, lane, st); WALK_STAMP(2);
-    ply_step<2, NP>(e, lane, st); WALK_STAMP(3);
-    ply_step<3, NP>(e, lane, st); WALK_STAMP(4);
-    ply_step<4, NP>(e, lane, st); WALK_STAMP(5);
-    ply_step<5, NP>(e, lane, st); WALK_STAMP(6);
+    ply_step<0, NP>(e, lane, st, a0, a1); WALK_STAMP(1);
+    ply_step<1, NP>(e, lane, st, a1, a2); WALK_STAMP(2);
+    ply_step<2, NP>(e, lane, st, a2, a3); WALK_STAMP(3);
+    ply_step<3, NP>(e, lane, st, a3, a4); WALK_STAMP(4);
+    ply_step<4, NP>(e, lane, st, a4, a5); WALK_STAMP(5);
+    ply_step<5, NP>(e, lane, st, a5, al); WALK_STAMP(6);
     my_pairs += NP;
+    uint4 u[6];
     {
-        uint4 lf[2];
-#pragma unroll
-        for (int q = 0; q < 2; q++) lf[q] = lds_read_u4(e.tab + 1024u * (uint32_t)(kLvLeaf + q));
+        const uint4 (&lf)[2] = al.lf;
         uint32_t ppk[NP][2];
 #pragma unroll
         for (int i = 0; i < NP; i++)
 #pragma unroll
             for (int q = 0; q < 2; q++) ppk[i][q] = lds_read_u32(e.wsb + lf[q].x + (uint32_t)(i * sizeof(WaveScratch)));
+#pragma unroll
+        for (int q = 0; q < 6; q++) u[q] = lds_read_u4(e.tab + 1024u * (uint32_t)(kLvUpd + q));
         int I6[NP][2], I7[NP][2], pay[NP][2];
 #pragma unroll
         for (int i = 0; i < NP; i++)
@@ -309,9 +352,6 @@
     WALK_STAMP(7);
     if (lane < 2 * kUpd) {
         const bool trav1 = lane >= kUpd;
-        uint4 u[6];
-#pragma unroll
-        for (int q = 0; q < 6; q++) u[q] = lds_read_u4(e.tab + 1024u * (uint32_t)(kLvUpd + q));
         const uint32_t ro[5] = {u[0].x, u[0].y, u[0].z, u[0].w, u[1].x}, own = u[1].y;
         const int nX = (int)u[1].z;
         const uint32_t p6o[4] = {u[2].x, u[2].y, u[2].z, u[2].w};
@@ -405,7 +445,9 @@
     if (g_iter) iteration = *g_iter;
     __shared__ uint32_t s_next[1];
     __shared__ uint32_t s_slice[1];
-    __shared__ uint4 s_lane_tab[kLaneSlotVecs * 64];
+    __shared__ uint4 s_lane_tab[kLaneSlotVecs * 64 + kNodeTabLds];
+    uint4 *s_nodethr = s_lane_tab + kLaneSlotVecs * 64;
+    const uint4 *g_nodethr = g_lane_tab + kLaneSlotVecs * 64;
     const unsigned long long t_start = wall_clock64();
 #ifdef SCOPA_WALK_STAMPS
     const unsigned long long c_entry_ = clock64();
@@ -422,6 +464,7 @@
     const int tid = threadIdx.x, lane = tid & 63, wave = tid >> 6, n_waves = blockDim.x >> 6, nthr = blockDim.x;
     if (tid < 2) s_vis[tid] = 0u;
     const uint4 lane_piece = tid < kLaneSlotVecs * 64 ? g_lane_tab[tid] : make_uint4(0u, 0u, 0u, 0u);
+    const uint4 node_piece = tid < kWalkNodes ? g_nodethr[tid] : make_uint4(0u, 0u, 0u, 0u);
     if (tid == 0) {
         s_slice[0] = 0u;
         const uint32_t per_wg = (nb + gridDim.x - 1) / gridDim.x, W = blockDim.x >> 6;
@@ -430,14 +473,15 @@
     }
     const uint32_t *gi = reinterpret_cast<const uint32_t *>(g_infoset), *gp = reinterpret_cast<const uint32_t *>(g_payoff);
     {
-        constexpr int kSig = 5;
+        constexpr int kSig = 4;
+        constexpr int kRowPieces = kRow / 2;
         const double2 *g2 = reinterpret_cast<const double2 *>(g_sigcdf);
         double2 *s2 = reinterpret_cast<double2 *>(s_sigcdf);
         double2 v[kSig];
 #pragma unroll
         for (int j = 0; j < kSig; j++) {
             const int idx = tid + j * nthr;
-            v[j] = idx < I * 3 ? g2[idx] : make_double2(0.0, 0.0);
+            v[j] = idx < I * kRowPieces ? g2[idx] : make_double2(0.0, 0.0);
         }
         const uint32_t wi = tid < kDecision / 2 ? gi[tid] : 0u;
         const uint32_t wp = tid < kTerminal / 4 ? gp[tid] : 0u;
@@ -449,15 +493,17 @@
 #pragma unroll
         for (int j = 0; j < kSig; j++) {
             const int idx = tid + j * nthr;
-            if (idx < I * 3) s2[idx] = v[j];
-        }
-        for (int idx = tid + kSig * nthr; idx < I * 3; idx += nthr) s2[idx] = g2[idx];
+            if (idx < I * kRowPieces) s2[idx] = v[j];
+        }
+        for (int idx = tid + kSig * nthr; idx < I * kRowPieces; idx += nthr) s2[idx] = g2[idx];
         if (tid < kLaneSlotVecs * 64) s_lane_tab[tid] = lane_piece;
+        if (tid < kWalkNodes) s_nodethr[tid] = node_piece;
         if (tid < kDecision / 2) reinterpret_cast<uint32_t *>(s_inf)[tid] = wi;
         if (tid == 0) s_inf[kDecision - 1] = last_inf;
         if (tid < kTerminal / 4) reinterpret_cast<uint32_t *>(s_pay)[tid] = wp;
     }
     for (int i = tid + nthr; i < kLaneSlotVecs * 64; i += nthr) s_lane_tab[i] = g_lane_tab[i];
+    for (int i = tid + nthr; i < kWalkNodes; i += nthr) s_nodethr[i] = g_nodethr[i];
     for (int i = tid + nthr; i < kDecision / 2; i += nthr) reinterpret_cast<uint32_t *>(s_inf)[i] = gi[i];
     for (int i = tid + nthr; i < kTerminal / 4; i += nthr) reinterpret_cast<uint32_t *>(s_pay)[i] = gp[i];
     __syncthreads();
@@ -470,7 +516,7 @@
     WaveScratch *ws = s_wave + 2 * wave;
     wave_scratch_init(ws, 2, lane, I);
     WalkEnv env;
-    env.wsb = lds_addr(ws); env.tab = lds_addr(s_lane_tab) + 16u * (uint32_t)lane;
+    env.wsb = lds_addr(ws); env.tab = lds_addr(s_lane_tab) + 16u * (uint32_t)lane; env.nthr = lds_addr(s_nodethr);
     env.s_inf = s_inf; env.s_pay = s_pay; env.s_sigcdf = s_sigcdf; env.s_dR = s_dR; env.s_seen = track_seen ? s_seen : nullptr; env.s_cnt = s_cnt;
     unsigned int my_pairs = 0;
     {
@@ -504,6 +550,7 @@
         if (lane == 0 && blockIdx.x == 0) { unsigned int hw; asm volatile("s_getreg_b32 %0, hwreg(HW_REG_HW_ID)" : "=s"(hw)); g_wave_clocks[32 + wave] = hw; }
 #endif
     }
+    if (lane == 0) { atomicAdd(&s_vis[0], my_pairs * kPairDecisionVisits); atomicAdd(&s_vis[1], my_pairs * kPairTerminalVisits); }
     {
         uint32_t sl = 0;
         if (lane == 0) sl = atomicAdd(s_slice, 1u);
@@ -545,8 +592,6 @@
             for (int r = tid + 2 * nthr; r < I; r += nthr)
                 if ((s_seen[r] || s_cnt[r]) && g_visit[r] == 0u) g_visit[r] = 0x40000000u + (uint32_t)r;
     }
-    if (lane == 0) { atomicAdd(&s_vis[0], my_pairs * kPairDecisionVisits); atomicAdd(&s_vis[1], my_pairs * kPairTerminalVisits); }
-    __syncthreads();
     if (tid < 2) atomicAdd(&g_wg_counts[blockIdx.x * 2 + tid], (unsigned long long)s_vis[tid]);
 #ifdef SCOPA_WALK_STAMPS
     if (blockIdx.x == 0 && (tid & 63) == 0) {
@@ -567,6 +612,7 @@
     extern __shared__ __align__(16) unsigned char smem[];
     __shared__ unsigned int s_vis[2];
     __shared__ uint4 s_lane_tab[kLaneSlotVecs * 64];
+    __shared__ uint4 s_nodethr[kNodeTabLds];
     for (int i = threadIdx.x; i < kLaneSlotVecs * 64; i += blockDim.x) s_lane_tab[i] = g_lane_tab[i];
     {
         const size_t deal = blockIdx.x;
@@ -592,17 +638,23 @@
     WaveScratch *ws = s_wave + wave;
     wave_scratch_init(ws, 1, lane, I);
     WalkEnv env;
-    env.wsb = lds_addr(ws); env.tab = lds_addr(s_lane_tab) + 16u * (uint32_t)lane;
+    env.wsb = lds_addr(ws); env.tab = lds_addr(s_lane_tab) + 16u * (uint32_t)lane; env.nthr = lds_addr(s_nodethr);
     env.s_inf = s_inf; env.s_pay = s_pay; env.s_sigcdf = s_sigcdf; env.s_dR = s_R; env.s_seen = s_seen; env.s_cnt = s_cnt;
     unsigned int my_pairs = 0;
     for (uint32_t it = 0; it < n_iters; it++) {
         for (int r = tid; r < I; r += blockDim.x) {
             const int n = (int)((g_key[r] >> 1) & 7);
             double sg[4];
+            mc_sigma(s_R + r * 4, n, sg);
+            for (int c = 0; c < 4; c++) s_sigcdf[r * kRow + c] = sg[c];
+        }
+        for (int x = tid; x < kWalkNodes; x += blockDim.x) {
+            const int r = s_inf[x], n = (int)((g_key[r] >> 1) & 7);
+            double sg[4];
             uint32_t thr[4];
             mc_sigma(s_R + r * 4, n, sg);
             choice_cdf(sg, n, thr);
-            for (int c = 0; c < 4; c++) { s_sigcdf[r * kRow + c] = sg[c]; reinterpret_cast<uint32_t *>(s_sigcdf + r * kRow + 4)[c] = thr[c]; }
+            s_nodethr[x] = make_uint4(thr[0], thr[1], thr[2], (uint32_t)r);
         }
         __syncthreads();
         for (uint32_t pg = (uint32_t)wave; pg < batch; pg += (uint32_t)n_waves) {
@@ -642,11 +694,13 @@
     for (int k = 0; k < 5; k++) g_delta[r * 5 + k] += d[k];
 }
 
-struct ApplyRow { double R[4], S[4], sg[4]; int n; };
+struct ApplyRow { double R[4], S[4], sg[4]; int n; uint4 nodes; };
 
 __device__ __forceinline__ ApplyRow apply_row_load(int r, const uint64_t *__restrict__ g_key, const double *__restrict__ g_regret,
-                                                   const double *__restrict__ g_strat, const double *__restrict__ g_sigcdf) {
+                                                   const double *__restrict__ g_strat, const double *__restrict__ g_sigcdf,
+                                                   const uint16_t *__restrict__ g_nodemap) {
     ApplyRow a;
+    a.nodes = *reinterpret_cast<const uint4 *>(g_nodemap + r * 8);
     const double2 r0 = *reinterpret_cast<const double2 *>(g_regret + r * 4), r1 = *reinterpret_cast<const double2 *>(g_regret + r * 4 + 2);
     const double2 s0 = *reinterpret_cast<const double2 *>(g_strat + r * 4), s1 = *reinterpret_cast<const double2 *>(g_strat + r * 4 + 2);
     const double2 g0 = *reinterpret_cast<const double2 *>(g_sigcdf + r * kRow), g1 = *reinterpret_cast<const double2 *>(g_sigcdf + r * kRow + 2);
@@ -658,7 +712,8 @@
 }
 
 __device__ __forceinline__ void apply_row_store(int r, ApplyRow &a, const double (&d)[5], double *__restrict__ g_regret,
-                                                double *__restrict__ g_strat, double *__restrict__ g_sigcdf) {
+                                                double *__restrict__ g_strat, double *__restrict__ g_sigcdf,
+                                                const uint16_t *__restrict__ g_nodemap, uint4 *__restrict__ g_nodethr) {
 #pragma unroll
     for (int c = 0; c < 4; c++)
         if (c < a.n) { a.R[c] += d[c]; a.S[c] += d[4] * a.sg[c]; }
@@ -670,7 +725,8 @@
     uint32_t thr[4];
     mc_sigma(a.R, a.n, sg);
     choice_cdf(sg, a.n, thr);
-    row_store(g_sigcdf + r * kRow, sg, thr);
+    row_store(g_sigcdf + r * kRow, sg);
+    node_thr_scatter(r, thr, a.nodes, g_nodemap, g_nodethr);
 }
 
 __device__ __forceinline__ double groups_cell_take(double *__restrict__ g_groups, int r, int k) {
@@ -690,35 +746,38 @@
 
 __global__ void __launch_bounds__(kApplyThreads)
 k_mccfr_apply_groups(const uint64_t *__restrict__ g_key, double *__restrict__ g_regret, double *__restrict__ g_strat,
-                     double *__restrict__ g_groups, int n_infosets, double *__restrict__ g_sigcdf, uint32_t *__restrict__ g_iter) {
+                     double *__restrict__ g_groups, int n_infosets, double *__restrict__ g_sigcdf, uint32_t *__restrict__ g_iter,
+                     const uint16_t *__restrict__ g_nodemap, uint4 *__restrict__ g_nodethr) {
     if (g_iter && blockIdx.x == 0 && threadIdx.x == 0) *g_iter += 1u;
     const int lane = threadIdx.x & 63, k = lane & (kApplyLanes - 1);
     const int r = (int)(blockIdx.x * blockDim.x + threadIdx.x) / kApplyLanes;
     const bool valid = r < n_infosets;
     ApplyRow a{};
-    if (valid && k == 0) a = apply_row_load(r, g_key, g_regret, g_strat, g_sigcdf);
+    if (valid && k == 0) a = apply_row_load(r, g_key, g_regret, g_strat, g_sigcdf, g_nodemap);
     const double mine = (valid && k < 5) ? groups_cell_take(g_groups, r, k) : 0.0;
     double d[5];
 #pragma unroll
     for (int j = 0; j < 5; j++) d[j] = __shfl(mine, (lane & ~(kApplyLanes - 1)) + j);
-    if (valid && k == 0) apply_row_store(r, a, d, g_regret, g_strat, g_sigcdf);
+    if (valid && k == 0) apply_row_store(r, a, d, g_regret, g_strat, g_sigcdf, g_nodemap, g_nodethr);
 }
 
 __global__ void __launch_bounds__(64)
 k_mccfr_apply(const uint64_t *__restrict__ g_key, double *__restrict__ g_regret, double *__restrict__ g_strat,
-              double *__restrict__ g_delta, int n_infosets, double *__restrict__ g_sigcdf) {
+              double *__restrict__ g_delta, int n_infosets, double *__restrict__ g_sigcdf,
+              const uint16_t *__restrict__ g_nodemap, uint4 *__restrict__ g_nodethr) {
     const int r = blockIdx.x * blockDim.x + threadIdx.x;
     if (r >= n_infosets) return;
     double d[5];
     for (int k = 0; k < 5; k++) d[k] = g_delta[r * 5 + k];
-    ApplyRow a = apply_row_load(r, g_key, g_regret, g_strat, g_sigcdf);
+    ApplyRow a = apply_row_load(r, g_key, g_regret, g_strat, g_sigcdf, g_nodemap);
     for (int k = 0; k < 5; k++) g_delta[r * 5 + k] = 0.0;
-    apply_row_store(r, a, d, g_regret, g_strat, g_sigcdf);
+    apply_row_store(r, a, d, g_regret, g_strat, g_sigcdf, g_nodemap, g_nodethr);
 }
 
 __global__ void __launch_bounds__(64)
 k_mccfr_exchange_apply(scopa::P2PArgs xa, double *__restrict__ g_groups, const uint64_t *__restrict__ g_key, double *__restrict__ g_regret,
-                       double *__restrict__ g_strat, double *__restrict__ g_sigcdf, int n_infosets) {
+                       double *__restrict__ g_strat, double *__restrict__ g_sigcdf, int n_infosets,
+                       const uint16_t *__restrict__ g_nodemap, uint4 *__restrict__ g_nodethr) {
     __shared__ double xch[4][scopa::kP2PMaxWorld][5];
     const int rl = threadIdx.x >> 4, q = threadIdx.x & 15;
     const int r = blockIdx.x * 4 + rl;
@@ -728,9 +787,9 @@
 #pragma unroll
     for (int j = 0; j < 5; j++) d[j] = __shfl(mine, (int)(threadIdx.x & ~15u) + j);
     ApplyRow a{};
-    if (valid && q == 0) a = apply_row_load(r, g_key, g_regret, g_strat, g_sigcdf);
+    if (valid && q == 0) a = apply_row_load(r, g_key, g_regret, g_strat, g_sigcdf, g_nodemap);
     scopa::p2p_exchange_wave4(xa, r, valid, q, d, xch[rl]);
-    if (valid && q == 0) apply_row_store(r, a, d, g_regret, g_strat, g_sigcdf);
+    if (valid && q == 0) apply_row_store(r, a, d, g_regret, g_strat, g_sigcdf, g_nodemap, g_nodethr);
 }
 
 namespace {
@@ -835,7 +894,8 @@
 
 static int32_t ensure_lane_table(scopa_ctx *ctx) {
     if (ctx->d_lane_tab) return SCOPA_OK;
-    SC_HIP(ctx, hipMalloc(&ctx->d_lane_tab, (size_t)kLaneSlotVecs * 64 * sizeof(uint4)));
+    SC_HIP(ctx, hipMalloc(&ctx->d_lane_tab, (size_t)(kLaneSlotVecs * 64 + kNodeTabLds) * sizeof(uint4)));
+    ctx->d_nodethr = ctx->d_lane_tab + (size_t)kLaneSlotVecs * 64 * 4;
     hipLaunchKernelGGL(k_lane_table, dim3(1), dim3(64), 0, ctx->stream, (uint4 *)ctx->d_lane_tab);
     SC_HIP(ctx, hipGetLastError());
     return SCOPA_OK;
@@ -871,7 +931,7 @@
     if (int32_t rc = refresh_all_seen(ctx, false)) return rc;
     if (!ctx->sigcdf_valid) {
         hipLaunchKernelGGL(k_mccfr_prepare, dim3((ctx->n_infosets + 255) / 256), dim3(256), 0, ctx->stream, ctx->d_key,
-                           ctx->d_regret, ctx->d_sigcdf, ctx->n_infosets);
+                           ctx->d_regret, ctx->d_sigcdf, ctx->n_infosets, (const uint16_t *)ctx->d_nodemap, (uint4 *)ctx->d_nodethr);
         SC_HIP(ctx, hipGetLastError());
         ctx->sigcdf_valid = true;
     }
@@ -921,7 +981,7 @@
                            ctx->d_sigcdf, ctx->d_groups, ctx->n_infosets, (uint32_t)ctx->seed, (uint32_t)(ctx->seed >> 32),
                            0u, 0u, batch, ctx->d_counters + 8, ctx->d_visit, (unsigned long long *)nullptr, (const uint4 *)ctx->d_lane_tab, (const uint32_t *)d_iter, track);
         hipLaunchKernelGGL(k_mccfr_apply_groups, dim3((ctx->n_infosets * kApplyLanes + kApplyThreads - 1) / kApplyThreads), dim3(kApplyThreads), 0, ctx->stream, ctx->d_key,
-                           ctx->d_regret, ctx->d_strat, ctx->d_groups, ctx->n_infosets, ctx->d_sigcdf, d_iter);
+                           ctx->d_regret, ctx->d_strat, ctx->d_groups, ctx->n_infosets, ctx->d_sigcdf, d_iter, (const uint16_t *)ctx->d_nodemap, (uint4 *)ctx->d_nodethr);
     }
     const hipError_t e_end = hipStreamEndCapture(ctx->stream, &graph);
     if (e_end != hipSuccess || !graph) return scopa::fail(ctx, SCOPA_EHIP, "mccfr graph: stream capture", e_end);
@@ -936,6 +996,33 @@
 }
 
 namespace scopa {
+int32_t mccfr_node_map_build(scopa_ctx *ctx) {
+    if (int32_t rc = ensure_lane_table(ctx)) return rc;
+    if (!ctx->d_nodemap) SC_HIP(ctx, hipMalloc(&ctx->d_nodemap, (size_t)kNodeMapHalves * sizeof(uint16_t)));
+    uint16_t inf[kWalkNodes];
+    SC_HIP(ctx, hipMemcpyAsync(inf, ctx->d_infoset, sizeof inf, hipMemcpyDeviceToHost, ctx->stream));
+    SC_HIP(ctx, hipStreamSynchronize(ctx->stream));
+    std::vector<uint16_t> map((size_t)kNodeMapHalves, (uint16_t)0), cnt((size_t)kDecision, (uint16_t)0);
+    for (int x = 0; x < kWalkNodes; x++) {
+        SC_REQUIRE(ctx, inf[x] < ctx->n_infosets, SCOPA_EHIP, "scopa_set_deal: node -> infoset map out of range");
+        cnt[inf[x]]++;
+    }
+    int over = 0;
+    for (int r = 0; r < ctx->n_infosets; r++) {
+        map[(size_t)r * 8] = cnt[r];
+        if (cnt[r] > kNodeMapInline) { map[(size_t)r * 8 + 1] = (uint16_t)over; over += cnt[r]; }
+        cnt[r] = 0;
+    }
+    for (int x = 0; x < kWalkNodes; x++) {
+        const int r = inf[x], k = cnt[r]++;
+        if (map[(size_t)r * 8] > kNodeMapInline) map[(size_t)kNodeMapOverflow + map[(size_t)r * 8 + 1] + k] = (uint16_t)x;
+        else map[(size_t)r * 8 + 1 + k] = (uint16_t)x;
+    }
+    SC_HIP(ctx, hipMemcpyAsync(ctx->d_nodemap, map.data(), map.size() * sizeof(uint16_t), hipMemcpyHostToDevice, ctx->stream));
+    SC_HIP(ctx, hipStreamSynchronize(ctx->stream));
+    return SCOPA_OK;
+}
+
 int32_t launch_mccfr_multi(scopa_ctx *ctx, int n_deals, int max_infosets, const uint16_t *d_infoset, const int8_t *d_payoff,
                            const uint64_t *d_key, double *d_regret, double *d_strat, const int32_t *d_meta, uint32_t *d_visit,
                            unsigned long long *d_counters, uint64_t seed, uint32_t iter0, uint32_t n_iters, uint32_t batch) {
@@ -1026,11 +1113,11 @@
     scopa::Range r("scopa mccfr apply (split path)");
     if (!ctx->sigcdf_valid) {
         hipLaunchKernelGGL(k_mccfr_prepare, dim3((ctx->n_infosets + 255) / 256), dim3(256), 0, ctx->stream, ctx->d_key,
-                           ctx->d_regret, ctx->d_sigcdf, ctx->n_infosets);
+                           ctx->d_regret, ctx->d_sigcdf, ctx->n_infosets, (const uint16_t *)ctx->d_nodemap, (uint4 *)ctx->d_nodethr);
         SC_HIP(ctx, hipGetLastError());
     }
     hipLaunchKernelGGL(k_mccfr_apply, dim3((ctx->n_infosets + 63) / 64), dim3(64), 0, ctx->stream, ctx->d_key,
-                       ctx->d_regret, ctx->d_strat, ctx->d_delta, ctx->n_infosets, ctx->d_sigcdf);
+                       ctx->d_regret, ctx->d_strat, ctx->d_delta, ctx->n_infosets, ctx->d_sigcdf, (const uint16_t *)ctx->d_nodemap, (uint4 *)ctx->d_nodethr);
     SC_HIP(ctx, hipGetLastError());
     ctx->sigcdf_valid = true;
     ctx->iteration++;
@@ -1070,11 +1157,26 @@
         if (rc != SCOPA_OK) return rc;
         scopa::Range r("scopa mccfr apply");
         hipLaunchKernelGGL(k_mccfr_apply_groups, dim3((ctx->n_infosets * kApplyLanes + kApplyThreads - 1) / kApplyThreads), dim3(kApplyThreads), 0, ctx->stream, ctx->d_key,
-                           ctx->d_regret, ctx->d_strat, ctx->d_groups, ctx->n_infosets, ctx->d_sigcdf, (uint32_t *)nullptr);
+                           ctx->d_regret, ctx->d_strat, ctx->d_groups, ctx->n_infosets, ctx->d_sigcdf, (uint32_t *)nullptr, (const uint16_t *)ctx->d_nodemap, (uint4 *)ctx->d_nodethr);
         SC_HIP(ctx, hipGetLastError());
         ctx->sigcdf_valid = true;
         ctx->iteration++;
     }
+    return SCOPA_OK;
+}
+
+int32_t scopa_debug_mccfr_node_table(scopa_ctx *ctx, uint32_t *h_entries) {
+    if (!ctx || !h_entries) return SCOPA_EINVAL;
+    SC_REQUIRE(ctx, ctx->has_deal, SCOPA_ESTATE, "scopa_debug_mccfr_node_table: no deal set");
+    SC_HIP(ctx, hipSetDevice(ctx->device));
+    if (!ctx->sigcdf_valid) {
+        hipLaunchKernelGGL(k_mccfr_prepare, dim3((ctx->n_infosets + 255) / 256), dim3(256), 0, ctx->stream, ctx->d_key,
+                           ctx->d_regret, ctx->d_sigcdf, ctx->n_infosets, (const uint16_t *)ctx->d_nodemap, (uint4 *)ctx->d_nodethr);
+        SC_HIP(ctx, hipGetLastError());
+        ctx->sigcdf_valid = true;
+    }
+    SC_HIP(ctx, hipMemcpyAsync(h_entries, ctx->d_nodethr, (size_t)kWalkNodes * sizeof(uint4), hipMemcpyDeviceToHost, ctx->stream));
+    SC_HIP(ctx, hipStreamSynchronize(ctx->stream));
     return SCOPA_OK;
 }
 
@@ -1098,7 +1200,7 @@
         if (rc != SCOPA_OK) return rc;
         scopa::Range r("scopa mccfr exchange + apply");
         hipLaunchKernelGGL(k_mccfr_exchange_apply, dim3((ctx->n_infosets + 3) / 4), dim3(64), 0, ctx->stream, xa, ctx->d_groups, ctx->d_key,
-                           ctx->d_regret, ctx->d_strat, ctx->d_sigcdf, ctx->n_infosets);
+                           ctx->d_regret, ctx->d_strat, ctx->d_sigcdf, ctx->n_infosets, (const uint16_t *)ctx->d_nodemap, (uint4 *)ctx->d_nodethr);
         SC_HIP(ctx, hipGetLastError());
         ctx->sigcdf_valid = true;
         ctx->iteration++;
diff --git a/scopa_amd/csrc/scopa_tree.hip b/scopa_amd/csrc/scopa_tree.hip
--- a/scopa_amd/csrc/scopa_tree.hip
+++ b/scopa_amd/csrc/scopa_tree.hip
@@ -224,6 +224,7 @@
     SC_HIP(ctx, hipStreamSynchronize(ctx->stream));
     SC_REQUIRE(ctx, n_inf > 0 && n_inf <= kDecision, SCOPA_EHIP, "scopa_set_deal: tree build produced a bad infoset count");
     ctx->n_infosets = n_inf;
+    { const int32_t rc = scopa::mccfr_node_map_build(ctx); if (rc != SCOPA_OK) return rc; }
     ctx->has_deal = true;
     ctx->d_delta = ctx->d_delta_own;
     ctx->sched_valid = false;
```

Measured after the change: 138.0 billion. 1.5% lower.
